# caltech-netlab/adacharge

Hardware: AMD Instinct MI355X
Metric: MPC QP solves/sec whole-node, 54 EVSE x horizon 12; max rate residual vs cvxpy (higher is better)
Workload: dtype f64; 1 GPU; caltech54 (Caltech-shaped, 54 EVSE) x horizon 12, quick_charge + equal_share*1e-12, SOC constraints, batches of 256 independent MPC snapshots (BASELINE.json configs[1]); one step = one acnqp_solve_batches call over 64 such batches per GPU (16384 problems), pinned host buffers in, host buffers out: H2D + kernels + D2H inside the timed region; batch=256, n_evse=54, horizon=12, constraint_type=SOC, parallelism=dp1 (own snapshots per GPU)

## Files before the change

adacharge_amd/backend.py:

```python
from __future__ import annotations

import ctypes as C
import dataclasses
import os
from dataclasses import dataclass
from typing import Optional

import numpy as np

from .builder import CONE_SOC, ProblemBatch, SiteData

_LIB_NAME = "libacn_qp_hip.so"
_LIB_DIR = os.path.join(os.path.dirname(os.path.abspath(__file__)), "lib")

STATUS_UNSET = 0
STATUS_SOLVED = 1
STATUS_MAX_ITER = 2
STATUS_PRIMAL_INFEASIBLE = 3
STATUS_EMPTY_SET = 4
STATUS_SOLVED_INACCURATE = 5
ACCEPTED_STATUSES = (STATUS_SOLVED, STATUS_SOLVED_INACCURATE)
STATUS_NAMES = {
    STATUS_UNSET: "unset",
    STATUS_SOLVED: "optimal",
    STATUS_MAX_ITER: "max_iter_reached",
    STATUS_PRIMAL_INFEASIBLE: "infeasible",
    STATUS_EMPTY_SET: "infeasible",
    STATUS_SOLVED_INACCURATE: "optimal_inaccurate",
}
PILOTS_CONTINUOUS, PILOTS_DISCRETE, PILOTS_REALLOCATE = 0, 1, 2
ADVANCE_REFUSED, ADVANCE_NO_ROW, ADVANCE_BAD_SLOT = 1, 2, 4
PREPARE_FUTURE = 1
PLANT_BAD_PLUG, PLANT_BAD_BATTERY = 1, 2
ESTIMATE_BAD_FRESH, ESTIMATE_BAD_SLOT = 1, 2
ROUTE_NAMES = {1: "wave1", 2: "wave2", 3: "wave3", 4: "wave4", 5: "wave5", 6: "tiled_ct1", 7: "tiled_ct2",
               8: "long_lds", 9: "long_ws", 10: "stream", 11: "general"}


class BackendUnavailable(RuntimeError):
    """The HIP library could not be loaded or no MI355X is visible."""


_I4, _F8, _U1 = np.int32, np.float64, np.uint8
_PROBLEM_ARRAYS = dict(horizon=_I4, lb=_F8, ub=_F8, q=_F8, pdiag=_F8, s_off=_I4, s_len=_I4, s_cap=_F8, s_eq=_U1, peak=_F8, lf=_F8,
                       dc=_F8, dfloor=_F8)
_NEXT_ARRAYS = tuple(k for k in _PROBLEM_ARRAYS if k != "s_eq")
_WARM = ("warm_x", "warm_y")
_TABLE_ARRAYS = dict(horizon=_I4, q_index=_I4, q_table=_F8, pdiag=_F8, s_eq=_U1, peak=_F8, lf=_F8, dc=_F8, dfloor=_F8, sess_seg=_I4,
                     s_evse=_I4, s_slot=_I4, s_off=_I4, s_len=_I4, s_cap=_F8, rate_seg=_I4, min_rates=_F8, max_rates=_F8)
_RESULT_ARRAYS = dict(x=_F8, status=_I4, iters=_I4, pri_res=_F8, dua_res=_F8, obj=_F8)
_PILOT_ARRAYS = dict(cre=_F8, cim=_F8, limits=_F8, max_pilot=_F8, levels=_F8, sess_seg=_I4, s_evse=_I4, s_arrived=_U1, s_cap=_F8)
_ADVANCE_ARRAYS = dict(q_table=_F8, h_scal=_F8, h_row=_I4, peak_series=_F8, a_seg=_I4, a_evse=_I4, a_slot=_I4, a_len=_I4, a_cap=_F8,
                       a_rate_seg=_I4, a_min=_F8, a_max=_F8)
_COST_ARRAYS = dict(c_weight=_F8, c_series=_F8)
_PREPARE_ARRAYS = dict(key=_I4, cre=_F8, cim=_F8, limits=_F8, min_pilot=_F8)
_PLANT_ARRAYS = dict(t_room=_F8, t_amps=_F8, t_knee=_F8, t_slope=_F8, plug=_I4)
_RESOLVE_ARRAYS = dict(sel_seg=_I4, sel_idx=_I4, pos=_I4)
SELECT_BAD_INDEX = 1
HOLD_BAD_ROW = 1


def _ints(*names):
    return [(k, C.c_int32) for k in names]


def _doubles(*names):
    return [(k, C.c_double) for k in names]


def _ptrs(*names):
    return [(k, C.c_void_p) for k in names]


class _Site(C.Structure):
    _fields_ = _ints("n_evse", "n_infra", "n_rows", "cone", "has_peak", "has_flat", "has_max") + _ptrs("G", "limits")


class _Problems(C.Structure):

    _fields_ = _ints("batch", "t_max", "k_sessions") + _ptrs(*_PROBLEM_ARRAYS, *_WARM)


class _Table(C.Structure):
    _fields_ = _ints("batch", "t_max", "k_sessions", "n_sessions", "n_horizons") + _ptrs(*_TABLE_ARRAYS)


class _Results(C.Structure):
    _fields_ = _ptrs(*_RESULT_ARRAYS, "y", "x_dev")


class _Duals(C.Structure):
    _fields_ = _ptrs("mu", "z", "res")


class _PilotPlan(C.Structure):
    _fields_ = _ints("batch", "t_max", "n_evse", "n_infra", "n_levels", "n_sessions", "mode") + _ptrs(*_PILOT_ARRAYS)


class _Pilots(C.Structure):
    _fields_ = _ptrs("pilots", "first", "visits")


class _AdvancePlan(C.Structure):
    _fields_ = (_ints("n_evse", "n_rows", "n_horizons", "step", "peak_len", "n_arrivals", "n_rates")
                + _doubles("done_tol", "kw_per_amp", "warm_arrival_gain") + _ptrs(*_ADVANCE_ARRAYS))


class ClockCost(C.Structure):

    _fields_ = _ints("n_evse", "series_len") + _doubles("coef") + _ptrs("weight", "series")


class _Next(C.Structure):
    _fields_ = _ptrs(*_NEXT_ARRAYS, *_WARM)


class _PreparePlan(C.Structure):
    _fields_ = _ints("n_evse", "n_infra") + _ptrs(*_PREPARE_ARRAYS)


class _PrepareView(C.Structure):
    _fields_ = _ptrs("v_evse", "v_arrived", "v_cap")


class Options(C.Structure):

    _fields_ = (_doubles("eps_abs", "eps_rel") + _ints("max_iter", "check_every", "adapt_every")
                + _doubles("rho", "sigma", "alpha", "adapt_tol", "reg_rel")
                + _ints("precision", "accel_mem", "stall_iters", "retry_passes", "retry_max_iter", "polish_iters")
                + _doubles("retry_rho", "inaccurate_floor") + _ints("polish_stall"))


def _abi():
    P, ptr, i32, i64, rc = C.POINTER, C.c_void_p, C.c_int32, C.c_int64, C.c_int
    h = stream = ptr
    solve = [h, P(_Problems), P(Options), P(_Results)]
    advance = [h, P(_Problems), ptr, ptr, ptr, ptr, P(_AdvancePlan)]
    rows = [
        ("acnqp_create", rc, [P(_Site), i32, P(ptr)]),
        ("acnqp_destroy", None, [h]),
        ("acnqp_solve_batch", rc, solve),
        ("acnqp_solve_batch_device", rc, solve + [stream]),
        ("acnqp_solve_batches", rc, [h, i32, P(_Problems), P(Options), P(_Results)]),
        ("acnqp_solve_table", rc, [h, P(_Table), P(Options), P(_Results)]),
        ("acnqp_host_alloc", ptr, [C.c_size_t]),
        ("acnqp_host_free", None, [ptr]),
        ("acnqp_default_options", None, [P(Options)]),
        ("acnqp_last_error", C.c_char_p, []),
        ("acnqp_abi_version", i32, []),
        ("acnqp_last_kernel_ms", C.c_float, [h]),
        ("acnqp_kernel_times", i32, [h, P(C.c_float), i32]),
        ("acnqp_launch_count", i64, [h]),
        ("acnqp_ordered_launch_count", i64, [h]),
        ("acnqp_polish_stats", rc, [h, P(i64), i32]),
        ("acnqp_accel_columns", i32, [h, i32, i32, i32, i32]),
        ("acnqp_route", i32, [h, i32, i32, i32, P(i32)]),
        ("acnqp_set_long_polish", rc, [h, i32]),
        ("acnqp_set_wide_polish", rc, [h, i32]),
    ]
    for stem, args in (
        ("acnqp_duals", [h, P(_Problems), P(Options), ptr, ptr, ptr, P(_Duals)]),
        ("acnqp_pilots", [h, P(_PilotPlan), ptr, P(_Pilots)]),
        ("acnqp_advance", advance + [P(_Next), ptr]),
        ("acnqp_advance_priced", advance + [P(ClockCost), P(_Next), ptr]),
        ("acnqp_prepare", [h, P(_Problems), P(_PreparePlan), ptr, ptr, P(_PrepareView), ptr]),
        ("acnqp_plant", [h, P(_Problems), ptr, ptr, i32] + [ptr] * 9),
        ("acnqp_estimate", [h, P(_Problems)] + [ptr] * 4 + [C.c_double] * 3 + [ptr] * 3),
        ("acnqp_select", [h, P(_Problems), i32, i32, i32, ptr, P(_Next), ptr, ptr]),
        ("acnqp_hold", [h, P(_Problems), i32, i32, i32, ptr, P(_Results), ptr, ptr, ptr, P(_Results), ptr, ptr]),
    ):
        rows += [(stem + "_host", rc, args), (stem + "_device", rc, args + [stream])]
    introspection = [
        ("acnqp_debug_polish_alongside", i64, [h]),
        ("acnqp_debug_direct_x", i64, [h]),
        ("acnqp_debug_wave_rank", rc, [h, P(i32)]),
        ("acnqp_debug_wave_evse_extent", rc, [h, P(i32)]),
        ("acnqp_debug_order_keys", rc, [h, P(_Problems), P(i32)]),
        ("acnqp_debug_copy_workspace", i64, [h, ptr, i64]),
    ]
    return tuple(r + (True,) for r in rows) + tuple(r + (False,) for r in introspection)


_ABI = _abi()
EXPORTED_SYMBOLS = tuple(name for name, _, _, declared in _ABI if declared)

_lib = None


def library_path() -> str:
    return os.environ.get("ACNQP_LIBRARY", os.path.join(_LIB_DIR, _LIB_NAME))


def load_library():
    global _lib
    if _lib is not None:
        return _lib
    try:
        import torch
    except ImportError:
        pass
    path = library_path()
    if not os.path.exists(path):
        raise BackendUnavailable(
            f"{path} not found: build it with `python -c 'import __graft_entry__ as g; g.build()'` "
            "(hipcc --offload-arch=gfx950).  adacharge_amd has no CPU fallback."
        )
    try:
        lib = C.CDLL(path)
    except OSError as exc:
        raise BackendUnavailable(f"cannot load {path}: {exc}") from exc
    for name, restype, argtypes, declared in _ABI:
        if declared or hasattr(lib, name):
            fn = getattr(lib, name)
            fn.restype, fn.argtypes = restype, argtypes
    _lib = lib
    return lib


def default_options(**overrides) -> Options:
    o = Options()
    load_library().acnqp_default_options(C.byref(o))
    for k, v in overrides.items():
        if not hasattr(o, k):
            raise TypeError(f"unknown solver option {k!r}")
        setattr(o, k, v)
    return o


def _check(rc: int, what: str):
    if rc != 0:
        msg = load_library().acnqp_last_error().decode()
        if rc == -3:
            raise BackendUnavailable(f"{what}: {msg}")
        if rc == -1:
            raise ValueError(f"{what}: {msg}")
        raise RuntimeError(f"{what} failed (rc={rc}): {msg}")


def _ptr(a: Optional[np.ndarray]):
    return None if a is None else a.ctypes.data_as(C.c_void_p)


def _addr(a: Optional[np.ndarray]):
    return None if a is None else a.ctypes.data


def _dptr(t):
    return None if t is None else C.c_void_p(t.data_ptr())


def _f8(a):
    return None if a is None else np.ascontiguousarray(a, np.float64)


def _i4(a):
    return None if a is None else np.ascontiguousarray(a, np.int32)


def _torch_dtype(dtype):
    import torch

    return getattr(torch, np.dtype(dtype).name)


def _want(t, name: str, dtype, shape=None, device=None) -> None:
    if t is None:
        return
    if device is None:
        ok = t.element_size() == np.dtype(dtype).itemsize
    else:
        import torch

        ok = isinstance(t, torch.Tensor) and t.device == device and t.dtype == _torch_dtype(dtype)
    if not ok or not t.is_contiguous() or (shape is not None and tuple(t.shape) != tuple(shape)):
        raise ValueError(f"{name} must be a contiguous torch.{np.dtype(dtype).name} tensor" + ("" if device is None else f" on {device}")
                         + ("" if shape is None else f" of shape {tuple(shape)}"))


def _absent(site: SiteData, peak: bool = False) -> tuple:
    return (() if site.has_flat else ("lf",)) + (() if site.has_max else ("dc", "dfloor")) + (("peak",) if peak and not site.has_peak else ())


def _host_arrays(src, arrays: dict, absent) -> dict:
    return {k: None if k in absent or (a := getattr(src, "T" if k == "horizon" else k)) is None else np.ascontiguousarray(a, dt)
            for k, dt in arrays.items()}


def _new_results(B: int, N: int, Tm: int, Mg: int, pinned: bool, want_y: bool, x_dev=None, out: Optional["BatchResult"] = None):
    if out is not None and out.x.shape == (B, N, Tm) and (not want_y or (out.y is not None and out.y.shape == (B, Mg, Tm))):
        res = out
    else:
        new = pinned_empty if pinned else np.zeros
        res = BatchResult(*[new((B, N, Tm) if k == "x" else B, dt) for k, dt in _RESULT_ARRAYS.items()])
        if want_y:
            res.y = new((B, Mg, Tm))
    r = _Results(*[_addr(getattr(res, k)) for k in _RESULT_ARRAYS], _addr(res.y) if want_y else None,
                 None if x_dev is None else C.c_void_p(int(x_dev)))
    return res, r


def _marshal_batch(site: SiteData, batch: ProblemBatch, pinned: bool, x_dev=None, warm=None, want_y=False):
    B, N, Tm = batch.B, batch.N, batch.Tm
    arrs = _host_arrays(batch, _PROBLEM_ARRAYS, _absent(site))
    wx = wy = None
    if warm is not None:
        wx, wy = _f8(warm[0]), _f8(warm[1])
        if wx.shape != (B, N, Tm) or wy.shape != (B, site.Mg, Tm):
            raise ValueError(f"warm start arrays must have shapes {(B, N, Tm)} and {(B, site.Mg, Tm)}")
    p = _Problems(B, Tm, batch.K, *[_addr(a) for a in arrs.values()], _addr(wx), _addr(wy))
    res, r = _new_results(B, N, Tm, site.Mg, pinned, want_y, x_dev)
    return p, r, res, (arrs, wx, wy)


def _device_problems(dev: "DeviceBatch", warm_x=None, warm_y=None) -> _Problems:
    return _Problems(dev.B, dev.Tm, dev.K, *[_dptr(getattr(dev, k)) for k in _PROBLEM_ARRAYS], _dptr(warm_x), _dptr(warm_y))


@dataclass
class BatchResult:
    x: np.ndarray
    status: np.ndarray
    iters: np.ndarray
    pri_res: np.ndarray
    dua_res: np.ndarray
    obj: np.ndarray
    kernel_ms: float = float("nan")
    y: Optional[np.ndarray] = None
    x_dev: Optional[object] = None
    handle: Optional[object] = None


@dataclass
class DualResult:
    mu: np.ndarray
    z: Optional[np.ndarray]
    stat: np.ndarray
    energy: np.ndarray
    site: np.ndarray
    comp: np.ndarray


class _PlanArrays:

    _DTYPES = {}

    def to_device(self, device):
        import torch

        moved = {k: None if getattr(self, k) is None else torch.from_numpy(np.ascontiguousarray(getattr(self, k), dt)).to(device)
                 for k, dt in self._DTYPES.items()}
        return dataclasses.replace(self, **moved)

    def _p(self, k: str, keep=None, row: int = 0, stacked: Optional[int] = None):
        a = getattr(self, k)
        if a is None or (a.numel() if hasattr(a, "numel") else a.size) == 0:
            return None
        if a.ndim == stacked:
            a = a[row]
        if hasattr(a, "data_ptr"):
            return C.c_void_p(a.data_ptr())
        a = np.ascontiguousarray(a, self._DTYPES[k])
        if keep is not None:
            keep.append(a)
        return _ptr(a)

    def _len(self, k: str, axis: int = 0) -> int:
        return 0 if getattr(self, k) is None else int(getattr(self, k).shape[axis])


@dataclass
class PilotPlan(_PlanArrays):
    mode: int
    B: int
    Tm: int
    N: int
    max_pilot: Optional[object] = None
    levels: Optional[object] = None
    cre: Optional[object] = None
    cim: Optional[object] = None
    limits: Optional[object] = None
    sess_seg: Optional[object] = None
    s_evse: Optional[object] = None
    s_arrived: Optional[object] = None
    s_cap: Optional[object] = None

    _DTYPES = _PILOT_ARRAYS
    _ARRAYS = tuple(_PILOT_ARRAYS)

    def _struct(self, batch=None, t_max=None, keep=None) -> "_PilotPlan":
        return _PilotPlan(int(self.B if batch is None else batch), int(self.Tm if t_max is None else t_max), self.N, self._len("cre"),
                          self._len("levels", 1), self._len("s_evse"), self.mode, *[self._p(k, keep) for k in _PILOT_ARRAYS])


@dataclass
class AdvancePlan(_PlanArrays):
    q_table: object
    h_scal: object
    h_row: object
    done_tol: float
    kw_per_amp: float
    peak_series: Optional[object] = None
    a_seg: Optional[object] = None
    a_evse: Optional[object] = None
    a_slot: Optional[object] = None
    a_len: Optional[object] = None
    a_cap: Optional[object] = None
    a_rate_seg: Optional[object] = None
    a_min: Optional[object] = None
    a_max: Optional[object] = None
    warm_arrival_gain: float = 0.0
    c_coef: Optional[float] = None
    c_weight: Optional[object] = None
    c_series: Optional[object] = None

    _DTYPES = {**_ADVANCE_ARRAYS, **_COST_ARRAYS}
    _ARRAYS = tuple(_ADVANCE_ARRAYS)

    def _struct(self, N: int, Mg: int, step: int, seg_row: int = 0, keep=None) -> "_AdvancePlan":
        A = self._len("a_evse")
        ptrs = [self._p(k, keep, seg_row, 2 if k == "a_seg" else None) for k in _ADVANCE_ARRAYS]
        if not A:
            ptrs[self._ARRAYS.index("a_seg")] = None
        return _AdvancePlan(int(N), int(Mg), int(self.q_table.shape[0]), int(step), self._len("peak_series", 1), A, self._len("a_min"),
                            float(self.done_tol), float(self.kw_per_amp), float(self.warm_arrival_gain), *ptrs)

    def _cost_struct(self, N: int, keep=None) -> Optional["ClockCost"]:
        given = [self.c_coef is not None, self.c_weight is not None, self.c_series is not None]
        if not any(given):
            return None
        if not all(given):
            raise ValueError("a clock cost needs c_coef, c_weight and c_series")
        if self.c_series.ndim != 2:
            raise ValueError("c_series must have shape (B, P)")
        for k, dt in _COST_ARRAYS.items():
            if hasattr(getattr(self, k), "data_ptr"):
                _want(getattr(self, k), k, dt)
        return ClockCost(int(N), int(self.c_series.shape[1]), float(self.c_coef), *[self._p(k, keep) for k in _COST_ARRAYS])


@dataclass
class PreparePlan(_PlanArrays):
    key: object
    cre: Optional[object] = None
    cim: Optional[object] = None
    limits: Optional[object] = None
    min_pilot: Optional[object] = None

    _DTYPES = _PREPARE_ARRAYS
    _ARRAYS = tuple(_PREPARE_ARRAYS)

    def _struct(self, N: int, key_row=None, min_rates: bool = True, keep=None) -> "_PreparePlan":
        return _PreparePlan(int(N), self._len("cre"), self._p("key", keep, 0 if key_row is None else key_row, 3), self._p("cre", keep),
                            self._p("cim", keep), self._p("limits", keep), self._p("min_pilot", keep) if min_rates else None)


@dataclass
class PlantPlan(_PlanArrays):
    t_room: object
    t_amps: object
    t_knee: object
    t_slope: object
    plug: object

    _DTYPES = _PLANT_ARRAYS
    _ARRAYS = tuple(_PLANT_ARRAYS)

    def _args(self, plug_row=None, keep=None) -> list:
        return [C.c_int32(self._len("t_room"))] + [self._p(k, keep, 0 if plug_row is None else plug_row, 3 if k == "plug" else None)
                                                   for k in _PLANT_ARRAYS]


@dataclass
class ResolvePlan(_PlanArrays):
    sel_seg: object
    sel_idx: object
    pos: object

# ... 255 lines not shown
                   warm_x=np.empty((B, N, Tm)) if xs is not None else None, warm_y=np.empty((B, Mg, Tm)) if ys is not None else None)
        flags = np.empty(B, np.int32)
        p = _Problems(B, Tm, K, lb=_ptr(lb), ub=_ptr(ub), s_off=_ptr(off), s_len=_ptr(ln), s_cap=_ptr(cap), dfloor=_ptr(dfl))
        keep = []
        pl = plan._struct(N, Mg, step, seg_row, keep)
        nx = _Next(*[_ptr(out[k]) for k in _NEXT_ARRAYS + _WARM])
        cost = plan._cost_struct(N, keep)
        if cost is not None and plan.c_series.shape[0] != B:
            raise ValueError(f"c_series has {plan.c_series.shape[0]} rows, the batch has {B} problems")
        head = (self._h, C.byref(p), _ptr(app), _ptr(stat), _ptr(xs), _ptr(ys), C.byref(pl))
        if cost is None:
            _check(self._lib.acnqp_advance_host(*head, C.byref(nx), _ptr(flags)), "acnqp_advance_host")
        else:
            _check(self._lib.acnqp_advance_priced_host(*head, C.byref(cost), C.byref(nx), _ptr(flags)), "acnqp_advance_priced_host")
        del keep
        out["flags"] = flags
        return {k: v for k, v in out.items() if v is not None}

    def advance_device(self, cur: "DeviceBatch", nxt: "DeviceBatch", applied, plan: AdvancePlan, step: int, flags, use_status: bool = True,
                       warm_x=None, warm_y=None, stream: int = 0, seg_row: int = 0) -> None:
        if (cur.B, cur.N, cur.Tm, cur.K) != (nxt.B, nxt.N, nxt.Tm, nxt.K):
            raise ValueError("cur and nxt must have the same shape (B, N, Tm, K)")
        if warm_y is not None and cur.y is None:
            raise ValueError("warm_y needs the site-row multipliers: DeviceBatch(..., want_y=True)")
        _want(applied, "applied", _F8, (cur.B, cur.N))
        _want(flags, "flags", _I4, (cur.B,))
        p = _device_problems(cur)
        pl = plan._struct(cur.N, self.site.Mg, step, seg_row)
        nx = _Next(*[_dptr(getattr(nxt, k)) for k in _NEXT_ARRAYS], _dptr(warm_x), _dptr(warm_y))
        cost = plan._cost_struct(cur.N)
        if cost is not None and plan.c_series.shape[0] != cur.B:
            raise ValueError(f"c_series has {plan.c_series.shape[0]} rows, the batch has {cur.B} problems")
        head = (self._h, C.byref(p), _dptr(applied), _dptr(cur.status) if use_status else None,
                _dptr(cur.x) if warm_x is not None else None, _dptr(cur.y) if warm_y is not None else None, C.byref(pl))
        if cost is None:
            _check(self._lib.acnqp_advance_device(*head, C.byref(nx), _dptr(flags), C.c_void_p(stream)), "acnqp_advance_device")
        else:
            _check(self._lib.acnqp_advance_priced_device(*head, C.byref(cost), C.byref(nx), _dptr(flags), C.c_void_p(stream)),
                   "acnqp_advance_priced_device")

    def prepare_host(self, cur: dict, plan: PreparePlan, want_view: bool = True, min_rates: bool = True, key_row=None) -> dict:
        lb, ub = np.array(cur["lb"], np.float64, order="C"), np.array(cur["ub"], np.float64, order="C")
        off, ln, cap = _i4(cur["s_off"]), _i4(cur["s_len"]), _f8(cur["s_cap"])
        if lb.ndim != 3 or lb.shape[1] != self.site.N or ub.shape != lb.shape:
            raise ValueError("cur needs lb, ub of shape (B, N, Tm) for the handle's site")
        B, N, Tm = lb.shape
        K = off.shape[1] if off.ndim == 3 else 1
        if off.size != B * K * N or ln.size != off.size or cap.size != off.size:
            raise ValueError("cur needs s_off, s_len, s_cap of shape (B, K, N)")
        view = dict(v_evse=np.empty((B, N), np.int32), v_arrived=np.empty((B, N), np.uint8), v_cap=np.empty((B, N))) if want_view else {}
        flags = np.empty(B, np.int32)
        p = _Problems(B, Tm, K, s_off=_ptr(off), s_len=_ptr(ln), s_cap=_ptr(cap))
        keep = []
        pl = plan._struct(N, key_row, min_rates, keep)
        v = _PrepareView(*[_ptr(view.get(k)) for k in ("v_evse", "v_arrived", "v_cap")])
        _check(self._lib.acnqp_prepare_host(self._h, C.byref(p), C.byref(pl), _ptr(lb), _ptr(ub), C.byref(v), _ptr(flags)), "acnqp_prepare_host")
        del keep
        return dict(lb=lb, ub=ub, flags=flags, **view)

    def prepare_device(self, cur: "DeviceBatch", plan: PreparePlan, flags, v_evse=None, v_arrived=None, v_cap=None, min_rates: bool = True,
                       key_row=None, stream: int = 0) -> None:
        import torch

        here = torch.device("cuda", self.device)
        B, N, Tm, K = cur.B, cur.N, cur.Tm, cur.K
        M = plan._len("cre")
        if plan.key is None or not hasattr(plan.key, "dim"):
            raise ValueError("plan.key must be a tensor on the handle's GPU (PreparePlan.to_device)")
        _want(plan.key, "plan.key", _I4, (B, N) if plan.key.dim() == 2 else (plan.key.shape[0], B, N), here)
        if plan.key.dim() == 3 and not 0 <= (0 if key_row is None else int(key_row)) < plan.key.shape[0]:
            raise ValueError("key_row is outside plan.key")
        for k, shape in dict(cre=(M, N), cim=(M, N), limits=(M,), min_pilot=(N,)).items():
            _want(getattr(plan, k), "plan." + k, _PREPARE_ARRAYS[k], shape, here)
        for k, shape in dict(lb=(B, N, Tm), ub=(B, N, Tm), s_off=(B, K, N), s_len=(B, K, N), s_cap=(B, K, N)).items():
            _want(getattr(cur, k), "cur." + k, _PROBLEM_ARRAYS[k], shape, here)
        _want(flags, "flags", _I4, (B,), here)
        if flags is None:
            raise ValueError("flags is required")
        for t, name, dt in ((v_evse, "v_evse", _I4), (v_arrived, "v_arrived", _U1), (v_cap, "v_cap", _F8)):
            _want(t, name, dt, (B, N), here)
        p = _Problems(B, Tm, K, s_off=_dptr(cur.s_off), s_len=_dptr(cur.s_len), s_cap=_dptr(cur.s_cap))
        pl = plan._struct(N, key_row, min_rates)
        v = _PrepareView(_dptr(v_evse), _dptr(v_arrived), _dptr(v_cap))
        _check(self._lib.acnqp_prepare_device(self._h, C.byref(p), C.byref(pl), _dptr(cur.lb), _dptr(cur.ub), C.byref(v), _dptr(flags),
                                              C.c_void_p(stream)), "acnqp_prepare_device")

    def plant_host(self, cur: dict, plan: PlantPlan, pilots, bat, room, status=None, plug_row=None) -> dict:
        off, ln, pil, stat = _i4(cur["s_off"]), _i4(cur["s_len"]), _f8(pilots), _i4(status)
        bat, room = np.array(bat, np.int32, order="C"), np.array(room, np.float64, order="C")
        if pil.ndim != 2 or pil.shape[1] != self.site.N:
            raise ValueError("pilots must have the shape (B, N) of the handle's site")
        B, N = pil.shape
        K = off.shape[1] if off.ndim == 3 else 1
        if off.size != B * K * N or ln.size != off.size or bat.shape != (B, N) or room.shape != (B, N):
            raise ValueError("cur needs s_off, s_len of shape (B, K, N); bat and room have the shape (B, N)")
        plug = plan.plug if plan.plug.ndim == 2 else plan.plug[0 if plug_row is None else plug_row]
        if plug.shape != (B, N) or (stat is not None and stat.shape != (B,)):
            raise ValueError("plan.plug needs one (B, N) block per step and status the shape (B,)")
        actual, flags = np.empty((B, N)), np.empty(B, np.int32)
        p = _Problems(B, 1, K, s_off=_ptr(off), s_len=_ptr(ln))
        keep = []
        _check(self._lib.acnqp_plant_host(self._h, C.byref(p), _ptr(pil), _ptr(stat), *plan._args(plug_row, keep), _ptr(bat), _ptr(room),
                                          _ptr(actual), _ptr(flags)), "acnqp_plant_host")
        del keep
        return dict(bat=bat, room=room, actual=actual, flags=flags)

    def plant_device(self, cur: "DeviceBatch", plan: PlantPlan, pilots, bat, room, actual, flags, status=None, plug_row=None,
                     stream: int = 0) -> None:
        import torch

        here = torch.device("cuda", self.device)
        B, N, K = cur.B, cur.N, cur.K
        R = plan._len("t_room")
        if plan.plug is None or not hasattr(plan.plug, "dim"):
            raise ValueError("plan.plug must be a tensor on the handle's GPU (PlantPlan.to_device)")
        _want(plan.plug, "plan.plug", _I4, (B, N) if plan.plug.dim() == 2 else (plan.plug.shape[0], B, N), here)
        if plan.plug.dim() == 3 and not 0 <= (0 if plug_row is None else int(plug_row)) < plan.plug.shape[0]:
            raise ValueError("plug_row is outside plan.plug")
        for k in ("t_room", "t_amps", "t_knee", "t_slope"):
            _want(getattr(plan, k), "plan." + k, _F8, (R,), here)
        for k in ("s_off", "s_len"):
            _want(getattr(cur, k), "cur." + k, _I4, (B, K, N), here)
        for t, name, dt, shape in ((pilots, "pilots", _F8, (B, N)), (bat, "bat", _I4, (B, N)), (room, "room", _F8, (B, N)),
                                   (actual, "actual", _F8, (B, N)), (flags, "flags", _I4, (B,)), (status, "status", _I4, (B,))):
            if t is None and name != "status":
                raise ValueError(f"{name} is required")
            _want(t, name, dt, shape, here)
        p = _Problems(B, cur.Tm, K, s_off=_dptr(cur.s_off), s_len=_dptr(cur.s_len))
        _check(self._lib.acnqp_plant_device(self._h, C.byref(p), _dptr(pilots), _dptr(status), *plan._args(plug_row), _dptr(bat), _dptr(room),
                                            _dptr(actual), _dptr(flags), C.c_void_p(stream)), "acnqp_plant_device")

    def estimate_host(self, cur: dict, fresh, est, pilots=None, actual=None, status=None, up_threshold: float = 1.0,
                      down_threshold: float = 1.0, up_increment: float = 1.0, fresh_row=None) -> dict:
        lb, ub = _f8(cur["lb"]), _f8(cur["ub"])
        off, ln, fr = _i4(cur["s_off"]), _i4(cur["s_len"]), _i4(fresh)
        pil, act, stat = _f8(pilots), _f8(actual), _i4(status)
        est = np.array(est, np.float64, order="C")
        if ub.ndim != 3 or ub.shape[1] != self.site.N or lb.shape != ub.shape:
            raise ValueError("cur needs lb, ub of shape (B, N, Tm) for the handle's site")
        B, N, Tm = ub.shape
        K = off.shape[1] if off.ndim == 3 else 1
        if fr.ndim == 3:
            fr = fr[0 if fresh_row is None else fresh_row]
        if off.size != B * K * N or ln.size != off.size or fr.shape != (B, N) or est.shape != (B, N):
            raise ValueError("cur needs s_off, s_len of shape (B, K, N); fresh needs one (B, N) block per step and est the shape (B, N)")
        for a, name, shape in ((pil, "pilots", (B, N)), (act, "actual", (B, N)), (stat, "status", (B,))):
            if a is not None and a.shape != shape:
                raise ValueError(f"{name} must have the shape {shape}")
        fr = np.ascontiguousarray(fr)
        ub_out, flags = np.empty((B, N, Tm)), np.empty(B, np.int32)
        p = _Problems(B, Tm, K, s_off=_ptr(off), s_len=_ptr(ln), lb=_ptr(lb), ub=_ptr(ub))
        _check(self._lib.acnqp_estimate_host(self._h, C.byref(p), _ptr(fr), _ptr(pil), _ptr(act), _ptr(stat), float(up_threshold),
                                             float(down_threshold), float(up_increment), _ptr(est), _ptr(ub_out), _ptr(flags)),
               "acnqp_estimate_host")
        return dict(est=est, ub=ub_out, flags=flags)

    def estimate_device(self, cur: "DeviceBatch", fresh, est, ub_out, flags, pilots=None, actual=None, status=None, up_threshold: float = 1.0,
                        down_threshold: float = 1.0, up_increment: float = 1.0, fresh_row=None, stream: int = 0) -> None:
        import torch

        here = torch.device("cuda", self.device)
        B, N, Tm, K = cur.B, cur.N, cur.Tm, cur.K
        if fresh is None or not hasattr(fresh, "dim"):
            raise ValueError("fresh must be a tensor on the handle's GPU")
        _want(fresh, "fresh", _I4, (B, N) if fresh.dim() == 2 else (fresh.shape[0], B, N), here)
        row = 0
        if fresh.dim() == 3:
            row = 0 if fresh_row is None else int(fresh_row)
            if not 0 <= row < fresh.shape[0]:
                raise ValueError("fresh_row is outside fresh")
        for k, shape in dict(lb=(B, N, Tm), ub=(B, N, Tm), s_off=(B, K, N), s_len=(B, K, N)).items():
            _want(getattr(cur, k), "cur." + k, _PROBLEM_ARRAYS[k], shape, here)
        for t, name, dt, shape in ((est, "est", _F8, (B, N)), (ub_out, "ub_out", _F8, (B, N, Tm)), (flags, "flags", _I4, (B,)),
                                   (pilots, "pilots", _F8, (B, N)), (actual, "actual", _F8, (B, N)), (status, "status", _I4, (B,))):
            if t is None and name in ("est", "ub_out", "flags"):
                raise ValueError(f"{name} is required")
            _want(t, name, dt, shape, here)
        p = _Problems(B, Tm, K, s_off=_dptr(cur.s_off), s_len=_dptr(cur.s_len), lb=_dptr(cur.lb), ub=_dptr(cur.ub))
        fr = C.c_void_p(fresh.data_ptr() + row * B * N * 4)
        _check(self._lib.acnqp_estimate_device(self._h, C.byref(p), fr, _dptr(pilots), _dptr(actual), _dptr(status), float(up_threshold),
                                               float(down_threshold), float(up_increment), _dptr(est), _dptr(ub_out), _dptr(flags),
                                               C.c_void_p(stream)), "acnqp_estimate_device")

    def select_device(self, cur: "DeviceBatch", dense: "DeviceBatch", idx, flags, m: Optional[int] = None, warm_x=None, warm_y=None,
                      out_warm_x=None, out_warm_y=None, stream: int = 0) -> None:
        m = int(idx.shape[0] if m is None else m)
        if (cur.N, cur.Tm, cur.K) != (dense.N, dense.Tm, dense.K):
            raise ValueError("cur and dense must have the same shape (N, Tm, K)")
        if m > dense.B or m > idx.shape[0] or m > flags.shape[0]:
            raise ValueError(f"dense, idx and flags need room for m = {m} problems")
        for t, name, rows in ((out_warm_x, "out_warm_x", (cur.N, cur.Tm)), (out_warm_y, "out_warm_y", (self.site.Mg, cur.Tm))):
            if t is not None and (t.shape[0] < m or tuple(t.shape[1:]) != rows):
                raise ValueError(f"{name} needs at least m = {m} rows of shape {rows}")
        _want(idx, "idx", _I4)
        _want(flags, "flags", _I4)
        _want(warm_x, "warm_x", _F8, (cur.B, cur.N, cur.Tm))
        _want(warm_y, "warm_y", _F8, (cur.B, self.site.Mg, cur.Tm))
        _want(out_warm_x, "out_warm_x", _F8)
        _want(out_warm_y, "out_warm_y", _F8)
        p = _device_problems(cur, warm_x, warm_y)
        nx = _Next(*[_dptr(getattr(dense, k)) for k in _NEXT_ARRAYS], _dptr(out_warm_x), _dptr(out_warm_y))
        _check(self._lib.acnqp_select_device(self._h, C.byref(p), cur.N, self.site.Mg, m, _dptr(idx), C.byref(nx), _dptr(dense.s_eq),
                                             _dptr(flags), C.c_void_p(stream)), "acnqp_select_device")

    def hold_device(self, cur: "DeviceBatch", dense: Optional["DeviceBatch"], pos, m: int, held_x, prev_status, solved, flags, held_y=None,
                    stream: int = 0) -> None:
        B, N, Tm, Mg = cur.B, cur.N, cur.Tm, self.site.Mg
        want_y = held_y is not None
        if want_y and (cur.y is None or (dense is not None and dense.y is None)):
            raise ValueError("held_y needs the site-row multipliers: DeviceBatch(..., want_y=True)")
        if dense is None and m != 0:
            raise ValueError("dense is required when m > 0")
        if dense is not None and ((dense.N, dense.Tm) != (N, Tm) or dense.B < m):
            raise ValueError(f"dense must have the shape (N, Tm) of cur and hold at least m = {m} problems")
        for t, name, dt, shape in ((pos, "pos", _I4, (B,)), (held_x, "held_x", _F8, (B, N, Tm)), (held_y, "held_y", _F8, (B, Mg, Tm)),
                                   (prev_status, "prev_status", _I4, (B,)), (solved, "solved", _U1, (B,)), (flags, "flags", _I4, (B,))):
            _want(t, name, dt, shape)
        p = _Problems(B, Tm, cur.K, lb=_dptr(cur.lb), ub=_dptr(cur.ub))
        r = _Results() if dense is None else _Results(x=_dptr(dense.x), status=_dptr(dense.status), iters=_dptr(dense.iters),
                                                      y=_dptr(dense.y) if want_y else None)
        o = _Results(x=_dptr(cur.x), status=_dptr(cur.status), iters=_dptr(cur.iters), y=_dptr(cur.y) if want_y else None)
        _check(self._lib.acnqp_hold_device(self._h, C.byref(p), N, Mg, int(m), _dptr(pos), C.byref(r), _dptr(held_x), _dptr(held_y),
                                           _dptr(prev_status), C.byref(o), _dptr(solved), _dptr(flags), C.c_void_p(stream)),
               "acnqp_hold_device")

    def select_host(self, cur: dict, idx, warm_x=None, warm_y=None) -> dict:
        src = {k: np.ascontiguousarray(cur[k], dt) for k, dt in _PROBLEM_ARRAYS.items() if cur.get(k) is not None and k not in _absent(self.site, peak=True)}
        idx = _i4(idx)
        wx, wy = _f8(warm_x), _f8(warm_y)
        B, N, Tm = src["lb"].shape
        K, m = src["s_off"].shape[1], len(idx)
        out = {k: np.empty((m,) + a.shape[1:], a.dtype) for k, a in src.items()}
        if wx is not None:
            out["warm_x"] = np.empty((m, N, Tm))
        if wy is not None:
            out["warm_y"] = np.empty((m,) + wy.shape[1:])
        out["flags"] = np.empty(m, np.int32)
        p = _Problems(B, Tm, K, *[_ptr(src.get(k)) for k in _PROBLEM_ARRAYS], _ptr(wx), _ptr(wy))
        nx = _Next(*[_ptr(out.get(k)) for k in _NEXT_ARRAYS + _WARM])
        _check(self._lib.acnqp_select_host(self._h, C.byref(p), N, self.site.Mg, m, _ptr(idx), C.byref(nx), _ptr(out["s_eq"]),
                                           _ptr(out["flags"])), "acnqp_select_host")
        return out

    def hold_host(self, pos, m: int, rx, rstatus, riters, held_x, prev_status, lb, ub, ry=None, held_y=None) -> dict:
        pos, rst, rit, pst = _i4(pos), _i4(rstatus), _i4(riters), _i4(prev_status)
        rx, ry, hx, hy, lb, ub = _f8(rx), _f8(ry), _f8(held_x), _f8(held_y), _f8(lb), _f8(ub)
        B, N, Tm = hx.shape
        out = dict(x=np.empty((B, N, Tm)), status=np.empty(B, np.int32), iters=np.empty(B, np.int32), solved=np.empty(B, np.uint8),
                   flags=np.empty(B, np.int32))
        if hy is not None:
            out["y"] = np.empty(hy.shape)
        nul = lambda a: None if a is None or a.size == 0 else _ptr(a)
        p = _Problems(B, Tm, 1, lb=_ptr(lb), ub=_ptr(ub))
        r = _Results(x=nul(rx), status=nul(rst), iters=nul(rit), y=nul(ry))
        o = _Results(x=_ptr(out["x"]), status=_ptr(out["status"]), iters=_ptr(out["iters"]), y=_ptr(out.get("y")))
        _check(self._lib.acnqp_hold_host(self._h, C.byref(p), N, self.site.Mg, int(m), _ptr(pos), C.byref(r), _ptr(hx), _ptr(hy), _ptr(pst),
                                         C.byref(o), _ptr(out["solved"]), _ptr(out["flags"])), "acnqp_hold_host")
        return out

    def _kernel_ms_of_call(self) -> float:
        before = int(self._lib.acnqp_launch_count(self._h))
        ms = self.kernel_times()
        if any(m < 0 for m in ms) or before - self._launches_seen > len(ms):
            self._launches_seen = before
            return float("nan")
        self._launches_seen = before
        return float(sum(ms))

    def polish_stats(self) -> dict:
        buf = (C.c_int64 * 16)()
        _check(self._lib.acnqp_polish_stats(self._h, buf, 16), "acnqp_polish_stats")
        out = dict(zip(("attempted", "solved", "gave_up_rows", "gave_up_pivot", "gave_up_rounds", "gave_up_kkt", "rounds"), [int(v) for v in buf[:7]]))
        out["phase_us"] = [int(v) // 100 for v in buf[8:16]]
        return out

    def polish_alongside(self) -> int:
        n = int(self._lib.acnqp_debug_polish_alongside(self._h))
        if n < 0:
            raise RuntimeError("acnqp_debug_polish_alongside failed")
        return n

    def wave_rank(self) -> dict:
        buf = (C.c_int32 * 3)()
        if self._lib.acnqp_debug_wave_rank(self._h, buf) != 0:
            raise RuntimeError("acnqp_debug_wave_rank failed")
        return dict(rank=int(buf[0]), eig_ksteps=int(buf[1]), extent=int(buf[2]))

    def wave_evse_extent(self) -> dict:
        buf = (C.c_int32 * 3)()
        if self._lib.acnqp_debug_wave_evse_extent(self._h, buf) != 0:
            raise RuntimeError("acnqp_debug_wave_evse_extent failed")
        return dict(n_evse=int(buf[0]), evse_ksteps=int(buf[1]), extent=int(buf[2]))

    def order_keys(self, dev: "DeviceBatch") -> np.ndarray:
        keys = np.empty(dev.B, np.int32)
        p = _device_problems(dev)
        if self._lib.acnqp_debug_order_keys(self._h, C.byref(p), keys.ctypes.data_as(C.POINTER(C.c_int32))) != 0:
            raise RuntimeError("acnqp_debug_order_keys failed")
        return keys

    def direct_x(self) -> int:
        return int(self._lib.acnqp_debug_direct_x(self._h))

    def ordered_launches(self) -> int:
        return int(self._lib.acnqp_ordered_launch_count(self._h))

    def last_kernel_ms(self) -> float:
        return float(self._lib.acnqp_last_kernel_ms(self._h))

    def kernel_times(self, capacity: int = 64):
        buf = (C.c_float * int(capacity))()
        n = int(self._lib.acnqp_kernel_times(self._h, buf, int(capacity)))
        return [float(buf[k]) for k in range(n)]

    def route(self, t_max: int, k_sessions: int, batch: int = 1):
        pol = C.c_int32(0)
        fam = int(self._lib.acnqp_route(self._h, int(t_max), int(k_sessions), int(batch), C.byref(pol)))
        if fam == 0:
            raise ValueError(f"acnqp_route: no route for t_max={t_max}, k_sessions={k_sessions}, batch={batch}")
        return ROUTE_NAMES[fam], bool(pol.value)

    def accel_columns(self, t_max: int, k_sessions: int, options: Options) -> int:
        return int(self._lib.acnqp_accel_columns(self._h, int(t_max), int(k_sessions), int(options.precision),
                                                 int(options.accel_mem)))


class DeviceBatch:

    def __init__(self, batch: ProblemBatch, device, want_y: bool = False):
        import torch

        dev = torch.device(device)
        self.B, self.N, self.Tm, self.K = batch.B, batch.N, batch.Tm, batch.K
        for k, dt in _PROBLEM_ARRAYS.items():
            a = getattr(batch, "T" if k == "horizon" else k)
            if a is None and k in ("lf", "dc", "dfloor"):
                a = np.zeros(batch.B)
            setattr(self, k, None if a is None else torch.from_numpy(np.ascontiguousarray(a, dt)).to(dev))
        self._alloc_results(batch.site.Mg, want_y, dev)

    def _alloc_results(self, Mg: int, want_y: bool, dev) -> None:
        import torch

        for k, dt in _RESULT_ARRAYS.items():
            setattr(self, k, torch.zeros((self.B, self.N, self.Tm) if k == "x" else self.B, dtype=_torch_dtype(dt), device=dev))
        self.y = torch.zeros((self.B, Mg, self.Tm), dtype=torch.float64, device=dev) if want_y else None

    def head(self, m: int) -> "DeviceBatch":
        if not 0 <= m <= self.B:
            raise ValueError(f"m must be in [0, {self.B}]")
        view = self.__class__.__new__(self.__class__)
        view.B, view.N, view.Tm, view.K = int(m), self.N, self.Tm, self.K
        for k in (*_PROBLEM_ARRAYS, *_RESULT_ARRAYS, "y"):
            t = getattr(self, k)
            setattr(view, k, None if t is None else t[:m])
        return view

    @classmethod
    def empty(cls, site: SiteData, B: int, Tm: int, K: int, device, want_y: bool = False, s_eq: int = 0, dfloor: float = 0.0,
              with_peak: Optional[bool] = None) -> "DeviceBatch":
        import torch

        dev = torch.device(device)
        self = cls.__new__(cls)
        self.B, self.N, self.Tm, self.K = int(B), site.N, int(Tm), int(K)
        shapes = dict(lb=(self.B, self.N, self.Tm), ub=(self.B, self.N, self.Tm), q=(self.B, self.N, self.Tm), s_off=(self.B, self.K, self.N),
                      s_len=(self.B, self.K, self.N), s_cap=(self.B, self.K, self.N), peak=(self.B, self.Tm))
        fill = dict(horizon=1, dfloor=float(dfloor), s_eq=int(s_eq), peak=float("inf"))
        no_peak = not (site.has_peak if with_peak is None else with_peak)
        for k, dt in _PROBLEM_ARRAYS.items():
            setattr(self, k, None if k == "peak" and no_peak else
                    torch.full(shapes.get(k, (self.B,)), fill.get(k, 0), dtype=_torch_dtype(dt), device=dev))
        self._alloc_results(site.Mg, want_y, dev)
        return self
```

adacharge_amd/csrc/acn_qp_api.hip:

```cpp
#include <hip/hip_runtime.h>

#include <algorithm>
#include <chrono>
#include <cmath>
#include <cstdint>
#include <cstdio>
#include <cstdlib>
#include <cstring>
#include <initializer_list>
#include <string>
#include <vector>

#include "acn_qp.h"
#include "acn_qp_launch.hpp"
#include "acn_qp_duals.hpp"
#include "acn_qp_pilots.hpp"
#include "acn_qp_advance.hpp"
#include "acn_qp_prepare.hpp"
#include "acn_qp_plant.hpp"
#include "acn_qp_estimate.hpp"
#include "acn_qp_hold.hpp"
#include "acn_qp_site.hpp"

namespace {

thread_local std::string g_last_error;

int fail(int rc, const std::string& msg) {
  g_last_error = msg;
  return rc;
}

#define HIP_TRY(expr)                                                                    \
  do {                                                                                   \
    hipError_t _e = (expr);                                                              \
    if (_e != hipSuccess)                                                                \
      return fail(ACNQP_ERR_HIP, std::string(#expr) + ": " + hipGetErrorString(_e));    \
  } while (0)

template <hipError_t (*Alloc)(void**, size_t), hipError_t (*Free)(void*)>
struct GrowBuf {
  void* p = nullptr;
  size_t cap = 0;
  hipError_t reserve(size_t bytes) {
    if (bytes <= cap) return hipSuccess;
    release();
    hipError_t e = Alloc(&p, bytes ? bytes : 16);
    if (e == hipSuccess) cap = bytes;
    return e;
  }
  void release() {
    if (p) (void)Free(p);
    p = nullptr;
    cap = 0;
  }
};
inline hipError_t device_alloc(void** p, size_t bytes) { return hipMalloc(p, bytes); }
inline hipError_t pinned_alloc(void** p, size_t bytes) { return hipHostMalloc(p, bytes, hipHostMallocDefault); }
using DevBuf = GrowBuf<device_alloc, hipFree>;
using HostBuf = GrowBuf<pinned_alloc, hipHostFree>;

struct Want { DevBuf* buf; size_t bytes; };
inline hipError_t reserve_behind(hipStream_t st, std::initializer_list<Want> wants) {
  const bool grow = std::any_of(wants.begin(), wants.end(), [](const Want& w) { return w.bytes > w.buf->cap; });
  hipError_t e = grow ? hipStreamSynchronize(st) : hipSuccess;
  for (const Want& w : wants)
    if (e == hipSuccess) e = w.buf->reserve(w.bytes);
  return e;
}

}

struct acnqp_handle {
  int device = 0;
  acnqp::SiteShape shape;
  std::vector<double> G, limits;
  acnqp::SiteDev site;
  static constexpr int kEvRing = 64;
  hipEvent_t ev_start[kEvRing] = {}, ev_stop[kEvRing] = {};
  long long launches = 0, reported = 0;
  long long ordered_launches = 0;
  long long direct_x_last = 0;
  static constexpr int kSlots = 4;
  struct Slot { hipStream_t st = nullptr; DevBuf in, out, tin; } slot[kSlots];
  HostBuf small_in, small_out;
  hipEvent_t h2d_done[kSlots] = {nullptr, nullptr, nullptr, nullptr};
  struct Work {
    hipStream_t st; DevBuf buf; DevBuf ord; DevBuf pol; long long used; hipEvent_t last; DevBuf dua;
    hipEvent_t fork = nullptr, join = nullptr;
    void release() {
      if (last) (void)hipEventDestroy(last);
      if (fork) (void)hipEventDestroy(fork);
      if (join) (void)hipEventDestroy(join);
      last = fork = join = nullptr;
      for (DevBuf* b : {&buf, &ord, &pol, &dua}) b->release();
    }
  };
  std::vector<Work> work;
  long long work_clock = 0;
  static size_t max_caller_workspaces() {
    static const size_t v = [] {
      const char* e = std::getenv("ACNQP_CALLER_STREAMS");
      const long n = e ? std::atol(e) : 0;
      return (size_t)(n > 0 && n <= 256 ? n : 16);
    }();
    return v;
  }
  Work* work_for(hipStream_t st) {
    for (auto& w : work) if (w.st == st) { w.used = ++work_clock; return &w; }
    bool own = false;
    for (auto& sl : slot) own = own || sl.st == st;
    if (!own) {
      size_t callers = 0, lru = work.size();
      for (size_t k = 0; k < work.size(); ++k) {
        bool mine = false;
        for (auto& sl : slot) mine = mine || sl.st == work[k].st;
        if (mine) continue;
        ++callers;
        if (lru == work.size() || work[k].used < work[lru].used) lru = k;
      }
      if (callers >= max_caller_workspaces()) {
        if (work[lru].last) (void)hipEventSynchronize(work[lru].last);
        work[lru].release();
        work.erase(work.begin() + (long)lru);
      }
    }
    hipEvent_t ev = nullptr;
    (void)hipEventCreateWithFlags(&ev, hipEventDisableTiming);
    work.push_back(Work{st, DevBuf(), DevBuf(), DevBuf(), ++work_clock, ev, DevBuf()});
    return &work.back();
  }
  int cus = 0;
  int32_t* pol_stats = nullptr;
  hipStream_t aux = nullptr;
  bool long_polish = false;
  bool wide_polish = false;
  DevBuf post_stage;
};

namespace {

static_assert(acnqp::kRouteMaxK == acnqp::kMaxK, "acn_qp_route.hpp restates the on-chip kernels' session slots");

acnqp::RouteSwitches route_switches() {
  static const bool no_wave = std::getenv("ACNQP_NO_WAVE") != nullptr;
  static const bool no_wave2 = std::getenv("ACNQP_NO_WAVE2") != nullptr;
  static const int min_batch = std::getenv("ACNQP_WAVE_MIN_BATCH") ? std::atoi(std::getenv("ACNQP_WAVE_MIN_BATCH")) : 1;
  acnqp::RouteSwitches sw;
  sw.no_wave = no_wave; sw.no_wave2 = no_wave2; sw.wave_min_batch = min_batch;
  sw.no_long = std::getenv("ACNQP_NO_LONG") != nullptr;
  const char* e = std::getenv("ACNQP_LDS_LONG");
  sw.lds_long = !(e && std::atoi(e) == 0);
  return sw;
}
acnqp::Route route_of(const acnqp_handle* h, int t_max, int k_sessions, int batch) {
  return acnqp::route_for(h->shape, t_max, k_sessions, batch, route_switches());
}

struct Kernels {
  static int wave_accel() { return acnqp::wave_accel_columns(); }
  static int tiled_accel(int MT, int CT, int NP, int K) { int single = 0; return acnqp::accel_capacity_best(4, MT, CT, NP, K, &single); }
  static int stream_accel() { return acnqp::kStreamAccelMax; }
  static int long_accel() { return acnqp::kLongAccelMax; }
  static int general_accel() { return acnqp::kGenAccelMax; }
  static long long stream_workspace(int NP, int CT, int K, int MT, int accel) { return acnqp::stream_workspace(NP, CT, K, MT, accel); }
  static long long long_workspace(int NP, int t_max, int K, int MT, int accel) { return acnqp::long_workspace(NP, acnqp::long_tiles(t_max), K, MT, accel); }
};

int polish_block_doubles(const acnqp_handle* h, const acnqp::Route& rt) {
  static const bool no_polish = std::getenv("ACNQP_NO_POLISH") != nullptr;
  if (no_polish) return -1;
  const acnqp::SiteShape& s = h->shape;
  const int nrow_site = s.M + s.has_peak;
  if (rt.polish_long_shape)
    return h->long_polish && acnqp::polish_long_holds(s.N, rt.t_max, rt.k_sessions, s.Mg, nrow_site) ? acnqp::polish_long_block_doubles(rt.t_max, s.Mg) : -1;
  if (!rt.polish_shape) return -1;
  const bool two_per_cu = rt.tiled && rt.t_max <= 16 && s.MR == 16 && rt.k_sessions == 1;
  const int blk = acnqp::polish_blocks_that_fit(s.N, rt.t_max, s.Mg, nrow_site, acnqp::polish_max_sess(s.N, rt.k_sessions),
                                                two_per_cu ? 76 * 1024 : 160 * 1024);
  return blk < 2 * nrow_site * (2 * nrow_site + 1) / 2 ? -1 : blk;
}

bool wide_polish_route(const acnqp_handle* h, const acnqp::Route& rt) {
  static const bool no_polish = std::getenv("ACNQP_NO_POLISH") != nullptr;
  const acnqp::SiteShape& s = h->shape;
  return !no_polish && h->wide_polish && rt.polish_wide_shape && acnqp::polish_wide_holds(s.N, rt.t_max, rt.k_sessions, s.Mg, s.M + s.has_peak);
}

int solve_batch_device(acnqp_handle* h, const acnqp_problems* p, const acnqp_options* o, acnqp_results* r, hipStream_t st, bool nothing_follows,
                       double* const* x_host = nullptr);

}

#include "acn_qp_pipeline.hpp"
#include "acn_qp_post.hpp"
extern "C" {

int32_t acnqp_abi_version(void) { return ACNQP_ABI_VERSION; }

int32_t acnqp_route(acnqp_handle* h, int32_t t_max, int32_t k_sessions, int32_t batch, int32_t* polish) {
  if (polish) *polish = 0;
  if (!h || t_max < 1 || t_max > 4096 || k_sessions < 1 || k_sessions > 4096 || batch < 1) return 0;
  const acnqp::Route r = route_of(h, t_max, k_sessions, batch);
  acnqp_options o;
  acnqp_default_options(&o);
  if (polish) *polish = (polish_block_doubles(h, r) >= 0 && o.polish_iters > 0 && o.polish_iters < o.max_iter) ? 1 : 0;
  if (polish && wide_polish_route(h, r) && o.polish_iters > 0) *polish = 1;
  return r.family;
}

const char* acnqp_last_error(void) { return g_last_error.c_str(); }

void acnqp_default_options(acnqp_options* o) {
  if (!o) return;
  o->eps_abs = 1e-8;
  o->eps_rel = 1e-8;
  o->max_iter = 20000;
  o->check_every = 20;
  o->adapt_every = 20;
  o->rho = 0.02;
  o->sigma = 1e-6;
  o->alpha = 1.4;
  o->adapt_tol = 3.0;
  o->reg_rel = 0.06;
  o->precision = 64;
  o->accel_mem = 5;
  o->stall_iters = 3000;
  o->retry_passes = 2;
  o->retry_max_iter = 8000;
  o->polish_iters = 800;
  o->retry_rho = 0.5;
  o->inaccurate_floor = 1e-5;
  o->polish_stall = 0;
}

int acnqp_create(const acnqp_site* site, int32_t device_id, acnqp_handle** out) {
  if (!site || !out) return fail(ACNQP_ERR_INVALID, "acnqp_create: null argument");
  *out = nullptr;
  const int N = site->n_evse, M = site->n_infra, Mg = site->n_rows;
  if (N < 1 || N > 1024)
    return fail(ACNQP_ERR_INVALID, "acnqp_create: n_evse must be in [1, 1024]");
  if (site->cone != ACNQP_CONE_LINEAR && site->cone != ACNQP_CONE_SOC)
    return fail(ACNQP_ERR_INVALID, "acnqp_create: cone must be ACNQP_CONE_LINEAR or ACNQP_CONE_SOC");
  const int expect = (site->cone == ACNQP_CONE_SOC ? 2 * M : M) + (site->has_peak ? 1 : 0) + (site->has_flat ? 1 : 0) + (site->has_max ? 1 : 0);
  if (M < 0 || Mg != expect || Mg > 48)
    return fail(ACNQP_ERR_INVALID, "acnqp_create: n_rows inconsistent with n_infra/cone/has_peak/has_flat/has_max or > 48");
  const int padded = acnqp::padded_rows(site->cone, M, site->has_peak, site->has_flat, site->has_max);
  if (padded > 48)
    return fail(ACNQP_ERR_INVALID, "acnqp_create: " + std::to_string(padded) + " site rows after padding (SOC: 8*ceil(n_infra/4) "
                                   "+ peak/flat/max rows) > 48, the padded limit");
  if (Mg > 0 && !site->G) return fail(ACNQP_ERR_INVALID, "acnqp_create: G is null");
  if (M > 0 && !site->limits) return fail(ACNQP_ERR_INVALID, "acnqp_create: limits is null");
  for (int j = 0; j < M; ++j)
    if (!(site->limits[j] >= 0)) return fail(ACNQP_ERR_INVALID, "acnqp_create: limits must be >= 0");

  int ndev = 0;
  if (hipGetDeviceCount(&ndev) != hipSuccess || ndev == 0)
    return fail(ACNQP_ERR_NO_DEVICE, "acnqp_create: no HIP device visible");
  if (device_id < 0 || device_id >= ndev) return fail(ACNQP_ERR_INVALID, "acnqp_create: bad device_id");
  HIP_TRY(hipSetDevice(device_id));

  acnqp_handle* h = new acnqp_handle();
  h->device = device_id;
  h->shape = acnqp::site_shape(N, M, site->cone, site->has_peak, site->has_flat, site->has_max);
  if (hipDeviceGetAttribute(&h->cus, hipDeviceAttributeMultiprocessorCount, device_id) != hipSuccess || h->cus < 1) h->cus = 256;
  h->G.assign(site->G, site->G + (size_t)Mg * N);
  h->limits.assign(site->limits, site->limits + M);
  hipError_t e = hipSuccess;
  for (int k = 0; k < acnqp_handle::kEvRing && e == hipSuccess; ++k) {
    e = hipEventCreate(&h->ev_start[k]);
    if (e == hipSuccess) e = hipEventCreate(&h->ev_stop[k]);
  }
  for (int k = 0; k < acnqp_handle::kSlots && e == hipSuccess; ++k) {
    e = hipStreamCreateWithFlags(&h->slot[k].st, hipStreamNonBlocking);
    if (e == hipSuccess) e = hipEventCreateWithFlags(&h->h2d_done[k], hipEventDisableTiming);
  }
  if (e != hipSuccess) {
    std::string msg = std::string("acnqp_create: ") + hipGetErrorString(e);
    acnqp_destroy(h);
    return fail(ACNQP_ERR_HIP, msg);
  }
  std::string err;
  const int rc = acnqp::build_site_dev(&h->shape, h->G, h->limits, &h->site, &err);
  if (rc != ACNQP_OK) { acnqp_destroy(h); return fail(rc, err); }
  if (hipMalloc((void**)&h->pol_stats, 32 * sizeof(int32_t)) != hipSuccess || hipMemset(h->pol_stats, 0, 32 * sizeof(int32_t)) != hipSuccess ||
      hipStreamCreateWithFlags(&h->aux, hipStreamNonBlocking) != hipSuccess) {
    acnqp_destroy(h);
    return fail(ACNQP_ERR_HIP, "acnqp_create: polish counters and stream");
  }
  *out = h;
  return ACNQP_OK;
}

void acnqp_destroy(acnqp_handle* h) {
  if (!h) return;
  (void)hipSetDevice(h->device);
  h->site.release();
  for (int k = 0; k < acnqp_handle::kEvRing; ++k) {
    if (h->ev_start[k]) (void)hipEventDestroy(h->ev_start[k]);
    if (h->ev_stop[k]) (void)hipEventDestroy(h->ev_stop[k]);
  }
  for (auto& sl : h->slot) {
    if (sl.st) { (void)hipStreamSynchronize(sl.st); (void)hipStreamDestroy(sl.st); }
    for (DevBuf* b : {&sl.in, &sl.out, &sl.tin}) b->release();
  }
  if (h->aux) { (void)hipStreamSynchronize(h->aux); (void)hipStreamDestroy(h->aux); }
  h->small_in.release();
  h->small_out.release();
  for (auto& ev : h->h2d_done) if (ev) (void)hipEventDestroy(ev);
  for (auto& w : h->work) w.release();
  h->post_stage.release();
  if (h->pol_stats) (void)hipFree(h->pol_stats);
  delete h;
}

static bool is_nan(double v) {
  uint64_t u;
  std::memcpy(&u, &v, sizeof u);
  return (u & 0x7fffffffffffffffull) > 0x7ff0000000000000ull;
}

static int check_problem_shapes(const acnqp_handle* h, const acnqp_problems* p, const acnqp_options* o,
                                const acnqp_results* r) {
  if (!h || !p || !o || !r) return fail(ACNQP_ERR_INVALID, "acnqp_solve_batch: null argument");
  if (p->batch < 0) return fail(ACNQP_ERR_INVALID, "acnqp_solve_batch: negative batch");
  if (p->batch == 0) return ACNQP_OK;
  if (p->t_max < 1 || p->t_max > 4096)
    return fail(ACNQP_ERR_INVALID, "acnqp_solve_batch: t_max must be in [1, 4096]");
  if (p->k_sessions < 1 || p->k_sessions > 4096)
    return fail(ACNQP_ERR_INVALID, "acnqp_solve_batch: k_sessions must be in [1, 4096]");
  if (!p->horizon || !p->lb || !p->ub || !p->q || !p->pdiag || !p->s_off || !p->s_len || !p->s_cap || !p->s_eq)
    return fail(ACNQP_ERR_INVALID, "acnqp_solve_batch: null problem array");
  if (h->shape.has_peak && !p->peak) return fail(ACNQP_ERR_INVALID, "acnqp_solve_batch: site has a peak row but peak is null");
  if (h->shape.has_flat && !p->lf) return fail(ACNQP_ERR_INVALID, "acnqp_solve_batch: site has a flat row but lf is null");
  if (h->shape.has_max && (!p->dc || !p->dfloor)) return fail(ACNQP_ERR_INVALID, "acnqp_solve_batch: site has a max row but dc/dfloor is null");
  if ((p->warm_x == nullptr) != (p->warm_y == nullptr))
    return fail(ACNQP_ERR_INVALID, "acnqp_solve_batch: warm_x and warm_y must be given together");
  if (!r->x || !r->status || !r->iters || !r->pri_res || !r->dua_res || !r->obj)
    return fail(ACNQP_ERR_INVALID, "acnqp_solve_batch: null result array");
  for (double v : {o->eps_abs, o->eps_rel, o->rho, o->sigma, o->alpha, o->adapt_tol, o->reg_rel, o->retry_rho, o->inaccurate_floor})
    if (is_nan(v)) return fail(ACNQP_ERR_INVALID, "acnqp_solve_batch: invalid option value");
  if (!(o->eps_abs >= 0) || !(o->eps_rel >= 0) || o->max_iter < 1 || o->check_every < 1 || !(o->rho > 0) ||
      !(o->sigma >= 0) || !(o->alpha > 0 && o->alpha < 2) || !(o->adapt_tol > 1) || !(o->reg_rel >= 0) ||
      o->adapt_every < 0 || o->polish_iters < 0 || o->polish_stall < 0 || o->stall_iters < 0 || o->retry_passes < 0 || o->retry_passes > 8 || o->retry_max_iter < 1 ||
      !(o->retry_rho > 0) || !(o->inaccurate_floor >= 0))
    return fail(ACNQP_ERR_INVALID, "acnqp_solve_batch: invalid option value");
  if (o->precision != 64)
    return fail(ACNQP_ERR_INVALID, "acnqp_solve_batch: precision must be 64 (the fp32 loop was removed: it missed the "
                                   "1e-4 rate tolerance on weakly convex problems and was not faster; DESIGN.md section 3)");
  return ACNQP_OK;
}

namespace {

acnqp::TiledArgs tiled_args(const acnqp_handle* h, const acnqp_problems* p, const acnqp_options* o, const acnqp_results* r, hipStream_t st) {
  const acnqp::SiteShape& s = h->shape;
  const acnqp::SiteDev* d = &h->site;
  acnqp::TiledArgs a;
  a.B = p->batch; a.N = s.N; a.Tm = p->t_max; a.K = p->k_sessions; a.NP = s.NP(); a.MR = s.MR;
  a.G = d->G; a.Ghat = d->Ghat; a.Q = d->Q; a.lam = d->lam; a.rowlim = d->rowlim; a.rowtype = d->rowtype;
  a.fragG = d->fragG; a.fragQ = d->fragQ; a.fragG2 = d->fragG2; a.fragQ2 = d->fragQ2;
  a.horizon = p->horizon; a.lb = p->lb; a.ub = p->ub; a.q = p->q; a.pdiag = p->pdiag;
  a.s_off = p->s_off; a.s_len = p->s_len; a.s_cap = p->s_cap; a.s_eq = p->s_eq; a.peak = s.has_peak ? p->peak : nullptr;
  a.lf = s.has_flat ? p->lf : nullptr;
  a.dc = s.has_max ? p->dc : nullptr;
  a.dfloor = s.has_max ? p->dfloor : nullptr;
  a.warm_x = (p->warm_x && p->warm_y) ? p->warm_x : nullptr;
  a.warm_y = (p->warm_x && p->warm_y) ? p->warm_y : nullptr;
  a.y_out = r->y;
  a.rowabi = d->rowabi; a.rowscale = d->rowscale; a.Mg = s.Mg;
  a.x = r->x; a.status = r->status; a.iters = r->iters; a.pri = r->pri_res; a.dua = r->dua_res; a.obj = r->obj;
  a.eps_abs = o->eps_abs; a.eps_rel = o->eps_rel; a.rho0 = o->rho; a.sigma = o->sigma; a.alpha = o->alpha;
  a.adapt_tol = o->adapt_tol; a.reg_rel = o->reg_rel;
  a.max_iter = o->max_iter; a.check_every = o->check_every; a.adapt_every = o->adapt_every;
  a.peak_scale = d->peak_scale; a.flat_scale = d->flat_scale; a.max_scale = d->max_scale;
  a.accel_mem = std::max(0, o->accel_mem);
  a.stall_iters = o->stall_iters; a.retry_passes = o->retry_passes; a.retry_max_iter = o->retry_max_iter;
  a.retry_rho = o->retry_rho; a.inacc_floor = o->inaccurate_floor;
  a.pbuf_single = 0;
  a.order = nullptr;
  a.queue = nullptr;
  bool own = false;
  for (auto& sl : h->slot) own = own || sl.st == st;
  a.grid_oversub = own ? 4 : 1;
  a.polish_iters = 0; a.polish_stall = 0; a.resume = 0; a.y_for_polish_only = 0; a.pol_rows = 0; a.pol_list = nullptr; a.pol_count = nullptr; a.pol_retired = nullptr; a.count_dev = nullptr;
  a.x_host = nullptr;
  return a;
}

hipError_t launch_order_keys(acnqp_handle* h, const acnqp::Route& rt, const acnqp_problems* p, hipStream_t st, int32_t* keys) {
  static const bool by_sessions = [] { const char* e = std::getenv("ACNQP_ORDER_KEY"); return e && std::strcmp(e, "sessions") == 0; }();
  const acnqp::SiteShape& s = h->shape;
  const int g_rows = s.cone == ACNQP_CONE_SOC ? 2 * s.M : s.M;
  const int waves = by_sessions || rt.family == ACNQP_ROUTE_WAVE4 ? 0 : order_key_waves((size_t)s.N, (size_t)p->t_max, (size_t)g_rows);
  if (waves == 0) {
    hipLaunchKernelGGL(session_keys_kernel, dim3((p->batch + 3) / 4), dim3(256), 0, st, p->s_len, p->k_sessions * s.N, p->batch, keys);
    return hipGetLastError();
  }
  OrderKeyArgs ka;
  ka.B = p->batch; ka.N = s.N; ka.Tm = p->t_max; ka.K = p->k_sessions; ka.M = s.M; ka.soc = s.cone == ACNQP_CONE_SOC; ka.has_peak = s.has_peak;
  ka.lb = p->lb; ka.ub = p->ub; ka.s_cap = p->s_cap; ka.peak = p->peak; ka.G = h->site.Gabi; ka.limits = h->site.limabi;
  ka.s_off = p->s_off; ka.s_len = p->s_len; ka.horizon = p->horizon; ka.keys = keys;
  const size_t lds = ((size_t)g_rows * s.N + (size_t)waves * s.N * p->t_max) * sizeof(double);
  const hipError_t e = acnqp::ensure_dynamic_lds(reinterpret_cast<const void*>(order_keys_kernel), lds);
  if (e != hipSuccess) return e;
  hipLaunchKernelGGL(order_keys_kernel, dim3((p->batch + waves - 1) / waves), dim3(64 * waves), lds, st, ka);
  return hipGetLastError();
}

int schedule_launch(acnqp_handle* h, acnqp_handle::Work* wk, const acnqp::Route& rt, const acnqp_problems* p, hipStream_t st, acnqp::TiledArgs* a) {
  static const bool no_order = std::getenv("ACNQP_NO_ORDER") != nullptr;
  static const bool no_queue_env = std::getenv("ACNQP_NO_QUEUE") != nullptr;
  static const bool queue_all = std::getenv("ACNQP_QUEUE_ALL") != nullptr;
  const bool no_queue = no_queue_env || !(rt.on_chip || queue_all);
  const bool want_order = p->batch >= kOrderMinBatch && !no_order && !h->shape.has_flat && !h->shape.has_max;
  if (!no_queue || want_order) {
    const size_t need = 256 + (want_order ? (size_t)p->batch * 2 * sizeof(int32_t) : 0);
    HIP_TRY(reserve_behind(st, {{&wk->ord, need}}));
    if (!no_queue) {
      a->queue = static_cast<int32_t*>(wk->ord.p);
      HIP_TRY(hipMemsetAsync(a->queue, 0, sizeof(int32_t), st));
    }
    if (want_order) {
      int32_t* keys = static_cast<int32_t*>(wk->ord.p) + 64;
      int32_t* order = keys + p->batch;
      HIP_TRY(launch_order_keys(h, rt, p, st, keys));
      hipLaunchKernelGGL(order_sort_kernel, dim3(1), dim3(kOrderKeys), 0, st, keys, p->batch, order);
      a->order = order;
      h->ordered_launches++;
    }
  }
  static const bool ws_per_problem = std::getenv("ACNQP_WS_PER_PROBLEM") != nullptr;
  a->ws_by_slot = a->queue && !ws_per_problem ? 1 : 0;
  a->grid_cap = a->ws_by_slot ? std::min(p->batch, 2 * h->cus) : p->batch;
  return ACNQP_OK;
}

struct Workspace { void* p = nullptr; long long per_problem = 0; };
int reserve_workspace(acnqp_handle::Work* wk, const acnqp::Route& rt, hipStream_t st, acnqp::TiledArgs* a, Workspace* ws) {
  if (rt.tiled) return ACNQP_OK;
  if (rt.stream || rt.lng) a->accel_mem = std::min(a->accel_mem, rt.accel_cap<Kernels>());
  ws->per_problem = rt.workspace_doubles<Kernels>(a->accel_mem);
  const size_t need = (size_t)ws->per_problem * a->grid_cap * sizeof(double);
  HIP_TRY(reserve_behind(st, {{&wk->buf, need}}));
  ws->p = wk->buf.p;
  return ACNQP_OK;
}

int wave_extent_of(const acnqp_handle* h) {
  static const bool full_rank = std::getenv("ACNQP_WAVE_FULL_RANK") != nullptr;
  return acnqp::wave_eig_extent(h->site.eig_ksteps, full_rank);
}

int wave_evse_extent_of(const acnqp_handle* h) {
  static const bool full_evse = std::getenv("ACNQP_WAVE_FULL_EVSE") != nullptr;
  return acnqp::wave_evse_extent(h->shape.N, full_evse);
}

hipError_t launch_solver(const acnqp_handle* h, const acnqp::Route& rt, const acnqp::TiledArgs& aa, const Workspace& ws, hipStream_t st) {
  if (rt.wv > 0) {
    acnqp::WaveSite w;
    w.Ghat = h->site.GhatW; w.lam = h->site.lamW; w.fragQ = h->site.fragQW; w.extent = wave_extent_of(h);
    w.evse_ksteps = wave_evse_extent_of(h);
    return acnqp::launch_wave(aa, w, st);
  }
  if (rt.tiled) return rt.t_max <= 16 ? acnqp::launch_tiled_ct1(aa, st) : acnqp::launch_tiled_ct2(aa, st);
  if (rt.stream || rt.lng) {
    acnqp::StreamArgs sa;
    sa.t = aa; sa.work = static_cast<double*>(ws.p); sa.ws_per_problem = ws.per_problem;
    return rt.stream ? acnqp::launch_stream(sa, st) : acnqp::launch_long(sa, st, rt.lds);
  }
  const long long nvar = (long long)rt.site.N * rt.t_max;
  const int nt = nvar <= 4096 ? 256 : (nvar <= 12288 ? 512 : 1024);
  acnqp::GeneralArgs ga;
  ga.t = aa; ga.work = ws.p; ga.ws_per_problem = ws.per_problem; ga.pair_stride = 4;
  return acnqp::launch_general(ga, nt, st);
}

__global__ __launch_bounds__(256) void pol_x_to_host_kernel(const int32_t* list, const int32_t* count, int B, int nv, const double* x,
                                                            double* const* x_host) {
  const int n = min(*count, B);
  for (int pos = blockIdx.x; pos < n; pos += gridDim.x) {
    const int b = list[pos];
    if (b < 0 || b >= B) continue;
    double* const dst = x_host[b];
    if (dst == nullptr) continue;
    for (int k = threadIdx.x; k < nv; k += blockDim.x) dst[k] = x[(size_t)b * nv + k];
  }
}

int launch_with_polish(acnqp_handle* h, acnqp_handle::Work* wk, const acnqp::Route& rt, const acnqp::TiledArgs& a, const Workspace& ws,
                       int pol_blk, const acnqp_problems* p, const acnqp_options* o, const acnqp_results* r, hipStream_t st, bool nothing_follows,
                       hipError_t* e) {
  static const bool no_alongside = std::getenv("ACNQP_NO_POLISH_ALONGSIDE") != nullptr;
  static const long long along_polls = [] {
    const char* v = std::getenv("ACNQP_POLISH_ALONGSIDE_SPINS");
    const long long n = v ? std::atoll(v) : (1ll << 21);
    return n < 0 ? 0ll : n;
  }();
  static const int along_grid = [] {
    const char* v = std::getenv("ACNQP_POLISH_ALONGSIDE_GRID");
    const int n = v ? std::atoi(v) : 0;
    return n > 0 && n <= 256 ? n : 16;
  }();
  const bool lng = rt.polish_long_shape;
  const bool alongside = nothing_follows && !no_alongside && rt.wv > 0 && rt.wv != 3 && a.queue != nullptr && !lng;
  const acnqp::SiteShape& s = h->shape;
  const acnqp::SiteDev* d = &h->site;
  const int nrow_site = s.M + s.has_peak;
  const int pol_max = lng ? acnqp::polish_long_rows(s.Mg, p->t_max) : acnqp::polish_max_rows(nrow_site, p->t_max);
  const int pol_grid = lng ? acnqp::polish_long_grid(p->batch) : std::max(1, std::min(p->batch, a.grid_oversub > 1 ? 32 : h->cus));
  const size_t sbytes = lng ? (size_t)acnqp::polish_long_slab_bytes(s.N, p->t_max, p->k_sessions, s.Mg, nrow_site, pol_grid) : 0;
  const size_t ybytes = r->y ? 0 : (size_t)p->batch * s.Mg * p->t_max * sizeof(double);
  const size_t lbytes = ((size_t)p->batch * sizeof(int32_t) + 255) & ~(size_t)255;
  const size_t yb256 = (ybytes + 255) & ~(size_t)255;
  const size_t need = 256 + lbytes + (lng ? yb256 + sbytes : ybytes);
  HIP_TRY(reserve_behind(st, {{&wk->pol, need}}));
  int32_t* ctr = static_cast<int32_t*>(wk->pol.p);
  int32_t* list = ctr + 64;
  double* ybuf = r->y ? r->y : reinterpret_cast<double*>(static_cast<char*>(wk->pol.p) + 256 + lbytes);
  double* slab = lng ? reinterpret_cast<double*>(static_cast<char*>(wk->pol.p) + 256 + lbytes + yb256) : nullptr;
  HIP_TRY(hipMemsetAsync(ctr, 0, 256, st));
  if (alongside) {
    HIP_TRY(hipMemsetAsync(list, 0xff, lbytes, st));
    if (!wk->fork) HIP_TRY(hipEventCreateWithFlags(&wk->fork, hipEventDisableTiming));
    if (!wk->join) HIP_TRY(hipEventCreateWithFlags(&wk->join, hipEventDisableTiming));
    HIP_TRY(hipEventRecord(wk->fork, st));
  }
  acnqp::TiledArgs a1 = a;
  a1.polish_iters = o->polish_iters - o->polish_iters % std::max(1, o->check_every);
  if (a1.polish_iters < o->check_every) a1.polish_iters = o->check_every;
  a1.pol_list = list; a1.pol_count = ctr + 2; a1.y_out = ybuf; a1.pol_rows = lng ? pol_max + 8 : pol_max;
  static const int early = std::getenv("ACNQP_EARLY_HANDOVER") ? std::atoi(std::getenv("ACNQP_EARLY_HANDOVER")) : 0;
  a1.polish_stall = early > 1 ? early : (early == 1 ? std::max(o->check_every, a1.polish_iters / 4) : o->polish_stall);
  a1.y_for_polish_only = r->y ? 0 : 1;
  a1.pol_retired = alongside ? ctr + 3 : nullptr;
  *e = launch_solver(h, rt, a1, ws, st);
  if (*e == hipSuccess) {
    acnqp::PolishArgs pa;
    pa.B = p->batch; pa.N = s.N; pa.Tm = p->t_max; pa.K = p->k_sessions; pa.M = s.M; pa.Mg = s.Mg; pa.cone = s.cone;
    pa.has_peak = s.has_peak; pa.max_rows = pol_max; pa.blk_doubles = pol_blk;
    pa.max_sess = lng ? acnqp::polish_long_sess(s.N, p->k_sessions) : acnqp::polish_max_sess(s.N, p->k_sessions);
    pa.G = d->Gabi; pa.limits = d->limabi;
    pa.horizon = p->horizon; pa.lb = p->lb; pa.ub = p->ub; pa.q = p->q; pa.pdiag = p->pdiag;
    pa.s_off = p->s_off; pa.s_len = p->s_len; pa.s_cap = p->s_cap; pa.s_eq = p->s_eq; pa.peak = s.has_peak ? p->peak : nullptr;
    pa.x = r->x; pa.y = ybuf; pa.status = r->status; pa.iters = r->iters; pa.pri = r->pri_res; pa.dua = r->dua_res; pa.obj = r->obj;
    pa.list = list; pa.count = ctr + 2; pa.queue = ctr + 0; pa.stats = h->pol_stats; pa.reg_rel = o->reg_rel;
    pa.alongside = 0; pa.expected = p->batch; pa.retired = ctr + 3; pa.max_polls = along_polls; pa.taken = h->pol_stats + 16;
    if (alongside) {
      acnqp::PolishArgs pc = pa;
      pc.alongside = 1;
      HIP_TRY(hipStreamWaitEvent(h->aux, wk->fork, 0));
      *e = acnqp::launch_polish(pc, along_grid, h->aux);
      HIP_TRY(hipEventRecord(wk->join, h->aux));
      HIP_TRY(hipStreamWaitEvent(st, wk->join, 0));
    }
    if (*e == hipSuccess) *e = acnqp::launch_polish(pa, pol_grid, st, slab);
  }
  if (*e == hipSuccess) {
    acnqp::TiledArgs a3 = a;
    a3.resume = 1; a3.order = list; a3.count_dev = ctr + 2; a3.queue = ctr + 1;
    a3.warm_x = r->x; a3.warm_y = ybuf;
    a3.x_host = nullptr;
    a3.ws_by_slot = 1; a3.grid_cap = std::min(p->batch, a.grid_oversub > 1 ? 64 : 2 * h->cus);
    if (!a.ws_by_slot) a3.grid_cap = std::min(a3.grid_cap, a.grid_cap);
    *e = launch_solver(h, rt, a3, ws, st);
  }
  if (*e == hipSuccess && a.x_host != nullptr) {
    hipLaunchKernelGGL(pol_x_to_host_kernel, dim3((unsigned)std::min(p->batch, 64)), dim3(256), 0, st, list, ctr + 2, p->batch,
                       s.N * p->t_max, r->x, a.x_host);
    *e = hipGetLastError();
  }
  return ACNQP_OK;
}

int launch_wide_polish(acnqp_handle* h, acnqp_handle::Work* wk, const acnqp::Route& rt, const acnqp::TiledArgs& a, const Workspace& ws,
                       const acnqp_problems* p, const acnqp_options* o, const acnqp_results* r, hipStream_t st, hipError_t* e) {
  const acnqp::SiteShape& s = h->shape;
  const acnqp::SiteDev* d = &h->site;
  const int nrow_site = s.M + s.has_peak;
  const int grid = acnqp::polish_wide_grid(p->batch);
  const size_t sbytes = (size_t)acnqp::polish_wide_slab_bytes(s.N, p->t_max, p->k_sessions, s.Mg, nrow_site, grid);
  const size_t lbytes = ((size_t)p->batch * sizeof(int32_t) + 255) & ~(size_t)255;
  const size_t ybytes = r->y ? 0 : (((size_t)p->batch * s.Mg * p->t_max * sizeof(double) + 255) & ~(size_t)255);
  HIP_TRY(reserve_behind(st, {{&wk->pol, 256 + 2 * lbytes + ybytes + sbytes}}));
  char* base = static_cast<char*>(wk->pol.p);
  int32_t* ctr = reinterpret_cast<int32_t*>(base);
  int32_t* list = reinterpret_cast<int32_t*>(base + 256);
  int32_t* saved = reinterpret_cast<int32_t*>(base + 256 + lbytes);
  double* ybuf = r->y ? r->y : reinterpret_cast<double*>(base + 256 + 2 * lbytes);
  double* slab = reinterpret_cast<double*>(base + 256 + 2 * lbytes + ybytes);
  HIP_TRY(hipMemsetAsync(ctr, 0, 256, st));
  acnqp::TiledArgs a1 = a;
  a1.y_out = ybuf;
  *e = launch_solver(h, rt, a1, ws, st);
  if (*e == hipSuccess) *e = acnqp::launch_polish_wide_list(r->status, saved, list, ctr + 2, p->batch, st);
  if (*e == hipSuccess) {
    acnqp::PolishArgs pa;
    pa.B = p->batch; pa.N = s.N; pa.Tm = p->t_max; pa.K = p->k_sessions; pa.M = s.M; pa.Mg = s.Mg; pa.cone = s.cone;
    pa.has_peak = s.has_peak; pa.max_rows = acnqp::polish_long_rows(s.Mg, p->t_max);
    pa.blk_doubles = acnqp::polish_wide_block_doubles(p->t_max, s.Mg);
    pa.max_sess = acnqp::polish_long_sess(s.N, p->k_sessions);
    pa.G = d->Gabi; pa.limits = d->limabi;
    pa.horizon = p->horizon; pa.lb = p->lb; pa.ub = p->ub; pa.q = p->q; pa.pdiag = p->pdiag;
    pa.s_off = p->s_off; pa.s_len = p->s_len; pa.s_cap = p->s_cap; pa.s_eq = p->s_eq; pa.peak = s.has_peak ? p->peak : nullptr;
    pa.x = r->x; pa.y = ybuf; pa.status = r->status; pa.iters = r->iters; pa.pri = r->pri_res; pa.dua = r->dua_res; pa.obj = r->obj;
    pa.list = list; pa.count = ctr + 2; pa.queue = ctr + 0; pa.stats = h->pol_stats; pa.reg_rel = o->reg_rel;
    pa.alongside = 0; pa.expected = p->batch; pa.retired = nullptr; pa.max_polls = 0; pa.taken = nullptr;
    *e = acnqp::launch_polish_wide(pa, slab, grid, st);
  }
  if (*e == hipSuccess) *e = acnqp::launch_polish_wide_restore(r->status, saved, list, ctr + 2, p->batch, st);
  return ACNQP_OK;
}

int solve_batch_device(acnqp_handle* h, const acnqp_problems* p, const acnqp_options* o, acnqp_results* r, hipStream_t st, bool nothing_follows,
                       double* const* x_host) {
  int rc = check_problem_shapes(h, p, o, r);
  if (rc != ACNQP_OK) return rc;
  if (p->batch == 0) return ACNQP_OK;
  HIP_TRY(hipSetDevice(h->device));
  acnqp::TiledArgs a = tiled_args(h, p, o, r, st);
  (void)hipGetLastError();
  HIP_TRY(hipMemsetAsync(r->status, 0, (size_t)p->batch * sizeof(int32_t), st));
  const int evk = (int)(h->launches % acnqp_handle::kEvRing);
  HIP_TRY(hipEventRecord(h->ev_start[evk], st));
  const acnqp::Route rt = route_of(h, p->t_max, p->k_sessions, p->batch);
  if (x_host != nullptr && !rt.direct_x()) return fail(ACNQP_ERR_INVALID, "direct x on a route that cannot store it");
  a.x_host = x_host;
  acnqp_handle::Work* wk = h->work_for(st);
  if ((rc = schedule_launch(h, wk, rt, p, st, &a)) != ACNQP_OK) return rc;
  Workspace ws;
  if ((rc = reserve_workspace(wk, rt, st, &a, &ws)) != ACNQP_OK) return rc;
  const int pol_blk = (o->polish_iters > 0 && o->polish_iters < o->max_iter && !a.warm_x) ? polish_block_doubles(h, rt) : -1;
  hipError_t e = hipSuccess;
  if (pol_blk >= 0) {
    if ((rc = launch_with_polish(h, wk, rt, a, ws, pol_blk, p, o, r, st, nothing_follows, &e)) != ACNQP_OK) return rc;
  } else if (o->polish_iters > 0 && wide_polish_route(h, rt)) {
    if ((rc = launch_wide_polish(h, wk, rt, a, ws, p, o, r, st, &e)) != ACNQP_OK) return rc;
  } else {
    e = launch_solver(h, rt, a, ws, st);
  }
  if (e != hipSuccess) return fail(ACNQP_ERR_HIP, std::string("kernel launch: ") + hipGetErrorString(e));
  HIP_TRY(hipEventRecord(h->ev_stop[evk], st));
  if (wk->last) HIP_TRY(hipEventRecord(wk->last, st));
  ++h->launches;
  return ACNQP_OK;
}

}

int acnqp_solve_batch_device(acnqp_handle* h, const acnqp_problems* p, const acnqp_options* o, acnqp_results* r,
                             void* hip_stream) {
  return solve_batch_device(h, p, o, r, reinterpret_cast<hipStream_t>(hip_stream), true);
}

int32_t acnqp_accel_columns(acnqp_handle* h, int32_t t_max, int32_t k_sessions, int32_t precision, int32_t requested) {
  if (!h || t_max < 1 || k_sessions < 1 || requested <= 0) return 0;
  if (precision != 64) return 0;
  return std::min(requested, route_of(h, t_max, k_sessions, acnqp::kRouteAnyBatch).accel_cap<Kernels>());
}

static float event_pair_ms(acnqp_handle* h, long long launch) {
  const int k = (int)(launch % acnqp_handle::kEvRing);
  if (hipEventSynchronize(h->ev_stop[k]) != hipSuccess) return -1.0f;
  float ms = -1.0f;
  if (hipEventElapsedTime(&ms, h->ev_start[k], h->ev_stop[k]) != hipSuccess) return -1.0f;
  return ms;
}

int acnqp_set_long_polish(acnqp_handle* h, int32_t on) {
  if (!h) return fail(ACNQP_ERR_INVALID, "acnqp_set_long_polish: null handle");
  h->long_polish = on != 0;
  return ACNQP_OK;
}

int acnqp_set_wide_polish(acnqp_handle* h, int32_t on) {
  if (!h) return fail(ACNQP_ERR_INVALID, "acnqp_set_wide_polish: null handle");
  h->wide_polish = on != 0;
  return ACNQP_OK;
}

int64_t acnqp_launch_count(acnqp_handle* h) { return h ? (int64_t)h->launches : 0; }
int64_t acnqp_ordered_launch_count(acnqp_handle* h) { return h ? (int64_t)h->ordered_launches : 0; }

int acnqp_polish_stats(acnqp_handle* h, int64_t* out, int32_t capacity) {
  if (!h || !out || capacity < 1) return fail(ACNQP_ERR_INVALID, "acnqp_polish_stats: null argument");
  HIP_TRY(hipSetDevice(h->device));
  HIP_TRY(hipDeviceSynchronize());
  int32_t v[16] = {0};
  HIP_TRY(hipMemcpy(v, h->pol_stats, sizeof(v), hipMemcpyDeviceToHost));
  for (int k = 0; k < capacity && k < 16; ++k) out[k] = v[k];
  return ACNQP_OK;
}

extern "C" int64_t acnqp_debug_polish_alongside(acnqp_handle* h) {
  if (!h || hipSetDevice(h->device) != hipSuccess || hipDeviceSynchronize() != hipSuccess) return -1;
  int32_t v = 0;
  if (hipMemcpy(&v, h->pol_stats + 16, sizeof v, hipMemcpyDeviceToHost) != hipSuccess) return -1;
  if (hipMemset(h->pol_stats + 16, 0, sizeof v) != hipSuccess) return -1;
  return v;
}

extern "C" int64_t acnqp_debug_direct_x(acnqp_handle* h) { return h ? (int64_t)h->direct_x_last : -1; }

extern "C" int acnqp_debug_wave_rank(acnqp_handle* h, int32_t* out) {
  if (!h || !out) return -1;
  const int ext = wave_extent_of(h);
  out[0] = h->site.rank; out[1] = h->site.eig_ksteps; out[2] = ext > 0 ? ext : h->shape.MR / 4;
  return 0;
}

extern "C" int acnqp_debug_order_keys(acnqp_handle* h, const acnqp_problems* p, int32_t* keys_out) {
  if (!h || !p || !keys_out || p->batch < 0 || p->t_max < 1 || p->k_sessions < 1) return -1;
  if (p->batch == 0) return 0;
  if (!p->lb || !p->ub || !p->s_off || !p->s_len || !p->s_cap || !p->horizon) return -1;
  if (hipSetDevice(h->device) != hipSuccess) return -1;
  int32_t* keys = nullptr;
  if (hipMalloc((void**)&keys, (size_t)p->batch * sizeof(int32_t)) != hipSuccess) return -1;
  hipError_t e = launch_order_keys(h, route_of(h, p->t_max, p->k_sessions, p->batch), p, nullptr, keys);
  if (e == hipSuccess) e = hipMemcpy(keys_out, keys, (size_t)p->batch * sizeof(int32_t), hipMemcpyDeviceToHost);
  (void)hipFree(keys);
  return e == hipSuccess ? 0 : -1;
}

extern "C" int acnqp_debug_wave_evse_extent(acnqp_handle* h, int32_t* out) {
  if (!h || !out) return -1;
  out[0] = h->shape.N; out[1] = (h->shape.N + 3) / 4; out[2] = wave_evse_extent_of(h);
  return 0;
}

#ifdef ACNQP_DEBUG_WS
extern "C" int64_t acnqp_debug_copy_workspace(acnqp_handle* h, double* out, int64_t n_doubles) {
  if (!h || h->work.empty()) return -1;
  size_t best = 0;
  for (size_t k = 1; k < h->work.size(); ++k) if (h->work[k].used > h->work[best].used) best = k;
  (void)hipDeviceSynchronize();
  const int64_t have = (int64_t)(h->work[best].buf.cap / sizeof(double));
  const int64_t n = std::min(have, n_doubles);
  if (out && n > 0 && hipMemcpy(out, h->work[best].buf.p, (size_t)n * sizeof(double), hipMemcpyDeviceToHost) != hipSuccess) return -2;
  return have;
}
#endif

float acnqp_last_kernel_ms(acnqp_handle* h) {
  if (!h || h->launches == 0) return -1.0f;
  return event_pair_ms(h, h->launches - 1);
}

int32_t acnqp_kernel_times(acnqp_handle* h, float* out_ms, int32_t capacity) {
  if (!h || !out_ms || capacity <= 0) return 0;
  long long first = std::max(h->reported, h->launches - acnqp_handle::kEvRing);
  first = std::max(first, h->launches - (long long)capacity);
  int32_t n = 0;
  for (long long l = first; l < h->launches; ++l) out_ms[n++] = event_pair_ms(h, l);
  h->reported = h->launches;
  return n;
}

namespace {

int check_table(const acnqp_handle* h, const acnqp_table* t, const acnqp_options* o, const acnqp_results* r) {
  if (!h || !t || !o || !r) return fail(ACNQP_ERR_INVALID, "acnqp_solve_table: null argument");
  if (t->batch < 0) return fail(ACNQP_ERR_INVALID, "acnqp_solve_table: negative batch");
  if (t->batch == 0) return ACNQP_OK;
  if (!t->horizon || !t->q_index || !t->q_table || !t->pdiag || !t->s_eq || !t->sess_seg || !t->rate_seg ||
      (t->n_sessions > 0 && (!t->s_evse || !t->s_slot || !t->s_off || !t->s_len || !t->s_cap)))
    return fail(ACNQP_ERR_INVALID, "acnqp_solve_table: null table array");
  if (t->n_sessions < 0 || t->n_horizons < 1) return fail(ACNQP_ERR_INVALID, "acnqp_solve_table: bad n_sessions / n_horizons");
  static const double dummy_d = 0;
  static const int32_t dummy_i = 0;
  acnqp_problems p;
  p.batch = t->batch; p.t_max = t->t_max; p.k_sessions = t->k_sessions; p.horizon = t->horizon;
  p.lb = p.ub = p.q = p.s_cap = &dummy_d; p.pdiag = t->pdiag; p.s_off = p.s_len = &dummy_i; p.s_eq = t->s_eq;
  p.peak = t->peak; p.lf = t->lf; p.dc = t->dc; p.dfloor = t->dfloor; p.warm_x = p.warm_y = nullptr;
  const int rc = check_problem_shapes(h, &p, o, r);
  if (rc != ACNQP_OK) return rc;
  const int B = t->batch, S = t->n_sessions, N = h->shape.N, Tm = t->t_max, K = t->k_sessions;
  if (t->sess_seg[0] != 0 || t->sess_seg[B] != S) return fail(ACNQP_ERR_INVALID, "acnqp_solve_table: sess_seg must run from 0 to n_sessions");
  for (int b = 0; b < B; ++b) {
    if (t->sess_seg[b + 1] < t->sess_seg[b]) return fail(ACNQP_ERR_INVALID, "acnqp_solve_table: sess_seg is not non-decreasing");
    if (t->q_index[b] < 0 || t->q_index[b] >= t->n_horizons) return fail(ACNQP_ERR_INVALID, "acnqp_solve_table: q_index out of range");
    if (t->horizon[b] < 1 || t->horizon[b] > Tm) return fail(ACNQP_ERR_INVALID, "acnqp_solve_table: horizon out of range");
  }
  if (t->rate_seg[0] != 0) return fail(ACNQP_ERR_INVALID, "acnqp_solve_table: rate_seg must start at 0");
  for (int s_ = 0; s_ < S; ++s_) {
    const int len = t->s_len[s_] > 0 ? t->s_len[s_] : 0;
    if (t->s_evse[s_] < 0 || t->s_evse[s_] >= N || (len > 0 && (t->s_slot[s_] < 0 || t->s_slot[s_] >= K)))
      return fail(ACNQP_ERR_INVALID, "acnqp_solve_table: session " + std::to_string(s_) + ": EVSE or slot out of range");
    if (len > 0 && (t->s_off[s_] < 0 || t->s_off[s_] + len > Tm))
      return fail(ACNQP_ERR_INVALID, "acnqp_solve_table: session " + std::to_string(s_) + ": window outside [0, t_max)");
    if (t->rate_seg[s_ + 1] - t->rate_seg[s_] != len)
      return fail(ACNQP_ERR_INVALID, "acnqp_solve_table: session " + std::to_string(s_) +
                                     ": min_rates / max_rates must have one entry per remaining period (aco.py:68, 73)");
  }
  if (t->rate_seg[S] > 0 && (!t->min_rates || !t->max_rates)) return fail(ACNQP_ERR_INVALID, "acnqp_solve_table: null rate arrays");
  return ACNQP_OK;
}

}

int acnqp_solve_table(acnqp_handle* h, const acnqp_table* t, const acnqp_options* o, acnqp_results* r) {
  const auto tcheck0 = std::chrono::steady_clock::now();
  const int rc0 = check_table(h, t, o, r);
  if (rc0 != ACNQP_OK) return rc0;
  if (t->batch == 0) return ACNQP_OK;
  HIP_TRY(hipSetDevice(h->device));
  Call call;
  call.T = t; call.R = r;
  call.bs.push_back(BatchShape{t->batch, t->t_max, t->k_sessions, false, r->y != nullptr});
  const double check_ms = std::chrono::duration<double, std::milli>(std::chrono::steady_clock::now() - tcheck0).count();
  return solve_call(h, call, o, "acnqp_solve_table", check_ms);
}

int acnqp_solve_batches(acnqp_handle* h, int32_t n_batches, const acnqp_problems* p, const acnqp_options* o, acnqp_results* r) {
  if (!h || !p || !o || !r || n_batches < 0) return fail(ACNQP_ERR_INVALID, "acnqp_solve_batches: null argument or negative count");
  Call call;
  call.P = p; call.R = r;
  for (int g = 0; g < n_batches; ++g) {
    const int rc = check_problem_shapes(h, p + g, o, r + g);
    if (rc != ACNQP_OK) return rc;
    call.bs.push_back(BatchShape{p[g].batch, p[g].t_max, p[g].k_sessions, p[g].warm_x != nullptr, r[g].y != nullptr});
  }
  HIP_TRY(hipSetDevice(h->device));
  return solve_call(h, call, o, "acnqp_solve_batches", -1.0);
}

int acnqp_solve_batch(acnqp_handle* h, const acnqp_problems* p, const acnqp_options* o, acnqp_results* r) {
  return acnqp_solve_batches(h, 1, p, o, r);
}

void* acnqp_host_alloc(size_t bytes) {
  void* p = nullptr;
  if (hipHostMalloc(&p, bytes ? bytes : 16, hipHostMallocDefault) != hipSuccess) {
    (void)hipGetLastError();
    g_last_error = "acnqp_host_alloc: hipHostMalloc failed";
    return nullptr;
  }
  return p;
}

void acnqp_host_free(void* p) {
  if (p) (void)hipHostFree(p);
}

}
```

adacharge_amd/csrc/acn_qp_common.hpp:

```cpp
#pragma once
#include <hip/hip_runtime.h>
#include <stdint.h>

#include "acn_qp_check.hpp"

namespace acnqp {

#ifdef ACNQP_STAMPS
__device__ unsigned long long g_stamps[1024 * 16 * 12];
#define STAMP(slot)                                                                    \
  do {                                                                                 \
    unsigned long long _t;                                                             \
    __builtin_amdgcn_sched_barrier(0);                                                 \
    asm volatile("s_memtime %0\n\ts_waitcnt lgkmcnt(0)" : "=s"(_t)::"memory");         \
    __builtin_amdgcn_sched_barrier(0);                                                 \
    st_acc[slot] += _t - st_prev;                                                      \
    st_prev = _t;                                                                      \
  } while (0)
#else
#define STAMP(slot) do {} while (0)
#endif

#ifndef ACNQP_GUARD_MAX
#define ACNQP_GUARD_MAX 120
#endif

constexpr int kMaxK = 4;
struct TiledArgs {
  int B, N, Tm, K, NP, MR;
  const void *G, *Ghat, *Q, *lam, *rowlim;
  const int32_t* rowtype;
  const void *fragG, *fragQ;
  const void *fragG2, *fragQ2;
  const int32_t* horizon;
  const int32_t* order;
  int32_t* queue;
  const double *lb, *ub, *q, *pdiag;
  const int32_t *s_off, *s_len;
  const double* s_cap;
  const uint8_t* s_eq;
  const double* peak;
  const double* lf;
  const double *dc, *dfloor;
  const double *warm_x, *warm_y;
  const int32_t* rowabi;
  const void* rowscale;
  int Mg;
  double* x;
  double* y_out;
  int32_t *status, *iters;
  double *pri, *dua, *obj;
  double eps_abs, eps_rel, rho0, sigma, alpha, adapt_tol, reg_rel;
  double peak_scale, flat_scale, max_scale;
  int max_iter, check_every, adapt_every;
  int accel_mem;
  int stall_iters, retry_passes, retry_max_iter;
  double inacc_floor, retry_rho;
  int pbuf_single;
  int polish_iters, resume;
  int polish_stall;
  int y_for_polish_only;
  int pol_rows;
  int32_t *pol_list, *pol_count;
  int32_t* pol_retired;
  const int32_t* count_dev;
  double* const* x_host;
  int ws_by_slot;
  int grid_oversub;
  int grid_cap;
};

typedef const __attribute__((address_space(4))) TiledArgs* KernargPtr;

__device__ inline int queue_length(const TiledArgs& a) {
  if (a.count_dev == nullptr) return a.B;
  const int n = *a.count_dev;
  return n < a.B ? n : a.B;
}
__device__ inline int queue_next(int32_t* queue, int B, int round, int* slot_lds) {
  if (queue == nullptr) return round == 0 && (int)blockIdx.x < B ? (int)blockIdx.x : -1;
  if (threadIdx.x == 0) *slot_lds = atomicAdd(queue, 1);
  __syncthreads();
  const int pos = __builtin_amdgcn_readfirstlane(*slot_lds);
  __syncthreads();
  return pos < B ? pos : -1;
}

template <typename real> struct Mfma;
template <> struct Mfma<double> {
  typedef double vec4 __attribute__((ext_vector_type(4)));
  __host__ __device__ static constexpr int rowof(int g, int r) { return g + 4 * r; }
  __device__ static inline vec4 mma(double a, double b, vec4 c) { return __builtin_amdgcn_mfma_f64_16x16x4f64(a, b, c, 0, 0, 0); }
  static constexpr double proj_tol = 1e-13;
  static constexpr double big = 1e300;
};

template <int CTRL> __device__ inline float dpp_mov(float v) {
  return __builtin_bit_cast(float, __builtin_amdgcn_update_dpp(0, __builtin_bit_cast(int, v), CTRL, 0xF, 0xF, true));
}
template <int CTRL> __device__ inline double dpp_mov(double v) {
  const long long b = __builtin_bit_cast(long long, v);
  const int lo = __builtin_amdgcn_update_dpp(0, (int)(b & 0xffffffffll), CTRL, 0xF, 0xF, true);
  const int hi = __builtin_amdgcn_update_dpp(0, (int)(b >> 32), CTRL, 0xF, 0xF, true);
  return __builtin_bit_cast(double, ((long long)hi << 32) | (unsigned int)lo);
}
constexpr int kQuadXor1 = 0xB1, kQuadXor2 = 0x4E, kRowHalfMirror = 0x141, kRowMirror = 0x140;

template <typename T> __device__ inline T row_sum(T v) {
  v += dpp_mov<kQuadXor1>(v);
  v += dpp_mov<kQuadXor2>(v);
  v += dpp_mov<kRowHalfMirror>(v);
  v += dpp_mov<kRowMirror>(v);
  return v;
}
template <typename T> __device__ inline T row_min(T v) {
  v = fmin(v, dpp_mov<kQuadXor1>(v));
  v = fmin(v, dpp_mov<kQuadXor2>(v));
  v = fmin(v, dpp_mov<kRowHalfMirror>(v));
  v = fmin(v, dpp_mov<kRowMirror>(v));
  return v;
}
template <typename T> __device__ inline T row_max(T v) {
  v = fmax(v, dpp_mov<kQuadXor1>(v));
  v = fmax(v, dpp_mov<kQuadXor2>(v));
  v = fmax(v, dpp_mov<kRowHalfMirror>(v));
  v = fmax(v, dpp_mov<kRowMirror>(v));
  return v;
}

__device__ inline double uniform_scalar(double v) {
  const unsigned long long b = __builtin_bit_cast(unsigned long long, v);
  const unsigned lo = __builtin_amdgcn_readfirstlane((unsigned)b), hi = __builtin_amdgcn_readfirstlane((unsigned)(b >> 32));
  return __builtin_bit_cast(double, ((unsigned long long)hi << 32) | lo);
}
__device__ inline double scalar_const(double v) {
  const unsigned long long b = __builtin_bit_cast(unsigned long long, v);
  unsigned lo = (unsigned)b, hi = (unsigned)(b >> 32);
  asm volatile("" : "+s"(lo), "+s"(hi));
  return __builtin_bit_cast(double, ((unsigned long long)hi << 32) | lo);
}
__device__ inline double lane_value(double v, int src) {
  const unsigned long long b = __builtin_bit_cast(unsigned long long, v);
  const unsigned lo = __builtin_amdgcn_readlane((unsigned)b, src), hi = __builtin_amdgcn_readlane((unsigned)(b >> 32), src);
  return __builtin_bit_cast(double, ((unsigned long long)hi << 32) | lo);
}
struct ScalarConst { __device__ static inline double c(double v) { return scalar_const(v); } };
__device__ inline float uniform_scalar(float v) { return __builtin_bit_cast(float, __builtin_amdgcn_readfirstlane(__builtin_bit_cast(unsigned, v))); }

__device__ inline double rsqrt_nr(double x) {
  double y = __builtin_amdgcn_rsq(x);
  y = y * (1.5 - 0.5 * x * y * y);
  y = y * (1.5 - 0.5 * x * y * y);
  return y;
}
__device__ inline float rsqrt_nr(float x) {
  float y = __builtin_amdgcn_rsqf(x);
  y = y * (1.5f - 0.5f * x * y * y);
  return y;
}

__device__ inline double rcp_nr(double x) {
  double y = __builtin_amdgcn_rcp(x);
  y = y + y * (1.0 - x * y);
  y = y + y * (1.0 - x * y);
  return y;
}
__device__ inline float rcp_nr(float x) {
  float y = __builtin_amdgcn_rcpf(x);
  y = y + y * (1.0f - x * y);
  return y;
}

__device__ inline double rcp_small(float nf) {
  const double x = (double)nf;
  double y = (double)__builtin_amdgcn_rcpf(nf);
  y = y + y * (1.0 - x * y);
  y = y + y * (1.0 - x * y);
  return y;
}

constexpr double kStartGain = 1e5;
constexpr double kRegResolve = 1e-6;
template <typename real>
__host__ __device__ inline real effective_pdiag(real pd_user, real reg_rel, real qnorm, real ubmax, int horizon, bool has_prox) {
  if (has_prox || !(ubmax > (real)0) || pd_user * ubmax > (real)kRegResolve * qnorm) return pd_user;
  const real fl = reg_rel * qnorm / (ubmax * (real)(horizon > 1 ? horizon : 1));
  return fl > pd_user ? fl : pd_user;
}
constexpr double kInaccurate = 100.0;
template <typename real>
__host__ __device__ inline bool inaccurate_ok(real pri, real dua, real npri, real ndua, double eps_abs, double eps_rel, double floor_) {
  const real ea = (real)(kInaccurate * eps_abs > floor_ ? kInaccurate * eps_abs : floor_);
  const real er = (real)(kInaccurate * eps_rel > floor_ ? kInaccurate * eps_rel : floor_);
  return pri <= ea + er * npri && dua <= ea + er * ndua;
}
__host__ __device__ inline int retry_min_iters(int stall_iters) { return stall_iters > 0 ? stall_iters : 3000; }
__host__ __device__ inline int status_rank(int st) { return st == 1 ? 3 : (st == 5 ? 2 : (st == 2 ? 1 : 0)); }
__host__ __device__ inline bool retry_wanted(int pass, int retry_passes, int status, int it, int stall_iters, int adapt_every0) {
  return pass < retry_passes && (status == 2 || status == 5) && it >= retry_min_iters(stall_iters) && adapt_every0 > 0;
}
constexpr int kAaPeriod = 5;
constexpr double kAaReg = 1e-4, kAaSafe = 1.2, kAaDrift = 1e-3;

typedef unsigned int u32x2 __attribute__((ext_vector_type(2)));
struct Pair32 { unsigned a, b; };
struct PairF { float a, b; };
struct PairD { double a, b; };
template <int WHICH> __device__ inline Pair32 swap_u32(unsigned v) {
  const u32x2 r = WHICH == 16 ? __builtin_amdgcn_permlane16_swap(v, v, false, false)
                              : __builtin_amdgcn_permlane32_swap(v, v, false, false);
  return {r[0], r[1]};
}
template <int WHICH> __device__ inline PairF swap_pair(float v) {
  const Pair32 p = swap_u32<WHICH>(__builtin_bit_cast(unsigned, v));
  return {__builtin_bit_cast(float, p.a), __builtin_bit_cast(float, p.b)};
}
template <int WHICH> __device__ inline PairD swap_pair(double v) {
  const unsigned long long bits = __builtin_bit_cast(unsigned long long, v);
  const Pair32 lo = swap_u32<WHICH>((unsigned)(bits & 0xffffffffull));
  const Pair32 hi = swap_u32<WHICH>((unsigned)(bits >> 32));
  return {__builtin_bit_cast(double, ((unsigned long long)hi.a << 32) | lo.a),
          __builtin_bit_cast(double, ((unsigned long long)hi.b << 32) | lo.b)};
}
template <typename T> __device__ inline T quarter_sum(T v) {
  auto p = swap_pair<16>(v); v = p.a + p.b;
  auto q = swap_pair<32>(v); return q.a + q.b;
}
template <typename T> __device__ inline T quarter_min(T v) {
  auto p = swap_pair<16>(v); v = fmin(p.a, p.b);
  auto q = swap_pair<32>(v); return fmin(q.a, q.b);
}
template <typename T> __device__ inline T quarter_max(T v) {
  auto p = swap_pair<16>(v); v = fmax(p.a, p.b);
  auto q = swap_pair<32>(v); return fmax(q.a, q.b);
}

template <typename T> __device__ inline T wave_max(T v) { return quarter_max<T>(row_max<T>(v)); }
template <typename T> __device__ inline T wave_sum(T v) { return quarter_sum<T>(row_sum<T>(v)); }

}
```

adacharge_amd/csrc/acn_qp_pipeline.hpp:

```cpp
#pragma once
#include <algorithm>
#include <cstddef>
#include <cstdint>
#include <cstdlib>
#include <vector>

#include "acn_qp.h"

namespace {
struct TableExpandArgs {
  int N, Tm, K;
  long long s_base, r_base;
  const int32_t *q_index, *sess_seg, *s_evse, *s_slot, *s_off, *s_len, *rate_seg;
  const double *q_table, *s_cap, *min_rates, *max_rates;
  double *lb, *ub, *q, *sc;
  int32_t *so, *sl;
};
}

namespace acnqp {

inline size_t al256(size_t b) { return (b + 255) & ~(size_t)255; }

struct ChunkShape { size_t N, Tm, K, Mg; bool peak, flat, max, warm, want_y, direct; };
enum class Per : uint8_t { One, NT, KN, T, MgT };
enum class When : uint8_t { Always, Peak, Flat, Max, Warm, WantY, Direct };
enum class Size : uint8_t { Large, Small };
constexpr size_t kNoField = ~(size_t)0;
struct ArrayRow { size_t field; uint8_t elem; Per per; When when; Size size; };

enum In { kLb, kUb, kQ, kPd, kHz, kSo, kSl, kSc, kEq, kPk, kLf, kDc, kDf, kXh, kWx, kWy, kInRows };
enum Out { kX, kSt, kIt, kPr, kDu, kOb, kY, kOutRows };
constexpr ArrayRow kIn[kInRows] = {
    {offsetof(acnqp_problems, lb), 8, Per::NT, When::Always, Size::Large},
    {offsetof(acnqp_problems, ub), 8, Per::NT, When::Always, Size::Large},
    {offsetof(acnqp_problems, q), 8, Per::NT, When::Always, Size::Large},
    {offsetof(acnqp_problems, pdiag), 8, Per::One, When::Always, Size::Small},
    {offsetof(acnqp_problems, horizon), 4, Per::One, When::Always, Size::Small},
    {offsetof(acnqp_problems, s_off), 4, Per::KN, When::Always, Size::Small},
    {offsetof(acnqp_problems, s_len), 4, Per::KN, When::Always, Size::Small},
    {offsetof(acnqp_problems, s_cap), 8, Per::KN, When::Always, Size::Small},
    {offsetof(acnqp_problems, s_eq), 1, Per::One, When::Always, Size::Small},
    {offsetof(acnqp_problems, peak), 8, Per::T, When::Peak, Size::Small},
    {offsetof(acnqp_problems, lf), 8, Per::One, When::Flat, Size::Small},
    {offsetof(acnqp_problems, dc), 8, Per::One, When::Max, Size::Small},
    {offsetof(acnqp_problems, dfloor), 8, Per::One, When::Max, Size::Small},
    {kNoField, sizeof(double*), Per::One, When::Direct, Size::Small},
    {offsetof(acnqp_problems, warm_x), 8, Per::NT, When::Warm, Size::Large},
    {offsetof(acnqp_problems, warm_y), 8, Per::MgT, When::Warm, Size::Large},
};
constexpr ArrayRow kOut[kOutRows] = {
    {offsetof(acnqp_results, x), 8, Per::NT, When::Always, Size::Large},
    {offsetof(acnqp_results, status), 4, Per::One, When::Always, Size::Small},
    {offsetof(acnqp_results, iters), 4, Per::One, When::Always, Size::Small},
    {offsetof(acnqp_results, pri_res), 8, Per::One, When::Always, Size::Small},
    {offsetof(acnqp_results, dua_res), 8, Per::One, When::Always, Size::Small},
    {offsetof(acnqp_results, obj), 8, Per::One, When::Always, Size::Small},
    {offsetof(acnqp_results, y), 8, Per::MgT, When::WantY, Size::Large},
};

constexpr bool present(const ArrayRow& r, const ChunkShape& s) {
  const bool on[] = {true, s.peak, s.flat, s.max, s.warm, s.want_y, s.direct};
  return on[(int)r.when];
}
constexpr size_t bytes_per_problem(const ArrayRow& r, const ChunkShape& s) {
  const size_t n[] = {1, s.N * s.Tm, s.K * s.N, s.Tm, s.Mg * s.Tm};
  return r.elem * n[(int)r.per];
}
struct RowRange { int first, end; };
constexpr RowRange small_rows(const ArrayRow* rows, int n) {
  int first = 0, end = 0;
  while (first < n && rows[first].size != Size::Small) ++first;
  for (end = first; end < n && rows[end].size == Size::Small;) ++end;
  for (int k = end; k < n; ++k)
    if (rows[k].size == Size::Small) return {n, n};
  return {first, end};
}
constexpr RowRange kSmallIn = small_rows(kIn, kInRows), kSmallOut = small_rows(kOut, kOutRows);
static_assert(kSmallIn.first < kSmallIn.end && kSmallOut.first < kSmallOut.end, "the small rows of a side are one contiguous run: the pinned mirror is one copy");

struct ChunkLayout {
  ChunkShape shape;
  size_t cn, in[kInRows + 1], out[kOutRows + 1];
  bool direct;
  ChunkLayout(size_t cn_, const ChunkShape& s) : shape(s), cn(cn_), direct(s.direct) {
    auto lay = [&](const ArrayRow* rows, int n, size_t* off) {
      off[0] = 0;
      for (int k = 0; k < n; ++k) off[k + 1] = off[k] + al256(present(rows[k], s) ? cn * bytes_per_problem(rows[k], s) : 0);
    };
    lay(kIn, kInRows, in);
    lay(kOut, kOutRows, out);
  }
  size_t mirror_in() const { return in[kSmallIn.first]; }
  size_t mirror_in_bytes() const { return in[kSmallIn.end] - in[kSmallIn.first]; }
  size_t mirror_out() const { return out[kSmallOut.first]; }
  size_t mirror_out_bytes() const { return out[kSmallOut.end] - out[kSmallOut.first]; }
};

struct TableSpan { long long lo = 0, cn = 0, s0 = 0, ns = 0, r0 = 0, nr = 0; size_t qt = 0; };
enum class Count : uint8_t { Cn, Cn1, Ns, Ns1, Nr, Qt };
enum class Base : uint8_t { Lo, S0, R0, Zero };
struct TableRow { size_t field, arg; uint8_t elem; Count count; Base base; };
#define ACNQP_T(f) offsetof(acnqp_table, f), offsetof(TableExpandArgs, f)
constexpr TableRow kTable[] = {
    {ACNQP_T(q_index), 4, Count::Cn, Base::Lo},
    {ACNQP_T(sess_seg), 4, Count::Cn1, Base::Lo},
    {ACNQP_T(s_evse), 4, Count::Ns, Base::S0},
    {ACNQP_T(s_slot), 4, Count::Ns, Base::S0},
    {ACNQP_T(s_off), 4, Count::Ns, Base::S0},
    {ACNQP_T(s_len), 4, Count::Ns, Base::S0},
    {ACNQP_T(rate_seg), 4, Count::Ns1, Base::S0},
    {ACNQP_T(s_cap), 8, Count::Ns, Base::S0},
    {ACNQP_T(min_rates), 8, Count::Nr, Base::R0},
    {ACNQP_T(max_rates), 8, Count::Nr, Base::R0},
    {ACNQP_T(q_table), 8, Count::Qt, Base::Zero},
};
#undef ACNQP_T
constexpr int kTableRows = (int)(sizeof(kTable) / sizeof(kTable[0]));
constexpr size_t table_count(const TableRow& r, const TableSpan& s) {
  const size_t n[] = {(size_t)s.cn, (size_t)s.cn + 1, (size_t)s.ns, (size_t)s.ns + 1, (size_t)s.nr, s.qt};
  return n[(int)r.count];
}
constexpr size_t table_base(const TableRow& r, const TableSpan& s) {
  const long long at[] = {s.lo, s.s0, s.r0, 0};
  return (size_t)at[(int)r.base];
}
struct TableLayout {
  TableSpan span;
  size_t off[kTableRows] = {}, total = 0;
  TableLayout() = default;
  explicit TableLayout(const TableSpan& s) : span(s) {
    for (int k = 0; k < kTableRows; ++k) { off[k] = total; total += al256(table_count(kTable[k], s) * kTable[k].elem); }
  }
};

struct PlanEnv {
  long long chunk = 0;
  const char* plan = nullptr;
  bool ramp = true;
  bool direct = false;
};

inline long long chunk_cap_by_memory(size_t N, size_t Tm, size_t K) {
  const size_t per_problem = 4 * N * Tm * 8 + K * N * 16 + Tm * 8 + 96;
  return (long long)((size_t)1024 * 1024 * 1024 / std::max<size_t>(per_problem, 1));
}

inline std::vector<long long> plan_chunk_caps(long long total, long long want, long long by_mem, bool wave, bool uniform,
                                              const PlanEnv& env) {
  if (env.chunk > 0) want = env.chunk;
  long long cap = std::max<long long>(1, std::min(want, by_mem));
  if (cap >= 512) cap -= cap % 512;
  std::vector<long long> caps;
  if (env.ramp && wave && uniform) {
    if (env.plan) {
      for (const char* q = env.plan; *q;) { caps.push_back(std::max<long long>(1, std::atoll(q))); while (*q && *q != ',') ++q; if (*q == ',') ++q; }
    } else if (env.direct && total >= 2048 && cap >= 2048) {
      long long m = 1, u = 0;
      for (;; ++m) {
        u = (total + 4 + 3 * m) / (5 + 3 * m);
        if (3 * u <= cap) break;
      }
      const long long f = total - 3 * u * m;
      caps.push_back(std::max<long long>(1, f / 5));
      caps.push_back(std::max<long long>(1, 2 * f / 5));
      caps.push_back(std::max<long long>(1, f - f / 5 - 2 * f / 5));
      for (long long i = 0; i < m; ++i) caps.push_back(3 * u);
    } else if (total >= 2048 && cap >= 2048) {
      const long long k = (total + cap - 1) / cap - 1;
      long long c = total / (k + 1);
      c = std::max<long long>(2048, std::min(cap, c - c % 512));
      caps.push_back(c / 4);
      caps.push_back(c / 2);
      for (long long i = 0; i < k; ++i) caps.push_back(c);
    }
    caps.push_back(std::max<long long>(1, total));
  } else if (env.ramp && cap >= 1024) {
    caps = {cap / 4, cap / 2, cap};
  } else {
    caps = {cap};
  }
  return caps;
}
inline long long chunk_cap(const std::vector<long long>& caps, size_t c) { return caps[std::min(c, caps.size() - 1)]; }

}

#ifdef __HIPCC__
#include <hip/hip_runtime.h>

#include <chrono>
#include <cstdio>
#include <cstring>
#include <string>

#include "acn_qp.h"
#include "acn_qp_route.hpp"

namespace {

using namespace acnqp;

constexpr int kOrderKeys = 1024;
constexpr int kOrderMinBatch = 768;
constexpr size_t kOrderLdsPerProblem = (size_t)64 << 10;
constexpr size_t kOrderLdsPerGroup = (size_t)160 << 10;
inline int order_key_waves(size_t N, size_t Tm, size_t g_rows) {
  const size_t sched = N * Tm * sizeof(double), g = g_rows * N * sizeof(double);
  if (sched == 0 || sched > kOrderLdsPerProblem || g + sched > kOrderLdsPerGroup) return 0;
  return (int)std::min<size_t>(4, (kOrderLdsPerGroup - g) / sched);
}

__global__ __launch_bounds__(256) void session_keys_kernel(const int32_t* s_len, int KN, int B, int32_t* keys) {
  const int wave = threadIdx.x >> 6, lane = threadIdx.x & 63;
  const int b = blockIdx.x * 4 + wave;
  if (b >= B) return;
  int c = 0;
  for (int k = lane; k < KN; k += 64) c += s_len[(size_t)b * KN + k] > 0 ? 1 : 0;
  for (int o = 32; o > 0; o >>= 1) c += __shfl_xor(c, o);
  if (lane == 0) keys[b] = c < kOrderKeys ? c : kOrderKeys - 1;
}

struct OrderKeyArgs {
  int B, N, Tm, K, M, soc, has_peak;
  const double *lb, *ub, *s_cap, *peak, *G, *limits;
  const int32_t *s_off, *s_len, *horizon;
  int32_t* keys;
};

__global__ __launch_bounds__(256) void order_keys_kernel(const OrderKeyArgs a) {
  extern __shared__ __attribute__((aligned(16))) unsigned char order_lds[];
  const int wave = threadIdx.x >> 6, lane = threadIdx.x & 63;
  const int N = a.N, Tm = a.Tm, M = a.M;
  const int g_rows = a.soc ? 2 * M : M;
  double* Gs = reinterpret_cast<double*>(order_lds);
  double* x0 = Gs + (size_t)g_rows * N + (size_t)wave * N * Tm;
  const int b = blockIdx.x * (int)(blockDim.x >> 6) + wave;
  const bool live = b < a.B;
  for (int k = threadIdx.x; k < g_rows * N; k += blockDim.x) Gs[k] = a.G[k];
  if (live)
    for (int k = lane; k < N * Tm; k += 64) x0[k] = 0.0;
  __syncthreads();
  int sessions = 0;
  if (live) {
    const int hz = min(a.horizon[b], Tm);
    const size_t sb = (size_t)b * a.K * N, vb = (size_t)b * N * Tm;
    for (int k = lane; k < a.K * N; k += 64) {
      const int len = a.s_len[sb + k];
      if (len <= 0) continue;
      ++sessions;
      const int i = k % N, off = a.s_off[sb + k];
      const int t0 = max(off, 0), t1 = (int)min((long long)off + len, (long long)hz);
      double rem = a.s_cap[sb + k];
      for (int t = t0; t < t1; ++t) {
        const double d = fmax(a.lb[vb + (size_t)i * Tm + t], fmin(a.ub[vb + (size_t)i * Tm + t], fmax(rem, 0.0)));
        x0[i * Tm + t] = d;
        rem -= d;
      }
    }
  }
  __syncthreads();
  int over = 0;
  if (live) {
    const int cells = (M + (a.has_peak && a.peak ? 1 : 0)) * Tm;
    for (int c = lane; c < cells; c += 64) {
      const int j = c / Tm, t = c - j * Tm;
      double load, limit;
      if (j < M) {
        double re = 0.0, im = 0.0;
        for (int i = 0; i < N; ++i) re += Gs[j * N + i] * x0[i * Tm + t];
        if (a.soc)
          for (int i = 0; i < N; ++i) im += Gs[(j + M) * N + i] * x0[i * Tm + t];
        load = a.soc ? hypot(re, im) : re;
        limit = a.limits[j];
      } else {
        load = 0.0;
        for (int i = 0; i < N; ++i) load += x0[i * Tm + t];
        limit = a.peak[(size_t)b * Tm + t];
      }
      over += (limit > 0.0 ? load > (1.0 + 1e-9) * limit : limit == 0.0 && load > 0.0) ? 1 : 0;
    }
  }
  for (int o = 32; o > 0; o >>= 1) { over += __shfl_xor(over, o); sessions += __shfl_xor(sessions, o); }
  if (live && lane == 0) a.keys[b] = min(kOrderKeys - 1, 8 * min(over, 127) + min(7, sessions / 8));
}
__global__ __launch_bounds__(kOrderKeys) void order_sort_kernel(const int32_t* keys, int B, int32_t* order) {
  __shared__ int hist[kOrderKeys], scan[kOrderKeys];
  const int tid = threadIdx.x;
  hist[tid] = 0;
  __syncthreads();
  for (int b = tid; b < B; b += kOrderKeys) atomicAdd(&hist[keys[b]], 1);
  __syncthreads();
  scan[tid] = hist[kOrderKeys - 1 - tid];
  __syncthreads();
  for (int o = 1; o < kOrderKeys; o <<= 1) {
    const int v = tid >= o ? scan[tid - o] : 0;
    __syncthreads();
    scan[tid] += v;
    __syncthreads();
  }
  hist[kOrderKeys - 1 - tid] = scan[tid] - hist[kOrderKeys - 1 - tid];
  __syncthreads();
  for (int b = tid; b < B; b += kOrderKeys) order[atomicAdd(&hist[keys[b]], 1)] = b;
}

__global__ __launch_bounds__(256) void table_expand_kernel(const TableExpandArgs a) {
  const int b = blockIdx.x, tid = threadIdx.x;
  const size_t nv = (size_t)a.N * a.Tm, ns = (size_t)a.K * a.N;
  double *lb = a.lb + b * nv, *ub = a.ub + b * nv, *q = a.q + b * nv;
  const double* qt = a.q_table + (size_t)a.q_index[b] * nv;
  for (size_t k = tid; k < nv; k += 256) { lb[k] = 0.0; ub[k] = 0.0; q[k] = qt[k]; }
  for (size_t k = tid; k < ns; k += 256) { a.so[b * ns + k] = 0; a.sl[b * ns + k] = 0; a.sc[b * ns + k] = 0.0; }
  __syncthreads();
  const int wave = tid >> 6, lane = tid & 63;
  const long long s0 = a.sess_seg[b] - a.s_base, s1 = a.sess_seg[b + 1] - a.s_base;
  for (long long s = s0 + wave; s < s1; s += 4) {
    const int ev = a.s_evse[s], off = a.s_off[s], len = a.s_len[s];
    const long long r0 = a.rate_seg[s] - a.r_base;
    for (int p_ = lane; p_ < len; p_ += 64) {
      const double lo = a.min_rates[r0 + p_], hi = a.max_rates[r0 + p_];
      lb[(size_t)ev * a.Tm + off + p_] = lo;
      ub[(size_t)ev * a.Tm + off + p_] = hi < lo ? lo : hi;
    }
    if (lane == 0 && len > 0) {
      const size_t k = (size_t)b * ns + (size_t)a.s_slot[s] * a.N + ev;
      a.so[k] = off; a.sl[k] = len; a.sc[k] = a.s_cap[s];
    }
  }
}

struct BatchShape { long long batch; int t_max, k_sessions; bool warm, want_y; };
struct Piece { int g; long long lo, n, pos; };
struct Scatter { Piece pc; size_t c; const char* host; };

struct Call {
  const acnqp_problems* P = nullptr;
  const acnqp_table* T = nullptr;
  acnqp_results* R = nullptr;
  std::vector<BatchShape> bs;
  std::vector<ChunkLayout> layout;
  std::vector<Scatter> scatter;
  std::vector<double*> xdst;
};

double* direct_destination(const double* x) {
  static const bool off = std::getenv("ACNQP_NO_DIRECT_X") != nullptr;
  if (off || x == nullptr) return nullptr;
  hipPointerAttribute_t at;
  if (hipPointerGetAttributes(&at, x) != hipSuccess) {
    (void)hipGetLastError();
    return nullptr;
  }
  return at.type == hipMemoryTypeHost ? static_cast<double*>(at.devicePointer) : nullptr;
}

inline char* member(const void* s, size_t field) { char* p; std::memcpy(&p, static_cast<const char*>(s) + field, sizeof p); return p; }
inline void set_member(void* s, size_t field, const void* p) { std::memcpy(static_cast<char*>(s) + field, &p, sizeof p); }

void device_views(const ChunkLayout& L, char* di, char* dq, const BatchShape& b, acnqp_problems* dp, acnqp_results* dr) {
  dp->batch = (int32_t)L.cn; dp->t_max = b.t_max; dp->k_sessions = b.k_sessions;
  for (int k = 0; k < kInRows; ++k)
    if (kIn[k].field != kNoField) set_member(dp, kIn[k].field, present(kIn[k], L.shape) ? di + L.in[k] : nullptr);
  for (int k = 0; k < kOutRows; ++k) set_member(dr, kOut[k].field, present(kOut[k], L.shape) ? dq + L.out[k] : nullptr);
  dr->x_dev = nullptr;
}

std::vector<std::vector<Piece>> split_call(const acnqp_handle* h, const std::vector<BatchShape>& bs, const acnqp::PlanEnv& env) {
  long long total = 0;
  bool uniform = true;
  for (const BatchShape& b : bs) {
    total += b.batch;
    uniform = uniform && b.t_max == bs[0].t_max && b.k_sessions == bs[0].k_sessions && b.warm == bs[0].warm && b.want_y == bs[0].want_y;
  }
  std::vector<std::vector<Piece>> chunks;
  std::vector<long long> caps;
  long long fill = 0, cap = 0;
  const BatchShape* cur = nullptr;
  for (int g = 0; g < (int)bs.size(); ++g) {
    const BatchShape& b = bs[g];
    for (long long lo = 0; lo < b.batch;) {
      if (!cur || b.t_max != cur->t_max || b.k_sessions != cur->k_sessions || b.warm != cur->warm || b.want_y != cur->want_y || fill >= cap) {
        chunks.emplace_back();
        cur = &b; fill = 0;
        if (caps.empty() || !uniform) {
          const acnqp::Route rt = acnqp::route_for(h->shape, b.t_max, b.k_sessions, (int)std::min<long long>(total, acnqp::kRouteAnyBatch), route_switches());
          acnqp::PlanEnv e = env;
          e.direct = env.direct && rt.direct_x();
          caps = acnqp::plan_chunk_caps(total, rt.chunk_want(), acnqp::chunk_cap_by_memory((size_t)h->shape.N, (size_t)b.t_max, (size_t)b.k_sessions),
                                        rt.wv > 0, uniform, e);
        }
        cap = acnqp::chunk_cap(caps, chunks.size() - 1);
      }
      const long long n = std::min(b.batch - lo, cap - fill);
      chunks.back().push_back({g, lo, n, fill});
      fill += n; lo += n;
    }
  }
  return chunks;
}

hipError_t upload_piece(const ChunkLayout& L, const acnqp_problems& src, size_t lo, size_t n, size_t pos, char* di, char* hs, hipStream_t st) {
  hipError_t e = hipSuccess;
  for (int k = 0; k < kInRows && e == hipSuccess; ++k) {
    const char* from = kIn[k].field != kNoField && present(kIn[k], L.shape) ? member(&src, kIn[k].field) : nullptr;
    if (!from) continue;
    const size_t per = bytes_per_problem(kIn[k], L.shape);
    if (hs && kIn[k].size == Size::Small) std::memcpy(hs + L.in[k] + pos * per, from + lo * per, n * per);
    else e = hipMemcpyAsync(di + L.in[k] + pos * per, from + lo * per, n * per, hipMemcpyHostToDevice, st);
  }
  return e;
}

int fill_dense(acnqp_handle* h, const Call& call, size_t c, const std::vector<Piece>& pcs, const ChunkLayout& L,
               acnqp_handle::Slot& S, char* hs) {
  char* di = static_cast<char*>(S.in.p);
  static const bool chain = std::getenv("ACNQP_NO_H2D_CHAIN") == nullptr;
  if (chain && c > 0) HIP_TRY(hipStreamWaitEvent(S.st, h->h2d_done[(c - 1) % acnqp_handle::kSlots], 0));
  for (const Piece& pc : pcs) {
    const size_t lo = (size_t)pc.lo, n = (size_t)pc.n, pos = (size_t)pc.pos;
    HIP_TRY(upload_piece(L, call.P[pc.g], lo, n, pos, di, hs, S.st));
    if (hs && L.direct) {
      double** tab = reinterpret_cast<double**>(hs + L.in[kXh]) + pos;
      double* const dst = call.xdst[pc.g];
      for (size_t i = 0; i < n; ++i) tab[i] = dst ? dst + (lo + i) * L.shape.N * L.shape.Tm : nullptr;
    }
  }
  if (hs) HIP_TRY(hipMemcpyAsync(di + L.mirror_in(), hs + L.mirror_in(), L.mirror_in_bytes(), hipMemcpyHostToDevice, S.st));
  if (chain) HIP_TRY(hipEventRecord(h->h2d_done[c % acnqp_handle::kSlots], S.st));
  return ACNQP_OK;
}

TableSpan table_span(const acnqp_table* T, long long lo, long long cn, size_t nv) {
  const long long s0 = T->sess_seg[lo], ns = T->sess_seg[lo + cn] - s0, r0 = T->rate_seg[s0], nr = T->rate_seg[s0 + ns] - r0;
  return TableSpan{lo, cn, s0, ns, r0, nr, (size_t)T->n_horizons * nv};
}

int fill_table(const Call& call, const Piece& pc, const ChunkLayout& L, const TableLayout& TL, acnqp_handle::Slot& S) {
  const acnqp_table* T = call.T;
  char* di = static_cast<char*>(S.in.p);
  char* dt = static_cast<char*>(S.tin.p);
  acnqp_problems src = {};
  src.horizon = T->horizon; src.pdiag = T->pdiag; src.s_eq = T->s_eq; src.peak = T->peak; src.lf = T->lf; src.dc = T->dc; src.dfloor = T->dfloor;
  HIP_TRY(upload_piece(L, src, (size_t)pc.lo, (size_t)pc.n, 0, di, nullptr, S.st));
  TableExpandArgs ea;
  for (int k = 0; k < kTableRows; ++k) {
    const TableRow& r = kTable[k];
    const size_t bytes = table_count(r, TL.span) * r.elem;
    if (bytes > 0) HIP_TRY(hipMemcpyAsync(dt + TL.off[k], member(T, r.field) + table_base(r, TL.span) * r.elem, bytes, hipMemcpyHostToDevice, S.st));
    set_member(&ea, r.arg, dt + TL.off[k]);
  }
  ea.N = (int)L.shape.N; ea.Tm = (int)L.shape.Tm; ea.K = (int)L.shape.K; ea.s_base = TL.span.s0; ea.r_base = TL.span.r0;
  ea.lb = reinterpret_cast<double*>(di + L.in[kLb]); ea.ub = reinterpret_cast<double*>(di + L.in[kUb]); ea.q = reinterpret_cast<double*>(di + L.in[kQ]);
  ea.so = reinterpret_cast<int32_t*>(di + L.in[kSo]); ea.sl = reinterpret_cast<int32_t*>(di + L.in[kSl]); ea.sc = reinterpret_cast<double*>(di + L.in[kSc]);
  hipLaunchKernelGGL(table_expand_kernel, dim3((unsigned)pc.n), dim3(256), 0, S.st, ea);
  return ACNQP_OK;
}

int run_call(acnqp_handle* h, Call& call, const acnqp_options* o) {
  const acnqp::SiteShape& s = h->shape;
  const size_t N = s.N, Mg = s.Mg;
  const bool table = call.T != nullptr;
  acnqp::PlanEnv env;
  if (const char* e = std::getenv("ACNQP_CHUNK")) env.chunk = std::atoll(e);
  env.plan = std::getenv("ACNQP_PLAN");
  static const bool ramp = std::getenv("ACNQP_NO_RAMP") == nullptr;
  env.ramp = ramp;
  h->direct_x_last = 0;
  call.xdst.assign(call.bs.size(), nullptr);
  env.direct = !table && !call.bs.empty();
  for (size_t g = 0; g < call.bs.size() && !table; ++g) {
    call.xdst[g] = call.bs[g].batch > 0 ? direct_destination(call.R[g].x) : nullptr;
    env.direct = env.direct && (call.xdst[g] != nullptr || call.bs[g].batch == 0);
  }
  const std::vector<std::vector<Piece>> chunks = split_call(h, call.bs, env);
  std::vector<char> direct(chunks.size(), 0);
  for (size_t c = 0; c < chunks.size() && !table; ++c) {
    const std::vector<Piece>& pcs = chunks[c];
    const BatchShape& b = call.bs[pcs[0].g];
    if (!route_of(h, b.t_max, b.k_sessions, (int)(pcs.back().pos + pcs.back().n)).direct_x()) continue;
    for (const Piece& pc : pcs) direct[c] = direct[c] || call.xdst[pc.g] != nullptr;
  }
  auto layout = [&](size_t c) {
    const std::vector<Piece>& pcs = chunks[c];
    const BatchShape& b = call.bs[pcs[0].g];
    return ChunkLayout((size_t)(pcs.back().pos + pcs.back().n),
                       ChunkShape{N, (size_t)b.t_max, (size_t)b.k_sessions, Mg, s.has_peak != 0, s.has_flat != 0, s.has_max != 0, b.warm, b.want_y, direct[c] != 0});
  };
  constexpr size_t kSmallCap = (size_t)256 << 20;
  std::vector<size_t> in_off(chunks.size()), out_off(chunks.size());
  size_t in_sum = 0, out_sum = 0;
  for (size_t c = 0; c < chunks.size() && !table; ++c) {
    const ChunkLayout L = layout(c);
    in_off[c] = in_sum; in_sum += L.mirror_in_bytes();
    out_off[c] = out_sum; out_sum += L.mirror_out_bytes();
  }
  static const bool no_stage = std::getenv("ACNQP_NO_STAGING") != nullptr;
  const bool staged = !table && !no_stage && in_sum + out_sum <= kSmallCap;
  if (staged) {
    HIP_TRY(h->small_in.reserve(in_sum));
    HIP_TRY(h->small_out.reserve(out_sum));
  } else {
    std::fill(direct.begin(), direct.end(), 0);
  }
  for (size_t c = 0; c < chunks.size(); ++c) {
    acnqp_handle::Slot& S = h->slot[c % acnqp_handle::kSlots];
    const std::vector<Piece>& pcs = chunks[c];
    const BatchShape& b = call.bs[pcs[0].g];
    call.layout.push_back(layout(c));
    const ChunkLayout& L = call.layout.back();
    const TableLayout TL = table ? TableLayout(table_span(call.T, pcs[0].lo, pcs[0].n, N * L.shape.Tm)) : TableLayout();
    HIP_TRY(reserve_behind(S.st, {{&S.in, L.in[kInRows]}, {&S.out, L.out[kOutRows]}, {&S.tin, TL.total}}));
    char* di = static_cast<char*>(S.in.p);
    char* dq = static_cast<char*>(S.out.p);
    char* hs = staged ? static_cast<char*>(h->small_in.p) + in_off[c] - L.mirror_in() : nullptr;
    char* ho = staged ? static_cast<char*>(h->small_out.p) + out_off[c] - L.mirror_out() : nullptr;
    int rc = table ? fill_table(call, pcs[0], L, TL, S) : fill_dense(h, call, c, pcs, L, S, hs);
    if (rc != ACNQP_OK) return rc;
    acnqp_problems dp;
    acnqp_results dr;
    device_views(L, di, dq, b, &dp, &dr);
    double* const* x_host = L.direct ? reinterpret_cast<double* const*>(di + L.in[kXh]) : nullptr;
    rc = solve_batch_device(h, &dp, o, &dr, S.st, c + 1 == chunks.size(), x_host);
    if (rc != ACNQP_OK) return rc;
    if (staged) HIP_TRY(hipMemcpyAsync(ho + L.mirror_out(), dq + L.mirror_out(), L.mirror_out_bytes(), hipMemcpyDeviceToHost, S.st));
    for (const Piece& pc : pcs) {
      const acnqp_results& r = call.R[pc.g];
      const size_t lo = (size_t)pc.lo, n = (size_t)pc.n, pos = (size_t)pc.pos;
      const bool stored = L.direct && call.xdst[pc.g];
      if (stored) h->direct_x_last += (long long)n;
      for (int k = 0; k < kOutRows; ++k) {
        if (!present(kOut[k], L.shape) || (k == kX && stored) || (staged && kOut[k].size == Size::Small)) continue;
        const size_t per = bytes_per_problem(kOut[k], L.shape);
        HIP_TRY(hipMemcpyAsync(member(&r, kOut[k].field) + lo * per, dq + L.out[k] + pos * per, n * per, hipMemcpyDeviceToHost, S.st));
      }
      if (staged) call.scatter.push_back(Scatter{pc, c, ho});
      if (r.x_dev) {
        const size_t per = bytes_per_problem(kOut[kX], L.shape);
        HIP_TRY(hipMemcpyAsync(reinterpret_cast<char*>(r.x_dev) + lo * per, dq + L.out[kX] + pos * per, n * per, hipMemcpyDeviceToDevice, S.st));
      }
    }
  }
  return ACNQP_OK;
}

int solve_call(acnqp_handle* h, Call& call, const acnqp_options* o, const char* who, double check_ms) {
  using clock = std::chrono::steady_clock;
  auto ms = [](clock::time_point a, clock::time_point b) { return std::chrono::duration<double, std::milli>(b - a).count(); };
  static const bool trace = std::getenv("ACNQP_TRACE") != nullptr;
  const auto t0 = clock::now();
  const int rc = run_call(h, call, o);
  const auto t1 = clock::now();
  hipError_t e = hipSuccess;
  for (auto& sl : h->slot) { const hipError_t e1 = hipStreamSynchronize(sl.st); if (e == hipSuccess) e = e1; }
  if (trace) {
    const auto t2 = clock::now();
    if (check_ms >= 0) std::fprintf(stderr, "[acnqp] %s: check %.3f ms, enqueue %.3f ms, drained after %.3f ms\n", who + 6, check_ms, ms(t0, t1), ms(t0, t2));
    else std::fprintf(stderr, "[acnqp] %s: enqueue %.3f ms, drained after %.3f ms\n", who + 6, ms(t0, t1), ms(t0, t2));
  }
  if (rc != ACNQP_OK) return rc;
  if (e != hipSuccess) return fail(ACNQP_ERR_HIP, std::string(who) + ": " + hipGetErrorString(e));
  for (const Scatter& sc : call.scatter) {
    const ChunkLayout& L = call.layout[sc.c];
    for (int k = kSmallOut.first; k < kSmallOut.end; ++k) {
      const size_t per = bytes_per_problem(kOut[k], L.shape);
      std::memcpy(member(&call.R[sc.pc.g], kOut[k].field) + (size_t)sc.pc.lo * per, sc.host + L.out[k] + (size_t)sc.pc.pos * per, (size_t)sc.pc.n * per);
    }
  }
  for (size_t g = 0; g < call.bs.size(); ++g)
    for (long long b = 0; b < call.bs[g].batch; ++b)
      if (call.R[g].status[b] == ACNQP_STATUS_UNSET)
        return fail(ACNQP_ERR_HIP, std::string(who) + ": " + (call.T ? "" : "batch " + std::to_string(g) + " ") + "problem " + std::to_string(b) +
                                   " was never written by the kernel (status UNSET after synchronisation): the launch did not execute completely");
  return ACNQP_OK;
}

}
#endif
```

adacharge_amd/csrc/acn_qp_route.hpp:

```cpp
#pragma once
#include <algorithm>

#include "acn_qp.h"

namespace acnqp {

constexpr int kRouteMaxK = 4;
constexpr int kRouteWaveTS = 12;

inline int padded_rows(int cone, int M, int has_peak, int has_flat, int has_max) {
  return (cone == ACNQP_CONE_SOC ? 8 * ((M + 3) / 4) : M) + (has_peak ? 1 : 0) + (has_flat ? 1 : 0) + (has_max ? 1 : 0);
}

struct SiteShape {
  int N = 0, M = 0, Mg = 0, MR = 0;
  int cone = 0, has_peak = 0, has_flat = 0, has_max = 0;
  int NP() const { return N <= 64 ? 64 : 16 * ((N + 15) / 16); }
};

inline SiteShape site_shape(int N, int M, int cone, int has_peak, int has_flat, int has_max) {
  SiteShape s;
  s.N = N; s.M = M; s.cone = cone;
  s.has_peak = has_peak ? 1 : 0; s.has_flat = has_flat ? 1 : 0; s.has_max = has_max ? 1 : 0;
  s.Mg = (cone == ACNQP_CONE_SOC ? 2 * M : M) + s.has_peak + s.has_flat + s.has_max;
  s.MR = 16 * std::max(1, (padded_rows(cone, M, has_peak, has_flat, has_max) + 15) / 16);
  return s;
}

struct RouteSwitches {
  bool no_wave = false;
  bool no_wave2 = false;
  int wave_min_batch = 1;
  bool no_long = false;
  bool lds_long = true;
};

inline int wave_shape(const SiteShape& s, int t_max, int k_sessions, int batch, const RouteSwitches& sw) {
  constexpr int TS = kRouteWaveTS;
  const bool off2 = sw.no_wave2;
  if (sw.no_wave || s.N > 64 || k_sessions != 1 || batch < sw.wave_min_batch) return 0;
  if (s.MR == 16 && t_max <= TS) return 1;
  if (s.MR == 16 && t_max <= 2 * TS) return off2 ? 0 : 2;
  if (s.MR == 16 && t_max > 32 && t_max <= 4 * TS) return off2 ? 0 : 5;
  if (s.MR == 32 && t_max <= TS) return off2 ? 0 : 3;
  if (s.MR == 32 && t_max <= 2 * TS) return off2 ? 0 : 4;
  return 0;
}

inline bool tiled_shape(const SiteShape& s, int t_max, int k_sessions) {
  if (t_max > 16 && s.MR > 16) return false;
  return s.N <= 64 && t_max <= 32 && k_sessions <= kRouteMaxK;
}
inline bool lds_long_shape(const SiteShape& s, int t_max, const RouteSwitches& sw) {
  return sw.lds_long && s.N <= 64 && t_max > 16 && t_max <= 32 && !s.has_max && s.MR == 32;
}
inline bool stream_shape(const SiteShape& s, int t_max) { return s.N > 64 && t_max <= 48; }
inline bool long_shape(const SiteShape& s, int t_max, int k_sessions, const RouteSwitches& sw) {
  return !sw.no_long && !tiled_shape(s, t_max, k_sessions) && !stream_shape(s, t_max) && t_max <= 288 && s.MR <= 32;
}

struct Route {
  int family = 0;
  int wv = 0;
  bool tiled = false, stream = false, lng = false, lds = false, on_chip = false;
  bool polish_shape = false;
  bool polish_long_shape = false;
  bool polish_wide_shape = false;
  SiteShape site;
  int t_max = 0, k_sessions = 0;

  long long chunk_want() const { return wv > 0 ? 8192 : (tiled ? 1024 : 2048); }

  bool direct_x() const { return wv == 1; }

  template <class Kn> int accel_cap() const {
    if (wv > 0) return Kn::wave_accel();
    if (tiled) return Kn::tiled_accel(site.MR / 16, (t_max + 15) / 16, site.NP(), k_sessions);
    if (stream) return Kn::stream_accel();
    if (lng) return Kn::long_accel();
    return Kn::general_accel();
  }

  template <class Kn> long long workspace_doubles(int accel_req) const {
    if (tiled) return 0;
    const int accel = std::min(std::max(0, accel_req), accel_cap<Kn>());
    if (stream) return Kn::stream_workspace(site.NP(), (t_max + 15) / 16, k_sessions, site.MR / 16, accel);
    if (lng) return Kn::long_workspace(site.NP(), t_max, k_sessions, site.MR / 16, accel);
    const long long n = (long long)site.N * t_max, mt = (long long)site.MR * t_max, Dn = n + mt;
    return 7 * n + 8 * mt + 3LL * k_sessions * site.N + 8 + 2 * Dn + ((1 + 2LL * accel) * Dn * 4 + 7) / 8 + 2;
  }
};

inline Route route_for(const SiteShape& s, int t_max, int k_sessions, int batch, const RouteSwitches& sw) {
  Route r;
  r.site = s; r.t_max = t_max; r.k_sessions = k_sessions;
  r.wv = wave_shape(s, t_max, k_sessions, batch, sw);
  r.tiled = r.wv > 0 || tiled_shape(s, t_max, k_sessions);
  r.stream = !r.tiled && stream_shape(s, t_max);
  r.lng = !r.tiled && long_shape(s, t_max, k_sessions, sw);
  r.lds = r.lng && lds_long_shape(s, t_max, sw);
  r.on_chip = r.tiled || r.lds;
  if (r.wv > 0) r.family = r.wv;
  else if (r.tiled) r.family = t_max <= 16 ? ACNQP_ROUTE_TILED_CT1 : ACNQP_ROUTE_TILED_CT2;
  else if (r.stream) r.family = ACNQP_ROUTE_STREAM;
  else if (r.lng) r.family = r.lds ? ACNQP_ROUTE_LONG_LDS : ACNQP_ROUTE_LONG_WS;
  else r.family = ACNQP_ROUTE_GENERAL;
  r.polish_shape = r.on_chip && s.N <= 64 && t_max <= 32 && k_sessions <= kRouteMaxK && !s.has_flat && !s.has_max &&
                   s.M + s.has_peak > 0;
  r.polish_long_shape = s.N <= 64 && t_max > 32 && t_max <= 288 && k_sessions <= kRouteMaxK && !s.has_flat && !s.has_max &&
                        s.M + s.has_peak > 0 && (r.family == ACNQP_ROUTE_WAVE5 || r.family == ACNQP_ROUTE_LONG_WS);
  r.polish_wide_shape = r.family == ACNQP_ROUTE_STREAM && s.N > 64 && s.N <= 1024 && t_max <= 48 && k_sessions <= kRouteMaxK &&
                        8 * ((s.N * k_sessions + 7) / 8) <= 1024 && s.Mg <= 48 && !s.has_flat && !s.has_max && s.M + s.has_peak > 0;
  return r;
}

constexpr int kRouteAnyBatch = 1 << 30;

}
```

adacharge_amd/csrc/acn_qp_wave.hip:

```cpp
#include "acn_qp_launch.hpp"
#include "acn_qp_rank.hpp"
#include "acn_qp_wave.hpp"

#ifndef ACNQP_WAVE_NE
#define ACNQP_WAVE_NE 0
#endif

namespace acnqp {

static_assert(ACNQP_WAVE_NE == 0 || ACNQP_WAVE_NE == kWaveEvseExtent, "the EVSE extents instantiated: 14 k-steps and all 16");

static_assert(kRouteWaveTS == kWaveTS, "acn_qp_route.hpp restates the period slots per lane");

template <int NPW, int TSV, int MT, bool PROX, int EK, int NE = ACNQP_WAVE_NE>
static hipError_t launch_wave_prox(const TiledArgs& a_in, const WaveSite& ws, hipStream_t st) {
  TiledArgs a = a_in;
  if (EK > 0) { a.Ghat = ws.Ghat; a.lam = ws.lam; a.fragQ = ws.fragQ; }
  a.accel_mem = std::min(a.accel_mem, kWaveAM);
  const WaveLds L(a.accel_mem, NPW, MT, TSV);
  const size_t lds = (size_t)L.total * 8;
  auto kern = &admm_wave_kernel<kWaveAM, NPW, TSV, MT, PROX, EK, NE>;
  if (lds > 64 * 1024) {
    hipError_t e = ensure_dynamic_lds(reinterpret_cast<const void*>(kern), lds);
    if (e != hipSuccess) return e;
  }
  constexpr int per_wg = kWaveNW / NPW;
  const int groups = (a.B + per_wg - 1) / per_wg;
  int grid = groups;
  if (a.queue) {
    const int per_cu = resident_per_cu(reinterpret_cast<const void*>(kern), kWaveNW * 64, lds), cus = device_cus();
    const int cap = a.grid_cap > 0 ? a.grid_cap : groups;
    int resident = per_cu * cus;
    static const int grid_env = std::getenv("ACNQP_WAVE_GRID") ? std::atoi(std::getenv("ACNQP_WAVE_GRID")) : 0;
    if (a.grid_oversub > 1 && grid_env > 0) resident = grid_env;
    grid = std::max(1, std::min(std::min(groups, cap), resident));
  }
  hipLaunchKernelGGL(kern, dim3(grid), dim3(kWaveNW * 64), lds, st, a);
  return hipGetLastError();
}

template <int NPW, int TSV, int MT, int EK>
static hipError_t launch_wave_ek(const TiledArgs& a, const WaveSite& ws, hipStream_t st) {
  return a.lf != nullptr || a.dc != nullptr ? launch_wave_prox<NPW, TSV, MT, true, EK>(a, ws, st) : launch_wave_prox<NPW, TSV, MT, false, EK>(a, ws, st);
}
template <int NPW, int TSV, int MT>
static hipError_t launch_wave_npw(const TiledArgs& a, const WaveSite& ws, hipStream_t st) {
  if (ws.extent == kWaveExtentSmall) return launch_wave_ek<NPW, TSV, MT, kWaveExtentSmall>(a, ws, st);
  if (ws.extent == kWaveExtentMid) return launch_wave_ek<NPW, TSV, MT, kWaveExtentMid>(a, ws, st);
  return launch_wave_ek<NPW, TSV, MT, 0>(a, ws, st);
}

template <int = 0>
static hipError_t launch_wave_shape(const TiledArgs& a, const WaveSite& ws, hipStream_t st) {
  if (a.MR == 32) return a.Tm <= kWaveTS ? launch_wave_npw<2, 6, 2>(a, ws, st) : launch_wave_npw<4, 6, 2>(a, ws, st);
  if (a.Tm > 2 * kWaveTS) return launch_wave_npw<4, 12, 1>(a, ws, st);
  return a.Tm <= kWaveTS ? launch_wave_npw<1, 12, 1>(a, ws, st) : launch_wave_npw<2, 12, 1>(a, ws, st);
}

#if ACNQP_WAVE_NE == 0
int wave_accel_columns() { return kWaveAM; }

hipError_t launch_wave(const TiledArgs& a, const WaveSite& ws, hipStream_t st) {
  if (ws.evse_ksteps == kWaveEvseExtent && a.N <= 4 * kWaveEvseExtent) return launch_wave_e14(a, ws, st);
  return launch_wave_shape(a, ws, st);
}
#else
hipError_t launch_wave_e14(const TiledArgs& a, const WaveSite& ws, hipStream_t st) { return launch_wave_shape(a, ws, st); }
#endif

}

#if defined(ACNQP_STAMPS) && ACNQP_WAVE_NE == 0
extern "C" int acnqp_debug_read_wave_stamps(unsigned long long* out, int n) {
  return (int)hipMemcpyFromSymbol(out, HIP_SYMBOL(acnqp::g_stamps), sizeof(unsigned long long) * n);
}
#endif
```

adacharge_amd/csrc/acn_qp_wave.hpp:

```cpp
#pragma once
#include <type_traits>

#include "acn_qp_common.hpp"

namespace acnqp {

constexpr int kWaveTS = 12;
constexpr int kWaveXS = 17;
constexpr int kWaveNW = 4;
constexpr int kWaveAM = 5;

struct WaveLds {
  int fragp, fragx, fragq, rowc, wave0, wstride;
  int xt, rowd, aah, snap, hist, total;
  int xch;
  int xs;
  __host__ __device__ WaveLds(int accel_mem, int npw = 1, int mt = 1, int tsv = kWaveTS) {
    int o = 0;
    fragp = o; o += mt * 16 * 64;
    fragx = o; o += 4 * 4 * mt * 64;
    fragq = o; o += mt * mt * 2 * 4 * 64;
    rowc = o;  o += mt * (16 + 16 + 8);
    wave0 = o;
    int w = 0;
    xs = tsv > 8 ? kWaveXS : 9;
    xt = w;   w += 64 * xs;
    rowd = w; w += 16 * mt;
    aah = w;  w += kWaveAM * kWaveAM + kWaveAM + 1;
    w = (w + 1) & ~1;
    snap = w; xch = w;
    w += npw >= 2 ? 2 * 2 * 64 + 2 : 64 * 16 / 2;
    w = (w + 1) & ~1;
    hist = w; w += accel_mem * 64 * 16 / 2;
    wstride = (w + 1) & ~1;
    total = wave0 + kWaveNW * wstride;
  }
};

__device__ inline int wave_queue_next(int32_t* queue, int B, int round, int wave, int lane) {
  if (queue == nullptr) {
    const int pos = (int)blockIdx.x * kWaveNW + wave;
    return round == 0 && pos < B ? pos : -1;
  }
  int v = 0;
  if (lane == 0) v = atomicAdd(queue, 1);
  const int pos = __builtin_amdgcn_readfirstlane(v);
  return pos < B ? pos : -1;
}

__device__ inline void wave_lds_sync() {
  __builtin_amdgcn_fence(__ATOMIC_RELEASE, "wavefront");
  __builtin_amdgcn_wave_barrier();
  __builtin_amdgcn_fence(__ATOMIC_ACQUIRE, "wavefront");
}

__device__ __attribute__((always_inline)) inline void wave_x_to_host(const double* xt, int xs, int n, int Tm, double* dst) {
  const int lane = threadIdx.x & 63;
  int row = lane / Tm, col = lane - row * Tm;
  const int drow = 64 / Tm, dcol = 64 - drow * Tm;
  for (int k = lane; k < n; k += 64) {
    dst[k] = xt != nullptr ? xt[row * xs + col] : 0.0;
    row += drow; col += dcol;
    if (col >= Tm) { col -= Tm; ++row; }
  }
}

template <int AM, int NPW, int TSV, int MT, bool PROX, int EK = 0, int NE = 0>
__global__ __launch_bounds__(kWaveNW * 64, 1) void admm_wave_kernel(const TiledArgs A_kernarg) {
  static_assert(NPW == 1 || NPW == 2 || NPW == 4, "one, two or four waves per problem");
  static_assert((TSV == 12 && MT == 1) || (TSV == 6 && MT == 2 && NPW >= 2), "instantiated: 12 periods x one row tile, 6 periods x two row tiles");
  using M = Mfma<double>;
  using vec4 = typename M::vec4;
  typedef double real;
  constexpr int TS = TSV, XS = TSV > 8 ? kWaveXS : 9, XC = TSV > 8 ? 16 : 8;
  constexpr int SR = 4 * MT, KS = 4 * MT;
  constexpr int EKS = EK > 0 ? EK : KS, ET = (EKS + 3) / 4;
  static_assert(EKS <= KS, "eigen extent");
  constexpr int NKS = NE > 0 ? NE : 16;
  static_assert(NKS <= 16, "EVSE extent");
#define EKOF(m) (EKS - 4 * (m) < 4 ? EKS - 4 * (m) : 4)
#define BIGC (scalar_const(1e300))
  extern __shared__ __attribute__((aligned(16))) unsigned char smem_raw[];
  real* sm = reinterpret_cast<real*>(smem_raw);
  const int tid0 = threadIdx.x;
  const int lane = tid0 & 63, wave = __builtin_amdgcn_readfirstlane(tid0 >> 6);
  const int g = lane >> 4, tc = lane & 15;
  const int half = wave & (NPW - 1);
  const int tb = TSV * half;
  int xseq = 0;
  bool xbroken = false;

  {
    const WaveLds L0(0, NPW, MT, TSV);
    const int NP = A_kernarg.NP;
    const real* Gh = static_cast<const real*>(A_kernarg.Ghat);
    const real* FQg = static_cast<const real*>(A_kernarg.fragQ);
    for (int k = tid0; k < MT * 16 * 64; k += kWaveNW * 64) {
      const int m = k >> 10, s = (k >> 6) & 15, l = k & 63, gg = l >> 4, tt = l & 15;
      sm[L0.fragp + k] = Gh[(size_t)(16 * m + tt) * NP + 4 * s + gg];
    }
    for (int k = tid0; k < 4 * KS * 64; k += kWaveNW * 64) {
      const int ws = k >> 6, l = k & 63, gg = l >> 4, tt = l & 15;
      const int w = ws / KS, s = ws % KS;
      sm[L0.fragx + k] = Gh[(size_t)(16 * (s >> 2) + 4 * (s & 3) + gg) * NP + 16 * w + tt];
    }
    for (int k = tid0; k < MT * MT * 2 * 4 * 64; k += kWaveNW * 64) sm[L0.fragq + k] = FQg[k];
    if (tid0 < 16 * MT) {
      sm[L0.rowc + tid0] = static_cast<const real*>(A_kernarg.lam)[tid0];
      sm[L0.rowc + 16 * MT + tid0] = static_cast<const real*>(A_kernarg.rowlim)[tid0];
      const int m_ = tid0 >> 4, g_ = (tid0 >> 2) & 3, r_ = tid0 & 3;
      reinterpret_cast<int*>(sm + L0.rowc + 32 * MT)[tid0] = A_kernarg.rowtype[16 * m_ + M::rowof(g_, r_)];
    }
    const WaveLds L1(min(A_kernarg.accel_mem, AM), NPW, MT, TSV);
    real* XT0 = sm + L1.wave0 + (size_t)wave * L1.wstride;
    for (int k = lane; k < 64 * XS; k += 64) XT0[k] = 0;
    if (NPW >= 2 && lane < 2) reinterpret_cast<int*>(XT0 + L1.xch + 2 * 2 * 64)[lane] = 0;
  }
  __syncthreads();

  real* Xm = nullptr;
  const real* Xg = nullptr;
  int xstride = 0;
  if constexpr (NPW >= 2) {
    const WaveLds Lx(min(A_kernarg.accel_mem, AM), NPW, MT, TSV);
    Xm = sm + Lx.wave0 + (size_t)wave * Lx.wstride + Lx.xch;
    Xg = sm + Lx.wave0 + (size_t)(wave & ~(NPW - 1)) * Lx.wstride + Lx.xch;
    xstride = Lx.wstride;
  }
  auto grp_xchg = [&](real va, real vb, real (&pa)[NPW], real (&pb)[NPW]) __attribute__((always_inline)) {
    if constexpr (NPW >= 2) {
      ++xseq;
      const int o = (xseq & 1) * 128;
      Xm[o + lane] = va;
      Xm[o + 64 + lane] = vb;
      __builtin_amdgcn_fence(__ATOMIC_RELEASE, "wavefront");
      if (lane == 0) *reinterpret_cast<volatile int*>(Xm + 256) = xseq;
#pragma unroll
      for (int k = 0; k < NPW; ++k) {
        const real* Xk = Xg + (size_t)k * xstride;
        if (!xbroken) {
          int spins = 0;
          while (*reinterpret_cast<const volatile int*>(Xk + 256) - xseq < 0) {
            if (++spins > 64) __builtin_amdgcn_s_sleep(1);
            if (spins > (1 << 22)) { xbroken = true; break; }
          }
        }
        __builtin_amdgcn_fence(__ATOMIC_ACQUIRE, "wavefront");
        pa[k] = Xk[o + lane];
        pb[k] = Xk[o + 64 + lane];
      }
    } else {
      pa[0] = va; pb[0] = vb;
    }
  };
  auto pl_sum2 = [&](real& va, real& vb) __attribute__((always_inline)) {
    if constexpr (NPW >= 2) {
      real pa[NPW], pb[NPW];
      grp_xchg(va, vb, pa, pb);
      va = pa[0]; vb = pb[0];
#pragma unroll
      for (int k = 1; k < NPW; ++k) { va += pa[k]; vb += pb[k]; }
    }
  };
  auto pl_minmax = [&](real& lo_, real& hi_) __attribute__((always_inline)) {
    if constexpr (NPW >= 2) {
      real pa[NPW], pb[NPW];
      grp_xchg(lo_, hi_, pa, pb);
#pragma unroll
      for (int k = 0; k < NPW; ++k) { lo_ = fmin(lo_, pa[k]); hi_ = fmax(hi_, pb[k]); }
    }
  };
  auto pu_sum = [&](real* d, int n) __attribute__((always_inline)) {
    if constexpr (NPW >= 2) {
      real v = 0, pa[NPW], pb[NPW];
#pragma unroll
      for (int j = 0; j < 8; ++j) if (j < n) v = lane == j ? d[j] : v;
      grp_xchg(v, 0.0, pa, pb);
#pragma unroll
      for (int j = 0; j < 8; ++j)
        if (j < n) {
          real t_ = lane_value(pa[0], j);
#pragma unroll
          for (int k = 1; k < NPW; ++k) t_ += lane_value(pa[k], j);
          d[j] = t_;
        }
    }
  };
  auto pu_max = [&](real* d, int n) __attribute__((always_inline)) {
    if constexpr (NPW >= 2) {
      real v = 0, pa[NPW], pb[NPW];
#pragma unroll
      for (int j = 0; j < 8; ++j) if (j < n) v = lane == j ? d[j] : v;
      grp_xchg(v, 0.0, pa, pb);
#pragma unroll
      for (int j = 0; j < 8; ++j)
        if (j < n) {
#pragma unroll
          for (int k = 0; k < NPW; ++k) d[j] = fmax(d[j], lane_value(pa[k], j));
        }
    }
  };

  int q_round = 0;
  for (;; ++q_round) {
  int q_pos;
  if constexpr (NPW >= 2) {
    int mine = 0;
    if (half == 0) {
      if (A_kernarg.queue == nullptr) {
        const int pos = (int)blockIdx.x * (kWaveNW / NPW) + wave / NPW;
        mine = q_round == 0 && pos < queue_length(A_kernarg) ? pos : -1;
      } else {
        mine = wave_queue_next(A_kernarg.queue, queue_length(A_kernarg), q_round, wave, lane);
      }
    }
    real pa[NPW], pb[NPW];
    grp_xchg((real)mine, 0.0, pa, pb);
    q_pos = __builtin_amdgcn_readfirstlane((int)pa[0]);
  } else {
    q_pos = wave_queue_next(A_kernarg.queue, queue_length(A_kernarg), q_round, wave, lane);
  }
  if (q_pos < 0) break;
  int it_total = 0, best_status = 0;
  for (int pass = 0;; ++pass) {
  int b_ = q_pos;
  asm volatile("" : "+v"(b_));
  const int wg_ = __builtin_amdgcn_readfirstlane(b_);
  KernargPtr Ap = (KernargPtr)__builtin_amdgcn_kernarg_segment_ptr();
  asm volatile("" : "+s"(Ap));
  const auto& A = *Ap;
  const int b = __builtin_amdgcn_readfirstlane(A.order ? A.order[wg_] : wg_);
  if (A.resume) {
    if (A.status[b] != kStatusPolish && pass == 0) break;
    if (pass == 0) it_total = A.iters[b];
  }
  const int max_iter_p = pass == 0 ? A.max_iter : min(A.max_iter, A.retry_max_iter);
  const int adapt_p = pass == 0 ? A.adapt_every : 0;
  const int N = A.N, Tm = A.Tm;
  const int aa_m = min(A.accel_mem, AM);
  const WaveLds L(aa_m, NPW, MT, TSV);
  const real* FragP = sm + L.fragp;
  const real* FragX = sm + L.fragx;
  const real* FQs = sm + L.fragq;
  const real* RowLam = sm + L.rowc;
  const real* RowLim = RowLam + 16 * MT;
  const int* RowTy = reinterpret_cast<const int*>(RowLam + 32 * MT);
  real* Wv = sm + L.wave0 + (size_t)wave * L.wstride;
  real* XT = Wv + L.xt;
  real* RowDj = Wv + L.rowd;
  real* AaH = Wv + L.aah;
  float* Snap = reinterpret_cast<float*>(Wv + L.snap);
  float* HistF = reinterpret_cast<float*>(Wv + L.hist);
  const real* Gm = static_cast<const real*>(A.G);
  auto row_types = [&](int m, int (&ty)[4]) __attribute__((always_inline)) {
    const int4 v = *reinterpret_cast<const int4*>(RowTy + (m * 4 + g) * 4);
    ty[0] = v.x; ty[1] = v.y; ty[2] = v.z; ty[3] = v.w;
  };

  auto evse_to_rows = [&](const real (&v)[TS], const real* frag, vec4 (&out)[MT]) __attribute__((always_inline)) {
    __builtin_amdgcn_wave_barrier();
#pragma unroll
    for (int t = 0; t < TS; ++t) XT[lane * XS + t] = v[t];
    wave_lds_sync();
    real bop[NKS];
#pragma unroll
    for (int s = 0; s < NKS; ++s) {
      if constexpr (XC == 16) bop[s] = XT[(4 * s + g) * XS + tc];
      else bop[s] = tc < XC ? XT[(4 * s + g) * XS + (tc < XC ? tc : 0)] : 0.0;
    }
#pragma unroll
    for (int m = 0; m < ET; ++m) {
      real aop[NKS];
#pragma unroll
      for (int s = 0; s < NKS; ++s) aop[s] = frag[(m * 16 + s) * 64 + lane];
      vec4 acc0 = {0, 0, 0, 0}, acc1 = {0, 0, 0, 0};
#pragma unroll
      for (int s = 0; s < NKS; ++s) {
        if ((s & 1) == 0) acc0 = M::mma(aop[s], bop[s], acc0);
        else acc1 = M::mma(aop[s], bop[s], acc1);
      }
      out[m] = acc0 + acc1;
    }
  };
  auto rows_to_evse = [&](const vec4 (&c4)[MT], auto&& bfrag, real (&out)[TS], auto kn) __attribute__((always_inline)) {
    constexpr int KN = decltype(kn)::value;
    real bf[4][KN];
#pragma unroll
    for (int w = 0; w < 4; ++w)
#pragma unroll
      for (int s = 0; s < KN; ++s) bf[w][s] = bfrag(w, s);
    vec4 acc[4];
#pragma unroll
    for (int w = 0; w < 4; ++w) acc[w] = vec4{0, 0, 0, 0};
#pragma unroll
    for (int s = 0; s < KN; ++s)
#pragma unroll
      for (int w = 0; w < 4; ++w) acc[w] = M::mma(c4[s >> 2][s & 3], bf[w][s], acc[w]);
    __builtin_amdgcn_wave_barrier();
#pragma unroll
    for (int w = 0; w < 4; ++w)
#pragma unroll
      for (int r = 0; r < 3; ++r) {
        if constexpr (TS >= 12) XT[(16 * w + tc) * XS + g + 4 * r] = acc[w][r];
        else if (4 * r < TS) { if (g + 4 * r < TS) XT[(16 * w + tc) * XS + g + 4 * r] = acc[w][r]; }
      }
    wave_lds_sync();
#pragma unroll
    for (int t = 0; t < TS; ++t) out[t] = XT[lane * XS + t];
  };
  auto frag_ghat = [&](int w, int s) __attribute__((always_inline)) -> real { return FragX[(w * KS + s) * 64 + lane]; };
  constexpr std::integral_constant<int, KS> all_rows{};
  constexpr std::integral_constant<int, EKS> live_eigen{};
  auto frag_g = [&](int w, int s) __attribute__((always_inline)) -> real { return Gm[(size_t)(16 * (s >> 2) + 4 * (s & 3) + g) * A.NP + 16 * w + tc]; };

  const bool act = lane < N;
  real x[TS], z1[TS], y1[TS], qv[TS], lbv[TS], ubv[TS];
#pragma unroll
  for (int t = 0; t < TS; ++t) {
    const bool ok = act && tb + t < Tm;
    const size_t idx = ((size_t)b * N + (ok ? lane : 0)) * Tm + (ok ? tb + t : 0);
    lbv[t] = ok ? A.lb[idx] : 0.0;
    ubv[t] = ok ? A.ub[idx] : 0.0;
    qv[t] = ok ? A.q[idx] : 0.0;
    if (ubv[t] < lbv[t]) ubv[t] = lbv[t];
    x[t] = 0; z1[t] = 0; y1[t] = 0;
  }
  const bool eq = A.s_eq[b] != 0;
  unsigned swm = 0;
  int smode = 4;
  real scap = 0, mu = 0;
  unsigned imask = 0;
  bool empty_set = false;
  {
    const size_t sidx = (size_t)b * N + (act ? lane : 0);
    const int off = act ? A.s_off[sidx] : 0;
    const int len = act ? A.s_len[sidx] : 0;
    real sl = 0, su = 0;
#pragma unroll
    for (int t = 0; t < TS; ++t)
      if (tb + t >= off && tb + t < off + len && tb + t < Tm) { swm |= 1u << t; sl += lbv[t]; su += ubv[t]; }
    pl_sum2(sl, su);
    scap = act ? A.s_cap[sidx] : 0.0;
    if (len > 0) {
      smode = 0;
      const real slack = 64.0 * M::proj_tol * fmax(1.0, fabs(scap));
      if (sl > scap + slack) empty_set = true;
      if (eq && su < scap - slack) empty_set = true;
      if (eq && scap >= su) smode = 2;
      else if (scap <= sl) smode = 3;
    }
  }
  real pk_lane = BIGC;
  if (A.peak && tc < TS && tb + tc < Tm) {
    const double pv = A.peak[(size_t)b * Tm + tb + tc];
    pk_lane = pv < 1e300 ? pv * A.peak_scale : BIGC;
  }

  const real pd_user = uniform_scalar(A.pdiag[b]);
  const real lfb = PROX ? uniform_scalar(A.lf ? A.lf[b] / (A.flat_scale * A.flat_scale) : 0.0) : 0.0;
  const real dcb = PROX ? uniform_scalar(A.dc ? A.dc[b] / A.max_scale : 0.0) : 0.0;
  const real dfl = PROX ? uniform_scalar(A.dfloor ? A.dfloor[b] * A.max_scale : 0.0) : 0.0;
  real tau_max = 0;
  const real sigma = A.sigma, alpha = A.alpha;
  real rho = A.rho0;
  if (pass > 0) {
    rho = A.retry_rho;
    for (int k = 1; k < pass; ++k) rho *= 4.0;
  }
  real qnorm, pd;
  bool plain_windows;
  {
    real f1 = 0, f2 = 0, f3 = 0;
#pragma unroll
    for (int t = 0; t < TS; ++t) {
      f1 = fmax(f1, fabs(qv[t]));
      f2 = fmax(f2, ubv[t]);
      if (!((swm >> t) & 1u)) f3 = fmax(f3, fmax(fabs(lbv[t]), fabs(ubv[t])));
    }
    f1 = wave_max<real>(f1); f2 = wave_max<real>(f2); f3 = wave_max<real>(f3);
    { real f[3] = {f1, f2, f3}; pu_max(f, 3); f1 = f[0]; f2 = f[1]; f3 = f[2]; }
    plain_windows = uniform_scalar(f3) == 0.0;
    qnorm = uniform_scalar(f1);
    pd = uniform_scalar(effective_pdiag<real>(pd_user, A.reg_rel, qnorm, uniform_scalar(f2), A.horizon[b], PROX && ((lfb > 0.0) | (dcb > 0.0))));
    if (__any(empty_set)) {
#pragma unroll
      for (int t = 0; t < TS; ++t)
        if (act && tb + t < Tm) A.x[((size_t)b * N + lane) * Tm + tb + t] = 0;
      if constexpr (NPW == 1) {
        double* const xh = A.x_host != nullptr ? A.x_host[b] : nullptr;
        if (xh != nullptr) wave_x_to_host(nullptr, 0, N * Tm, Tm, xh);
      }
      if (A.y_out && !A.y_for_polish_only && half == 0)
        for (int k = lane; k < A.Mg * Tm; k += 64) A.y_out[(size_t)b * A.Mg * Tm + k] = 0;
      if (lane == 0 && half == 0) {
        A.status[b] = 4; A.iters[b] = 0;
        A.pri[b] = 1e300; A.dua[b] = 1e300; A.obj[b] = 0;
      }
      break;
    }
  }

  real z2[SR], y2[SR], gx[SR];
#pragma unroll
  for (int r = 0; r < SR; ++r) { z2[r] = 0; y2[r] = 0; gx[r] = 0; }

  rho = uniform_scalar(rho);
  real a = sigma + pd + rho, inv_a = uniform_scalar(1.0 / a), inv_rho = uniform_scalar(1.0 / rho);
  __builtin_amdgcn_wave_barrier();
  if (lane < 16 * MT) RowDj[lane] = rho / (a + rho * RowLam[lane]);
  wave_lds_sync();

  int status = 2, it = 0, n_adapt = 0, best_it = 0;
  const int check_every = A.check_every;
  int next_check = check_every, next_aa = kAaPeriod;
  real best_score = BIGC;
  real pri = BIGC, dua = BIGC;
  bool done = false, have_prev = false;
  float sn1[TS], sn2[SR];
#pragma unroll
  for (int t = 0; t < TS; ++t) sn1[t] = 0.f;
#pragma unroll
  for (int r = 0; r < SR; ++r) sn2[r] = 0.f;

  constexpr int DV = TS + SR, DVP = 16;
  static_assert(DV <= DVP, "ring row");
  real up[DV];
  float fp[DV], cp[DV];
  float hg[AM][DV];
#pragma unroll
  for (int k = 0; k < DV; ++k) {
    up[k] = 0; fp[k] = 0.f; cp[k] = 0.f;
#pragma unroll
    for (int j = 0; j < AM; ++j) hg[j][k] = 0.f;
  }
  int aa_cnt = 0, aa_head = 0, aa_cool = 0, aa_pen = 1;
  unsigned aa_valid = 0;
  bool aa_have_prev = false, aa_was = false;
  real fn_prev = 0;
  if (aa_m > 0) {
    for (int k = lane; k < AM * AM + AM; k += 64) AaH[k] = 0;
    for (int k = lane; k < aa_m * 64 * 16; k += 64) HistF[k] = 0.f;
    wave_lds_sync();
  }

#ifdef ACNQP_STAMPS
  unsigned long long st_acc[24] = {0}, st_prev;
  asm volatile("s_memtime %0\n\ts_waitcnt lgkmcnt(0)" : "=s"(st_prev)::"memory");
#endif
  auto project_B = [&](const real (&zin)[TS], auto&& between) __attribute__((always_inline)) {
    between();
    STAMP(5);
    const real cap = scap;
    const real tol = M::proj_tol * fmax(1.0, fabs(cap));
    bool need = smode == 0;
    real m = smode == 0 ? mu : 0.0;
    m = smode == 2 ? -BIGC : m;
    m = smode == 3 ? BIGC : m;
    if (plain_windows) {
      real sp = 0;
#pragma unroll
      for (int t = 0; t < TS; ++t) sp += ((imask >> t) & 1u) ? zin[t] : z1[t];
      int ni = __builtin_popcount(imask);
      if constexpr (NPW >= 2) { real nr = (real)ni; pl_sum2(sp, nr); ni = (int)nr; }
      real mp = (sp - cap) * rcp_small((float)(ni > 0 ? ni : 1));
      mp = (!eq & (mp < 0.0)) ? 0.0 : mp;
      m = (need & (ni > 0)) ? mp : m;
    }
    real lo = eq ? -BIGC : -1.0;
    real hi = BIGC;
    int guard = 0;
    for (;;) {
      ++guard;
#ifdef ACNQP_STAMPS
      st_acc[8] += 1000;
#endif
      real gl = 0;
      unsigned im = 0;
      if (plain_windows) {
#pragma unroll
        for (int t = 0; t < TS; ++t) {
          const real v = zin[t] - m;
          const real z = fmin(fmax(v, lbv[t]), ubv[t]);
          z1[t] = z;
          gl += z;
          im |= ((v > lbv[t]) & (v < ubv[t])) ? (1u << t) : 0u;
        }
      } else {
#pragma unroll
        for (int t = 0; t < TS; ++t) {
          const bool inw = (swm >> t) & 1u;
          const real v = zin[t] - (inw ? m : 0.0);
          const real z = fmin(fmax(v, lbv[t]), ubv[t]);
          z1[t] = z;
          gl += inw ? z : 0.0;
          im |= (inw & (v > lbv[t]) & (v < ubv[t])) ? (1u << t) : 0u;
        }
      }
      imask = im;
      float nl = (float)__builtin_popcount(im);
      if constexpr (NPW >= 2) { real nr = (real)nl; pl_sum2(gl, nr); nl = (float)nr; }
      const real d = gl - cap;
      const real big_ = BIGC;
      const bool fin = (fabs(d) <= tol) | (!eq & (m <= 0.0) & (d <= 0.0)) | (guard > ACNQP_GUARD_MAX);
      need = need & !fin;
      if (!__any(need)) break;
      const bool dpos = d > 0;
      lo = (need & dpos) ? m : lo;
      hi = (need & !dpos) ? m : hi;
      const bool open = need & (nl <= 0.f) & !((lo > -big_) & (hi < big_));
      if (__any(open)) {
        real lo_l = big_, hi_l = -big_;
#pragma unroll
        for (int t = 0; t < TS; ++t) {
          const bool inw = (swm >> t) & 1u;
          lo_l = inw ? fmin(lo_l, zin[t] - ubv[t]) : lo_l;
          hi_l = inw ? fmax(hi_l, zin[t] - lbv[t]) : hi_l;
        }
        pl_minmax(lo_l, hi_l);
        lo = open ? fmax(lo, lo_l) : lo;
        hi = open ? fmin(hi, hi_l) : hi;
      }
      const bool bracketed = (lo > -big_) & (hi < big_);
      const real mid = 0.5 * (lo + hi);
      const bool newton = nl > 0.f;
      real rc = rcp_small(newton ? nl : 1.f);
      asm volatile("" : "+v"(rc));
      real c_newton = m + d * rc, c_clamped = fmin(fmax(m + d, lo), hi);
      asm volatile("" : "+v"(c_newton), "+v"(c_clamped));
      real cand = newton ? c_newton : (bracketed ? mid : c_clamped);
      cand = (!eq & (cand < 0.0)) ? 0.0 : cand;
      real a_clamped = fmin(fmax(cand, lo), hi);
      asm volatile("" : "+v"(a_clamped));
      real alt = bracketed ? mid : a_clamped;
      alt = (!eq & (alt < 0.0)) ? 0.0 : alt;
      const bool inside = (cand > lo) & (cand < hi);
      cand = inside ? cand : alt;
      need = need & (cand != m);
      m = need ? cand : m;
    }
    mu = smode == 0 ? m : mu;
  };

  {
    const bool warm = pass == 0 && A.warm_x != nullptr && A.warm_y != nullptr;
    real zs[TS];
#pragma unroll
    for (int t = 0; t < TS; ++t) {
      zs[t] = -scalar_const(kStartGain) * qv[t];
      if (warm) {
        const bool ok = act && tb + t < Tm;
        zs[t] = ok ? A.warm_x[((size_t)b * N + (ok ? lane : 0)) * Tm + (ok ? tb + t : 0)] : 0.0;
      }
    }
    project_B(zs, []() {});
    mu = 0;
    real gty[TS];
#pragma unroll
    for (int t = 0; t < TS; ++t) gty[t] = 0;
    if (warm) {
      const real* RS = static_cast<const real*>(A.rowscale);
      const int Th = min(A.horizon[b], Tm);
      vec4 yv[MT];
#pragma unroll
      for (int r = 0; r < SR; ++r) {
        const int j = 16 * (r >> 2) + M::rowof(g, r & 3);
        const int ja = A.rowabi[j];
        const bool ok = ja >= 0 && tc < TS && tb + tc < Th;
        y2[r] = ok ? A.warm_y[((size_t)b * A.Mg + (ok ? ja : 0)) * Tm + (ok ? tb + tc : 0)] / RS[j] : 0.0;
        yv[r >> 2][r & 3] = y2[r];
      }
      rows_to_evse(yv, frag_g, gty, all_rows);
    }
#pragma unroll
    for (int t = 0; t < TS; ++t) {
      x[t] = z1[t];
      y1[t] = -(qv[t] + pd * z1[t] + gty[t]);
      up[t] = z1[t] + y1[t] * inv_rho;
      cp[t] = 0.f;
    }
    vec4 g0[MT];
    evse_to_rows(z1, FragP, g0);
#pragma unroll
    for (int mo = 0; mo < MT; ++mo) {
      vec4 zt = {0, 0, 0, 0};
#pragma unroll
      for (int mi = 0; mi < ET; ++mi)
#pragma unroll
        for (int s = 0; s < EKOF(mi); ++s) zt = M::mma(FQs[(((mo * MT + mi) * 2 + 1) * 4 + s) * 64 + lane], g0[mi][s], zt);
#pragma unroll
      for (int r = 0; r < 4; ++r) {
        const int k = 4 * mo + r;
        z2[k] = zt[r]; gx[k] = zt[r];
        if (!warm) y2[k] = 0;
        up[TS + k] = zt[r] + y2[k] * inv_rho;
        cp[TS + k] = 0.f;
      }
    }
  }

#ifdef ACNQP_STAMPS
  for (int k = 0; k < 24; ++k) st_acc[k] = 0;
  unsigned long long st_rt0, st_t0;
  asm volatile("s_memrealtime %0\n\ts_waitcnt lgkmcnt(0)" : "=s"(st_rt0)::"memory");
  asm volatile("s_memtime %0\n\ts_waitcnt lgkmcnt(0)" : "=s"(st_prev)::"memory");
  st_t0 = st_prev;
#endif
  while (!done) {
    ++it;
    asm volatile("" : "+v"(swm));
    asm volatile("" : "+v"(smode));
    real r0[TS];
#pragma unroll
    for (int t = 0; t < TS; ++t) r0[t] = sigma * x[t] - qv[t] + rho * z1[t] - y1[t];
    vec4 wh[MT];
#pragma unroll
    for (int mo = 0; mo < ET; ++mo) {
      vec4 acc = {0, 0, 0, 0};
#pragma unroll
      for (int mi = 0; mi < MT; ++mi)
// ... 513 lines not shown
```

Measured before the change: 1.067 million QP solves/s.

## Load first chunk's bounds and costs directly from pinned host memory in kernel

For the first chunk of a pipelined call, the wave kernel now reads lb, ub and q straight from pinned host memory via device-mapped pointers. It copies them into the device input buffers itself instead of waiting on separate H2D memcpys. Per-problem host pointer tables are built in the small pinned mirror, and the order-key pass falls back to session keys so it does not read inputs that have not arrived yet. The aim is to shorten pipeline fill latency before the first kernel starts. The cost is zero-copy PCIe reads from inside the kernel and an extra kernel template instantiation.

```diff
diff --git a/adacharge_amd/backend.py b/adacharge_amd/backend.py
--- a/adacharge_amd/backend.py
+++ b/adacharge_amd/backend.py
@@ -173,6 +173,7 @@
     introspection = [
         ("acnqp_debug_polish_alongside", i64, [h]),
         ("acnqp_debug_direct_x", i64, [h]),
+        ("acnqp_debug_direct_in", i64, [h]),
         ("acnqp_debug_wave_rank", rc, [h, P(i32)]),
         ("acnqp_debug_wave_evse_extent", rc, [h, P(i32)]),
         ("acnqp_debug_order_keys", rc, [h, P(_Problems), P(i32)]),
@@ -1034,6 +1035,9 @@
     def direct_x(self) -> int:
         return int(self._lib.acnqp_debug_direct_x(self._h))
 
+    def direct_in(self) -> int:
+        return int(self._lib.acnqp_debug_direct_in(self._h))
+
     def ordered_launches(self) -> int:
         return int(self._lib.acnqp_ordered_launch_count(self._h))
 
diff --git a/adacharge_amd/csrc/acn_qp_api.hip b/adacharge_amd/csrc/acn_qp_api.hip
--- a/adacharge_amd/csrc/acn_qp_api.hip
+++ b/adacharge_amd/csrc/acn_qp_api.hip
@@ -80,6 +80,7 @@
   hipEvent_t ev_start[kEvRing] = {}, ev_stop[kEvRing] = {};
   long long launches = 0, reported = 0;
   long long ordered_launches = 0;
+  long long direct_in_last = 0;
   long long direct_x_last = 0;
   static constexpr int kSlots = 4;
   struct Slot { hipStream_t st = nullptr; DevBuf in, out, tin; } slot[kSlots];
@@ -187,8 +188,14 @@
   return !no_polish && h->wide_polish && rt.polish_wide_shape && acnqp::polish_wide_holds(s.N, rt.t_max, rt.k_sessions, s.Mg, s.M + s.has_peak);
 }
 
+struct HostTables {
+  double* const* x = nullptr;
+  const double* const* lb = nullptr;
+  const double* const* ub = nullptr;
+  const double* const* q = nullptr;
+};
 int solve_batch_device(acnqp_handle* h, const acnqp_problems* p, const acnqp_options* o, acnqp_results* r, hipStream_t st, bool nothing_follows,
-                       double* const* x_host = nullptr);
+                       const HostTables& ht = HostTables());
 
 }
 
@@ -385,14 +392,15 @@
   a.grid_oversub = own ? 4 : 1;
   a.polish_iters = 0; a.polish_stall = 0; a.resume = 0; a.y_for_polish_only = 0; a.pol_rows = 0; a.pol_list = nullptr; a.pol_count = nullptr; a.pol_retired = nullptr; a.count_dev = nullptr;
   a.x_host = nullptr;
+  a.lb_host = nullptr; a.ub_host = nullptr; a.q_host = nullptr;
   return a;
 }
 
-hipError_t launch_order_keys(acnqp_handle* h, const acnqp::Route& rt, const acnqp_problems* p, hipStream_t st, int32_t* keys) {
+hipError_t launch_order_keys(acnqp_handle* h, const acnqp::Route& rt, const acnqp_problems* p, hipStream_t st, int32_t* keys, bool small_only = false) {
   static const bool by_sessions = [] { const char* e = std::getenv("ACNQP_ORDER_KEY"); return e && std::strcmp(e, "sessions") == 0; }();
   const acnqp::SiteShape& s = h->shape;
   const int g_rows = s.cone == ACNQP_CONE_SOC ? 2 * s.M : s.M;
-  const int waves = by_sessions || rt.family == ACNQP_ROUTE_WAVE4 ? 0 : order_key_waves((size_t)s.N, (size_t)p->t_max, (size_t)g_rows);
+  const int waves = by_sessions || small_only || rt.family == ACNQP_ROUTE_WAVE4 ? 0 : order_key_waves((size_t)s.N, (size_t)p->t_max, (size_t)g_rows);
   if (waves == 0) {
     hipLaunchKernelGGL(session_keys_kernel, dim3((p->batch + 3) / 4), dim3(256), 0, st, p->s_len, p->k_sessions * s.N, p->batch, keys);
     return hipGetLastError();
@@ -424,7 +432,7 @@
     if (want_order) {
       int32_t* keys = static_cast<int32_t*>(wk->ord.p) + 64;
       int32_t* order = keys + p->batch;
-      HIP_TRY(launch_order_keys(h, rt, p, st, keys));
+      HIP_TRY(launch_order_keys(h, rt, p, st, keys, a->lb_host != nullptr));
       hipLaunchKernelGGL(order_sort_kernel, dim3(1), dim3(kOrderKeys), 0, st, keys, p->batch, order);
       a->order = order;
       h->ordered_launches++;
@@ -562,6 +570,7 @@
     a3.resume = 1; a3.order = list; a3.count_dev = ctr + 2; a3.queue = ctr + 1;
     a3.warm_x = r->x; a3.warm_y = ybuf;
     a3.x_host = nullptr;
+    a3.lb_host = nullptr; a3.ub_host = nullptr; a3.q_host = nullptr;
     a3.ws_by_slot = 1; a3.grid_cap = std::min(p->batch, a.grid_oversub > 1 ? 64 : 2 * h->cus);
     if (!a.ws_by_slot) a3.grid_cap = std::min(a3.grid_cap, a.grid_cap);
     *e = launch_solver(h, rt, a3, ws, st);
@@ -614,7 +623,7 @@
 }
 
 int solve_batch_device(acnqp_handle* h, const acnqp_problems* p, const acnqp_options* o, acnqp_results* r, hipStream_t st, bool nothing_follows,
-                       double* const* x_host) {
+                       const HostTables& ht) {
   int rc = check_problem_shapes(h, p, o, r);
   if (rc != ACNQP_OK) return rc;
   if (p->batch == 0) return ACNQP_OK;
@@ -625,8 +634,10 @@
   const int evk = (int)(h->launches % acnqp_handle::kEvRing);
   HIP_TRY(hipEventRecord(h->ev_start[evk], st));
   const acnqp::Route rt = route_of(h, p->t_max, p->k_sessions, p->batch);
-  if (x_host != nullptr && !rt.direct_x()) return fail(ACNQP_ERR_INVALID, "direct x on a route that cannot store it");
-  a.x_host = x_host;
+  if (ht.x != nullptr && !rt.direct_x()) return fail(ACNQP_ERR_INVALID, "direct x on a route that cannot store it");
+  if (ht.lb != nullptr && !rt.direct_in()) return fail(ACNQP_ERR_INVALID, "direct inputs on a route that cannot load them");
+  a.x_host = ht.x;
+  a.lb_host = ht.lb; a.ub_host = ht.ub; a.q_host = ht.q;
   acnqp_handle::Work* wk = h->work_for(st);
   if ((rc = schedule_launch(h, wk, rt, p, st, &a)) != ACNQP_OK) return rc;
   Workspace ws;
@@ -702,6 +713,8 @@
 }
 
 extern "C" int64_t acnqp_debug_direct_x(acnqp_handle* h) { return h ? (int64_t)h->direct_x_last : -1; }
+
+extern "C" int64_t acnqp_debug_direct_in(acnqp_handle* h) { return h ? (int64_t)h->direct_in_last : -1; }
 
 extern "C" int acnqp_debug_wave_rank(acnqp_handle* h, int32_t* out) {
   if (!h || !out) return -1;
diff --git a/adacharge_amd/csrc/acn_qp_common.hpp b/adacharge_amd/csrc/acn_qp_common.hpp
--- a/adacharge_amd/csrc/acn_qp_common.hpp
+++ b/adacharge_amd/csrc/acn_qp_common.hpp
@@ -65,6 +65,9 @@
   int32_t* pol_retired;
   const int32_t* count_dev;
   double* const* x_host;
+  const double* const* lb_host;
+  const double* const* ub_host;
+  const double* const* q_host;
   int ws_by_slot;
   int grid_oversub;
   int grid_cap;
diff --git a/adacharge_amd/csrc/acn_qp_pipeline.hpp b/adacharge_amd/csrc/acn_qp_pipeline.hpp
--- a/adacharge_amd/csrc/acn_qp_pipeline.hpp
+++ b/adacharge_amd/csrc/acn_qp_pipeline.hpp
@@ -22,8 +22,12 @@
 
 inline size_t al256(size_t b) { return (b + 255) & ~(size_t)255; }
 
-struct ChunkShape { size_t N, Tm, K, Mg; bool peak, flat, max, warm, want_y, direct; };
-enum class Per : uint8_t { One, NT, KN, T, MgT };
+struct ChunkShape {
+  size_t N, Tm, K, Mg;
+  bool peak, flat, max, warm, want_y, direct;
+  bool direct_in = false;
+};
+enum class Per : uint8_t { One, NT, KN, T, MgT, Ptrs };
 enum class When : uint8_t { Always, Peak, Flat, Max, Warm, WantY, Direct };
 enum class Size : uint8_t { Large, Small };
 constexpr size_t kNoField = ~(size_t)0;
@@ -45,7 +49,7 @@
     {offsetof(acnqp_problems, lf), 8, Per::One, When::Flat, Size::Small},
     {offsetof(acnqp_problems, dc), 8, Per::One, When::Max, Size::Small},
     {offsetof(acnqp_problems, dfloor), 8, Per::One, When::Max, Size::Small},
-    {kNoField, sizeof(double*), Per::One, When::Direct, Size::Small},
+    {kNoField, sizeof(double*), Per::Ptrs, When::Direct, Size::Small},
     {offsetof(acnqp_problems, warm_x), 8, Per::NT, When::Warm, Size::Large},
     {offsetof(acnqp_problems, warm_y), 8, Per::MgT, When::Warm, Size::Large},
 };
@@ -60,11 +64,11 @@
 };
 
 constexpr bool present(const ArrayRow& r, const ChunkShape& s) {
-  const bool on[] = {true, s.peak, s.flat, s.max, s.warm, s.want_y, s.direct};
+  const bool on[] = {true, s.peak, s.flat, s.max, s.warm, s.want_y, s.direct || s.direct_in};
   return on[(int)r.when];
 }
 constexpr size_t bytes_per_problem(const ArrayRow& r, const ChunkShape& s) {
-  const size_t n[] = {1, s.N * s.Tm, s.K * s.N, s.Tm, s.Mg * s.Tm};
+  const size_t n[] = {1, s.N * s.Tm, s.K * s.N, s.Tm, s.Mg * s.Tm, s.direct_in ? (size_t)4 : (size_t)1};
   return r.elem * n[(int)r.per];
 }
 struct RowRange { int first, end; };
@@ -76,6 +80,7 @@
     if (rows[k].size == Size::Small) return {n, n};
   return {first, end};
 }
+enum HostTable { kHostX, kHostLb, kHostUb, kHostQ };
 constexpr RowRange kSmallIn = small_rows(kIn, kInRows), kSmallOut = small_rows(kOut, kOutRows);
 static_assert(kSmallIn.first < kSmallIn.end && kSmallOut.first < kSmallOut.end, "the small rows of a side are one contiguous run: the pinned mirror is one copy");
 
@@ -83,7 +88,8 @@
   ChunkShape shape;
   size_t cn, in[kInRows + 1], out[kOutRows + 1];
   bool direct;
-  ChunkLayout(size_t cn_, const ChunkShape& s) : shape(s), cn(cn_), direct(s.direct) {
+  bool direct_in;
+  ChunkLayout(size_t cn_, const ChunkShape& s) : shape(s), cn(cn_), direct(s.direct), direct_in(s.direct_in) {
     auto lay = [&](const ArrayRow* rows, int n, size_t* off) {
       off[0] = 0;
       for (int k = 0; k < n; ++k) off[k + 1] = off[k] + al256(present(rows[k], s) ? cn * bytes_per_problem(rows[k], s) : 0);
@@ -95,6 +101,7 @@
   size_t mirror_in_bytes() const { return in[kSmallIn.end] - in[kSmallIn.first]; }
   size_t mirror_out() const { return out[kSmallOut.first]; }
   size_t mirror_out_bytes() const { return out[kSmallOut.end] - out[kSmallOut.first]; }
+  size_t host_table(HostTable k) const { return in[kXh] + (size_t)k * cn * sizeof(double*); }
 };
 
 struct TableSpan { long long lo = 0, cn = 0, s0 = 0, ns = 0, r0 = 0, nr = 0; size_t qt = 0; };
@@ -139,6 +146,7 @@
   const char* plan = nullptr;
   bool ramp = true;
   bool direct = false;
+  bool direct_in = false;
 };
 
 inline long long chunk_cap_by_memory(size_t N, size_t Tm, size_t K) {
@@ -341,6 +349,8 @@
   std::vector<ChunkLayout> layout;
   std::vector<Scatter> scatter;
   std::vector<double*> xdst;
+  struct HostIn { const double *lb = nullptr, *ub = nullptr, *q = nullptr; };
+  std::vector<HostIn> isrc;
 };
 
 double* direct_destination(const double* x) {
@@ -352,6 +362,17 @@
     return nullptr;
   }
   return at.type == hipMemoryTypeHost ? static_cast<double*>(at.devicePointer) : nullptr;
+}
+
+const double* direct_source(const double* a) {
+  static const bool off = std::getenv("ACNQP_NO_DIRECT_IN") != nullptr;
+  if (off || a == nullptr) return nullptr;
+  hipPointerAttribute_t at;
+  if (hipPointerGetAttributes(&at, a) != hipSuccess) {
+    (void)hipGetLastError();
+    return nullptr;
+  }
+  return at.type == hipMemoryTypeHost ? static_cast<const double*>(at.devicePointer) : nullptr;
 }
 
 inline char* member(const void* s, size_t field) { char* p; std::memcpy(&p, static_cast<const char*>(s) + field, sizeof p); return p; }
@@ -386,6 +407,7 @@
           const acnqp::Route rt = acnqp::route_for(h->shape, b.t_max, b.k_sessions, (int)std::min<long long>(total, acnqp::kRouteAnyBatch), route_switches());
           acnqp::PlanEnv e = env;
           e.direct = env.direct && rt.direct_x();
+          e.direct_in = env.direct_in && rt.direct_in();
           caps = acnqp::plan_chunk_caps(total, rt.chunk_want(), acnqp::chunk_cap_by_memory((size_t)h->shape.N, (size_t)b.t_max, (size_t)b.k_sessions),
                                         rt.wv > 0, uniform, e);
         }
@@ -399,11 +421,12 @@
   return chunks;
 }
 
-hipError_t upload_piece(const ChunkLayout& L, const acnqp_problems& src, size_t lo, size_t n, size_t pos, char* di, char* hs, hipStream_t st) {
+hipError_t upload_piece(const ChunkLayout& L, const acnqp_problems& src, size_t lo, size_t n, size_t pos, char* di, char* hs, hipStream_t st,
+                        bool loaded = false) {
   hipError_t e = hipSuccess;
   for (int k = 0; k < kInRows && e == hipSuccess; ++k) {
     const char* from = kIn[k].field != kNoField && present(kIn[k], L.shape) ? member(&src, kIn[k].field) : nullptr;
-    if (!from) continue;
+    if (!from || (loaded && (k == kLb || k == kUb || k == kQ))) continue;
     const size_t per = bytes_per_problem(kIn[k], L.shape);
     if (hs && kIn[k].size == Size::Small) std::memcpy(hs + L.in[k] + pos * per, from + lo * per, n * per);
     else e = hipMemcpyAsync(di + L.in[k] + pos * per, from + lo * per, n * per, hipMemcpyHostToDevice, st);
@@ -418,11 +441,21 @@
   if (chain && c > 0) HIP_TRY(hipStreamWaitEvent(S.st, h->h2d_done[(c - 1) % acnqp_handle::kSlots], 0));
   for (const Piece& pc : pcs) {
     const size_t lo = (size_t)pc.lo, n = (size_t)pc.n, pos = (size_t)pc.pos;
-    HIP_TRY(upload_piece(L, call.P[pc.g], lo, n, pos, di, hs, S.st));
-    if (hs && L.direct) {
-      double** tab = reinterpret_cast<double**>(hs + L.in[kXh]) + pos;
-      double* const dst = call.xdst[pc.g];
-      for (size_t i = 0; i < n; ++i) tab[i] = dst ? dst + (lo + i) * L.shape.N * L.shape.Tm : nullptr;
+    const Call::HostIn in = hs && L.direct_in ? call.isrc[pc.g] : Call::HostIn();
+    HIP_TRY(upload_piece(L, call.P[pc.g], lo, n, pos, di, hs, S.st, in.lb != nullptr));
+    const size_t nv = L.shape.N * L.shape.Tm;
+    if (hs && (L.direct || L.direct_in)) {
+      double** tab = reinterpret_cast<double**>(hs + L.host_table(kHostX)) + pos;
+      double* const dst = L.direct ? call.xdst[pc.g] : nullptr;
+      for (size_t i = 0; i < n; ++i) tab[i] = dst ? dst + (lo + i) * nv : nullptr;
+    }
+    if (hs && L.direct_in) {
+      const double* const from[] = {in.lb, in.ub, in.q};
+      const HostTable which[] = {kHostLb, kHostUb, kHostQ};
+      for (int k = 0; k < 3; ++k) {
+        const double** tab = reinterpret_cast<const double**>(hs + L.host_table(which[k])) + pos;
+        for (size_t i = 0; i < n; ++i) tab[i] = from[k] ? from[k] + (lo + i) * nv : nullptr;
+      }
     }
   }
   if (hs) HIP_TRY(hipMemcpyAsync(di + L.mirror_in(), hs + L.mirror_in(), L.mirror_in_bytes(), hipMemcpyHostToDevice, S.st));
@@ -472,7 +505,31 @@
     call.xdst[g] = call.bs[g].batch > 0 ? direct_destination(call.R[g].x) : nullptr;
     env.direct = env.direct && (call.xdst[g] != nullptr || call.bs[g].batch == 0);
   }
+  h->direct_in_last = 0;
+  call.isrc.assign(call.bs.size(), Call::HostIn());
+  std::vector<char> asked(call.bs.size(), 0);
+  auto sources = [&](int g) {
+    if (!asked[g]) {
+      asked[g] = 1;
+      const acnqp_problems& P = call.P[g];
+      Call::HostIn in;
+      in.lb = direct_source(P.lb);
+      if (in.lb) in.ub = direct_source(P.ub);
+      if (in.ub) in.q = direct_source(P.q);
+      if (in.q) call.isrc[g] = in;
+    }
+    return call.isrc[g].lb != nullptr;
+  };
+  for (size_t g = 0; g < call.bs.size() && !table; ++g)
+    if (call.bs[g].batch > 0) { env.direct_in = sources((int)g); break; }
   const std::vector<std::vector<Piece>> chunks = split_call(h, call.bs, env);
+  bool direct_in = false;
+  if (!table && chunks.size() > 1) {
+    const std::vector<Piece>& pcs = chunks[0];
+    const BatchShape& b = call.bs[pcs[0].g];
+    if (route_of(h, b.t_max, b.k_sessions, (int)(pcs.back().pos + pcs.back().n)).direct_in())
+      for (const Piece& pc : pcs) direct_in = sources(pc.g) || direct_in;
+  }
   std::vector<char> direct(chunks.size(), 0);
   for (size_t c = 0; c < chunks.size() && !table; ++c) {
     const std::vector<Piece>& pcs = chunks[c];
@@ -484,7 +541,8 @@
     const std::vector<Piece>& pcs = chunks[c];
     const BatchShape& b = call.bs[pcs[0].g];
     return ChunkLayout((size_t)(pcs.back().pos + pcs.back().n),
-                       ChunkShape{N, (size_t)b.t_max, (size_t)b.k_sessions, Mg, s.has_peak != 0, s.has_flat != 0, s.has_max != 0, b.warm, b.want_y, direct[c] != 0});
+                       ChunkShape{N, (size_t)b.t_max, (size_t)b.k_sessions, Mg, s.has_peak != 0, s.has_flat != 0, s.has_max != 0, b.warm, b.want_y, direct[c] != 0,
+                                  direct_in && c == 0});
   };
   constexpr size_t kSmallCap = (size_t)256 << 20;
   std::vector<size_t> in_off(chunks.size()), out_off(chunks.size());
@@ -501,6 +559,7 @@
     HIP_TRY(h->small_out.reserve(out_sum));
   } else {
     std::fill(direct.begin(), direct.end(), 0);
+    direct_in = false;
   }
   for (size_t c = 0; c < chunks.size(); ++c) {
     acnqp_handle::Slot& S = h->slot[c % acnqp_handle::kSlots];
@@ -519,8 +578,14 @@
     acnqp_problems dp;
     acnqp_results dr;
     device_views(L, di, dq, b, &dp, &dr);
-    double* const* x_host = L.direct ? reinterpret_cast<double* const*>(di + L.in[kXh]) : nullptr;
-    rc = solve_batch_device(h, &dp, o, &dr, S.st, c + 1 == chunks.size(), x_host);
+    HostTables ht;
+    if (L.direct) ht.x = reinterpret_cast<double* const*>(di + L.host_table(kHostX));
+    if (L.direct_in) {
+      ht.lb = reinterpret_cast<const double* const*>(di + L.host_table(kHostLb));
+      ht.ub = reinterpret_cast<const double* const*>(di + L.host_table(kHostUb));
+      ht.q = reinterpret_cast<const double* const*>(di + L.host_table(kHostQ));
+    }
+    rc = solve_batch_device(h, &dp, o, &dr, S.st, c + 1 == chunks.size(), ht);
     if (rc != ACNQP_OK) return rc;
     if (staged) HIP_TRY(hipMemcpyAsync(ho + L.mirror_out(), dq + L.mirror_out(), L.mirror_out_bytes(), hipMemcpyDeviceToHost, S.st));
     for (const Piece& pc : pcs) {
@@ -528,6 +593,7 @@
       const size_t lo = (size_t)pc.lo, n = (size_t)pc.n, pos = (size_t)pc.pos;
       const bool stored = L.direct && call.xdst[pc.g];
       if (stored) h->direct_x_last += (long long)n;
+      if (L.direct_in && call.isrc[pc.g].lb) h->direct_in_last += (long long)n;
       for (int k = 0; k < kOutRows; ++k) {
         if (!present(kOut[k], L.shape) || (k == kX && stored) || (staged && kOut[k].size == Size::Small)) continue;
         const size_t per = bytes_per_problem(kOut[k], L.shape);
diff --git a/adacharge_amd/csrc/acn_qp_route.hpp b/adacharge_amd/csrc/acn_qp_route.hpp
--- a/adacharge_amd/csrc/acn_qp_route.hpp
+++ b/adacharge_amd/csrc/acn_qp_route.hpp
@@ -73,6 +73,8 @@
 
   bool direct_x() const { return wv == 1; }
 
+  bool direct_in() const { return wv == 1; }
+
   template <class Kn> int accel_cap() const {
     if (wv > 0) return Kn::wave_accel();
     if (tiled) return Kn::tiled_accel(site.MR / 16, (t_max + 15) / 16, site.NP(), k_sessions);
diff --git a/adacharge_amd/csrc/acn_qp_wave.hip b/adacharge_amd/csrc/acn_qp_wave.hip
--- a/adacharge_amd/csrc/acn_qp_wave.hip
+++ b/adacharge_amd/csrc/acn_qp_wave.hip
@@ -12,14 +12,14 @@
 
 static_assert(kRouteWaveTS == kWaveTS, "acn_qp_route.hpp restates the period slots per lane");
 
-template <int NPW, int TSV, int MT, bool PROX, int EK, int NE = ACNQP_WAVE_NE>
+template <int NPW, int TSV, int MT, bool PROX, int EK, bool HIN = false, int NE = ACNQP_WAVE_NE>
 static hipError_t launch_wave_prox(const TiledArgs& a_in, const WaveSite& ws, hipStream_t st) {
   TiledArgs a = a_in;
   if (EK > 0) { a.Ghat = ws.Ghat; a.lam = ws.lam; a.fragQ = ws.fragQ; }
   a.accel_mem = std::min(a.accel_mem, kWaveAM);
   const WaveLds L(a.accel_mem, NPW, MT, TSV);
   const size_t lds = (size_t)L.total * 8;
-  auto kern = &admm_wave_kernel<kWaveAM, NPW, TSV, MT, PROX, EK, NE>;
+  auto kern = &admm_wave_kernel<kWaveAM, NPW, TSV, MT, PROX, EK, NE, HIN>;
   if (lds > 64 * 1024) {
     hipError_t e = ensure_dynamic_lds(reinterpret_cast<const void*>(kern), lds);
     if (e != hipSuccess) return e;
@@ -41,6 +41,12 @@
 
 template <int NPW, int TSV, int MT, int EK>
 static hipError_t launch_wave_ek(const TiledArgs& a, const WaveSite& ws, hipStream_t st) {
+  if (a.lb_host != nullptr) {
+    if constexpr (NPW == 1)
+      return a.lf != nullptr || a.dc != nullptr ? launch_wave_prox<NPW, TSV, MT, true, EK, true>(a, ws, st) : launch_wave_prox<NPW, TSV, MT, false, EK, true>(a, ws, st);
+    else
+      return hipErrorInvalidValue;
+  }
   return a.lf != nullptr || a.dc != nullptr ? launch_wave_prox<NPW, TSV, MT, true, EK>(a, ws, st) : launch_wave_prox<NPW, TSV, MT, false, EK>(a, ws, st);
 }
 template <int NPW, int TSV, int MT>
diff --git a/adacharge_amd/csrc/acn_qp_wave.hpp b/adacharge_amd/csrc/acn_qp_wave.hpp
--- a/adacharge_amd/csrc/acn_qp_wave.hpp
+++ b/adacharge_amd/csrc/acn_qp_wave.hpp
@@ -65,9 +65,21 @@
   }
 }
 
-template <int AM, int NPW, int TSV, int MT, bool PROX, int EK = 0, int NE = 0>
+__device__ __attribute__((always_inline)) inline void wave_in_from_host(int n, const double* lh, const double* uh, const double* qh,
+                                                                        double* lb, double* ub, double* q) {
+  const int lane = threadIdx.x & 63;
+#pragma unroll 4
+  for (int k = lane; k < n; k += 64) {
+    const double l = lh[k], u = uh[k], c = qh[k];
+    lb[k] = l; ub[k] = u; q[k] = c;
+  }
+  __threadfence();
+}
+
+template <int AM, int NPW, int TSV, int MT, bool PROX, int EK = 0, int NE = 0, bool HIN = false>
 __global__ __launch_bounds__(kWaveNW * 64, 1) void admm_wave_kernel(const TiledArgs A_kernarg) {
   static_assert(NPW == 1 || NPW == 2 || NPW == 4, "one, two or four waves per problem");
+  static_assert(!HIN || NPW == 1, "host sources: one wave per problem");
   static_assert((TSV == 12 && MT == 1) || (TSV == 6 && MT == 2 && NPW >= 2), "instantiated: 12 periods x one row tile, 6 periods x two row tiles");
   using M = Mfma<double>;
   using vec4 = typename M::vec4;
@@ -315,6 +327,13 @@
 
   const bool act = lane < N;
   real x[TS], z1[TS], y1[TS], qv[TS], lbv[TS], ubv[TS];
+  if constexpr (HIN) {
+    const real* const lh = pass == 0 && A.lb_host != nullptr ? A.lb_host[b] : nullptr;
+    if (lh != nullptr) {
+      const size_t at = (size_t)b * N * Tm;
+      wave_in_from_host(N * Tm, lh, A.ub_host[b], A.q_host[b], const_cast<real*>(A.lb) + at, const_cast<real*>(A.ub) + at, const_cast<real*>(A.q) + at);
+    }
+  }
 #pragma unroll
   for (int t = 0; t < TS; ++t) {
     const bool ok = act && tb + t < Tm;
```

Result: faster. 1.083 million QP solves/s, median of 6 (+1.5%).
